# yangcaoai/CoDA_NeurIPS2023

Measured on NVIDIA H100. Metric: training scenes/sec (20k-pt SUN-RGBD synth, 256 queries), higher is better.
Workload: dtype fp32

## Files before the change

coda_neurips2023_b200/csrc/a32_prologue.cuh:

```cuda
#pragma once

namespace coda {
namespace a32 {

__device__ __forceinline__ float affine_relu(float x, float s, float h) { return fmaxf(fmaf(x, s, h), 0.f); }

__device__ __forceinline__ float bn_bwd(float y, float d, float s, float h, float al, float be) {
  return (fmaf(y, s, h) > 0.f ? s * d : 0.f) + fmaf(y, al, be);
}

__device__ __forceinline__ float bn_bwd_pooled(float y, float d, bool at_max, float s, float h, float al, float be) {
  return ((at_max && fmaf(y, s, h) > 0.f) ? s * d : 0.f) + fmaf(y, al, be);
}

__device__ __forceinline__ float bn_bwd_pooled_pre(float y, float d, bool at_max, float al, float be) {
  return (at_max ? d : 0.f) + fmaf(y, al, be);
}

}
}
```

coda_neurips2023_b200/csrc/gemm_a32_sm90.cu:

```cuda
#include "../../include/coda_gemm.h"
#include "a32_prologue.cuh"
#include "sm90_primitives.cuh"

#include <type_traits>

using namespace coda;

namespace {

constexpr int BM = 128;
constexpr int BK = 64;
constexpr int RAW_TILE = BM * BK * 4;
constexpr int A32_THREADS = 288;

struct A32Maps {
  CUtensorMap a;
  CUtensorMap a2;
  CUtensorMap b[3];
};

struct A32Params {
  int m, n, k;
  int mode;
  const float *scale;
  const float *shift;
  const float *alpha;
  const float *beta;
  const float *dpooled;
  const unsigned char *argmax;
  int group;
  const float *bias;
  int act;
  float *c;
  long long ldc;
  float *stats;
  int b_resident;
};

struct Alternation {
  int wg;
  bool started;
  __device__ __forceinline__ void begin() {
    if (wg == 1 || started) bar_sync(2 + wg, 256);
  }
  __device__ __forceinline__ void end() {
    bar_arrive(2 + (wg ^ 1), 256);
    started = true;
  }
  __device__ __forceinline__ void finish() {
    if (wg == 0 && started) bar_sync(2, 256);
  }
};

template <int NSPLIT, int BN, int RAW_KB, int B_STAGES, bool B_MN>
__global__ void __launch_bounds__(A32_THREADS, 1)
gemm_a32_kernel(const __grid_constant__ A32Maps maps, const A32Params P) {
  constexpr int MAX_RAW = RAW_KB / 32;
  constexpr int B_TILE = BN * BK * 2;
  constexpr int B_STAGE = NSPLIT * B_TILE;
  extern __shared__ __align__(1024) unsigned char smem_raw[];
  unsigned char *smem = smem_align1024(smem_raw);
  unsigned char *raw_ring = smem;
  const bool two_in = P.mode == CODA_A32_BN_BWD;
  const bool pooled = P.mode == CODA_A32_BN_BWD_POOLED || P.mode == CODA_A32_BN_BWD_POOLED_PRE;
  const int tile_groups = pooled ? (P.group >= BM ? 1 : BM / P.group) : 0;
  const int raw_stage_bytes = RAW_TILE * (two_in ? 2 : 1) + (tile_groups * 320 + 1023) / 1024 * 1024;
  const uint32_t nraw = (uint32_t)((RAW_KB * 1024) / raw_stage_bytes);
  unsigned char *b_ring = smem + (size_t)RAW_KB * 1024;
  float *s_stats = reinterpret_cast<float *>(b_ring + (size_t)B_STAGES * B_STAGE);
  __shared__ __align__(8) uint64_t raw_full[MAX_RAW], raw_empty[MAX_RAW];
  __shared__ __align__(8) uint64_t b_full[B_STAGES], b_empty[B_STAGES];

  const int warp = threadIdx.x >> 5, lane = threadIdx.x & 31;
  const int m = P.m, n = P.n;
  const int tiles_m = (m + BM - 1) / BM, tiles_n = (n + BN - 1) / BN;
  const long long nwork = (long long)tiles_m * tiles_n;
  const int nkb = (P.k + BK - 1) / BK;
  auto tile_at = [&](long long t, int &m0, int &n0) -> bool {
    if (P.b_resident) {
      const int per = (int)gridDim.x / tiles_n;
      const long long tm = (long long)(blockIdx.x / tiles_n) + t * per;
      if ((int)blockIdx.x >= per * tiles_n || tm >= tiles_m) return false;
      m0 = (int)tm * BM;
      n0 = (int)(blockIdx.x % tiles_n) * BN;
      return true;
    }
    const long long w = blockIdx.x + t * gridDim.x;
    if (w >= nwork) return false;
    n0 = (int)(w % tiles_n) * BN;
    m0 = (int)(w / tiles_n) * BM;
    return true;
  };

  if (threadIdx.x == 0) {
    for (int s = 0; s < MAX_RAW; ++s) { mbar_init(&raw_full[s], 1); mbar_init(&raw_empty[s], 8); }
    for (int s = 0; s < B_STAGES; ++s) { mbar_init(&b_full[s], 1); mbar_init(&b_empty[s], 2); }
    mbar_fence_init_cluster();
  }
  if (P.stats && warp < 8) {
    float *mine = s_stats + (size_t)warp * 2 * n;
    for (int i = lane; i < 2 * n; i += 32) mine[i] = 0.f;
  }
  __syncthreads();

  if (warp == 8) {
    if (lane == 0) {
      prefetch_tmap(&maps.a);
      if (two_in) prefetch_tmap(&maps.a2);
#pragma unroll
      for (int p = 0; p < NSPLIT; ++p) prefetch_tmap(&maps.b[p]);
    }
    uint32_t it = 0;
    int m0, n0;
    auto load_b = [&](int kb, int bs) {
      unsigned char *bt = b_ring + (size_t)bs * B_STAGE;
      mbar_arrive_expect_tx(&b_full[bs], (uint32_t)B_STAGE);
#pragma unroll
      for (int p = 0; p < NSPLIT; ++p) {
        if (!B_MN) {
          tma_load_3d(bt + p * B_TILE, &maps.b[p], &b_full[bs], kb * BK, n0, 0);
        } else {
#pragma unroll
          for (int g = 0; g < BN / 64; ++g)
            tma_load_3d(bt + p * B_TILE + g * 8192, &maps.b[p], &b_full[bs], n0 + g * 64, kb * BK, 0);
        }
      }
    };
    if (P.b_resident && tile_at(0, m0, n0)) {
      if (elect_one_sync())
        for (int kb = 0; kb < nkb; ++kb) load_b(kb, kb);
      __syncwarp();
    }
    for (long long t = 0; tile_at(t, m0, n0); ++t) {
      for (int kb = 0; kb < nkb; ++kb, ++it) {
        const int rs = it % nraw, bs = it % B_STAGES;
        mbar_wait(&raw_empty[rs], ((it / nraw) & 1u) ^ 1u);
        if (!P.b_resident) mbar_wait(&b_empty[bs], ((it / B_STAGES) & 1u) ^ 1u);
        if (elect_one_sync()) {
          unsigned char *rt = raw_ring + (size_t)rs * raw_stage_bytes;
          mbar_arrive_expect_tx(&raw_full[rs], (uint32_t)(RAW_TILE * (two_in ? 2 : 1) + tile_groups * 320));
          if (pooled) {
            const long long ngroups = P.m / P.group;
            for (int gt = 0; gt < tile_groups; ++gt) {
              long long g = (long long)m0 / P.group + gt;
              if (g >= ngroups) g = ngroups - 1;
              bulk_load_1d(rt + RAW_TILE + gt * 320, P.dpooled + g * P.k + kb * BK, 256, &raw_full[rs]);
              bulk_load_1d(rt + RAW_TILE + gt * 320 + 256, P.argmax + g * P.k + kb * BK, 64, &raw_full[rs]);
            }
          }
          tma_load_3d(rt, &maps.a, &raw_full[rs], kb * BK, m0, 0);
          tma_load_3d(rt + RAW_TILE / 2, &maps.a, &raw_full[rs], kb * BK + 32, m0, 0);
          if (two_in) {
            tma_load_3d(rt + RAW_TILE, &maps.a2, &raw_full[rs], kb * BK, m0, 0);
            tma_load_3d(rt + RAW_TILE + RAW_TILE / 2, &maps.a2, &raw_full[rs], kb * BK + 32, m0, 0);
          }
          if (!P.b_resident) load_b(kb, bs);
        }
        __syncwarp();
      }
    }
    return;
  }

  const int wg = warp >> 2, wl = warp & 3;
  const int g = lane >> 2, t4 = lane & 3;
  const int rloc[2] = {wg * 64 + wl * 16 + g, wg * 64 + wl * 16 + g + 8};
  float acc[BN / 2];
  uint32_t it = 0;
  int m0, n0;
  Alternation mma_turn{wg, false};
  for (long long t = 0; tile_at(t, m0, n0); ++t) {
    for (int kb = 0; kb < nkb; ++kb, ++it) {
      const int rs = it % nraw, bs = P.b_resident ? kb : (int)(it % B_STAGES);
      mbar_wait(&raw_full[rs], (it / nraw) & 1u);
      const unsigned char *rt = raw_ring + (size_t)rs * raw_stage_bytes;
      const int k0 = kb * BK;
      uint32_t af[BK / 16][NSPLIT][4];
      auto convert = [&](auto mode_tag) {
        constexpr int MODE = decltype(mode_tag)::value;
        const int mode = MODE >= 0 ? MODE : P.mode;
        int pgt = 0, pgi[2] = {0, 0};
        if (MODE < 0 && pooled) {
          pgt = P.group >= BM ? 0 : rloc[0] / P.group;
#pragma unroll
          for (int i = 0; i < 2; ++i) pgi[i] = (int)(((long long)m0 + rloc[i]) % P.group);
        }
#pragma unroll
        for (int kk = 0; kk < BK / 16; ++kk) {
#pragma unroll
          for (int c2 = 0; c2 < 2; ++c2) {
            const int col = kk * 16 + c2 * 8 + 2 * t4;
            const int kc = k0 + col;
            auto off = [&](int i) {
              const int row = rloc[i];
              return (uint32_t)(col >> 5) * (RAW_TILE / 2) + (uint32_t)row * 128u +
                     ((uint32_t)(((col & 31) >> 2) ^ (row & 7)) << 4) + (uint32_t)(col & 3) * 4u;
            };
            auto put = [&](int i, float2 x) {
              uint32_t w[NSPLIT];
              split_pair<NSPLIT>(x.x, x.y, w);
#pragma unroll
              for (int pl = 0; pl < NSPLIT; ++pl) af[kk][pl][c2 * 2 + i] = w[pl];
            };
            auto ld2 = [&](const float *v) { return __ldg(reinterpret_cast<const float2 *>(v + kc)); };
            if (mode == CODA_A32_AFFINE_RELU) {
              const float2 s2 = ld2(P.scale), h2 = ld2(P.shift);
#pragma unroll
              for (int i = 0; i < 2; ++i) {
                float2 x = *reinterpret_cast<const float2 *>(rt + off(i));
                x.x = a32::affine_relu(x.x, s2.x, h2.x);
                x.y = a32::affine_relu(x.y, s2.y, h2.y);
                put(i, x);
              }
            } else if (mode == CODA_A32_BN_BWD) {
              const float2 s2 = ld2(P.scale), h2 = ld2(P.shift), a2 = ld2(P.alpha), b2 = ld2(P.beta);
#pragma unroll
              for (int i = 0; i < 2; ++i) {
                float2 x = *reinterpret_cast<const float2 *>(rt + off(i));
                const float2 d = *reinterpret_cast<const float2 *>(rt + RAW_TILE + off(i));
                x.x = a32::bn_bwd(x.x, d.x, s2.x, h2.x, a2.x, b2.x);
                x.y = a32::bn_bwd(x.y, d.y, s2.y, h2.y, a2.y, b2.y);
                put(i, x);
              }
            } else if (mode == CODA_A32_BN_BWD_POOLED_PRE) {
              const unsigned char *px = rt + RAW_TILE + pgt * 320;
              const float2 a2 = ld2(P.alpha), b2 = ld2(P.beta);
              const float2 d = *reinterpret_cast<const float2 *>(px + col * 4);
              const uchar2 id = *reinterpret_cast<const uchar2 *>(px + 256 + col);
#pragma unroll
              for (int i = 0; i < 2; ++i) {
                float2 x = *reinterpret_cast<const float2 *>(rt + off(i));
                const int gi = pgi[i];
                x.x = a32::bn_bwd_pooled_pre(x.x, d.x, id.x == gi, a2.x, b2.x);
                x.y = a32::bn_bwd_pooled_pre(x.y, d.y, id.y == gi, a2.y, b2.y);
                put(i, x);
              }
            } else if (mode == CODA_A32_BN_BWD_POOLED) {
              const unsigned char *px = rt + RAW_TILE + pgt * 320;
              const float2 s2 = ld2(P.scale), h2 = ld2(P.shift), a2 = ld2(P.alpha), b2 = ld2(P.beta);
              const float2 d = *reinterpret_cast<const float2 *>(px + col * 4);
              const uchar2 id = *reinterpret_cast<const uchar2 *>(px + 256 + col);
#pragma unroll
              for (int i = 0; i < 2; ++i) {
                float2 x = *reinterpret_cast<const float2 *>(rt + off(i));
                const int gi = pgi[i];
                x.x = a32::bn_bwd_pooled(x.x, d.x, id.x == gi, s2.x, h2.x, a2.x, b2.x);
                x.y = a32::bn_bwd_pooled(x.y, d.y, id.y == gi, s2.y, h2.y, a2.y, b2.y);
                put(i, x);
              }
            } else {
#pragma unroll
              for (int i = 0; i < 2; ++i) put(i, *reinterpret_cast<const float2 *>(rt + off(i)));
            }
          }
        }
      };
      switch (P.mode) {
        case CODA_A32_PLAIN: convert(std::integral_constant<int, CODA_A32_PLAIN>{}); break;
        case CODA_A32_AFFINE_RELU: convert(std::integral_constant<int, CODA_A32_AFFINE_RELU>{}); break;
        default: convert(std::integral_constant<int, -1>{}); break;
      }
      __syncwarp();
      if (lane == 0) mbar_arrive(&raw_empty[rs]);
      mma_turn.begin();
      mbar_wait(&b_full[bs], P.b_resident ? 0u : ((it / B_STAGES) & 1u));
      unsigned char *bt = b_ring + (size_t)bs * B_STAGE;
      acc_fence(acc);
      wgmma_fence();
#pragma unroll
      for (int p = 0; p < n_products(NSPLIT); ++p) {
        const void *btile = bt + prod_b(NSPLIT, p) * B_TILE;
        const uint64_t bd = B_MN ? gmma_desc_mn_sw128(btile) : gmma_desc_k_sw128(btile);
        constexpr uint32_t KSTEP = B_MN ? 16 * 128 : 32;
#pragma unroll
        for (int kk = 0; kk < BK / 16; ++kk)
          Wgmma<BN, false>::template rs<B_MN ? 1 : 0>(acc, af[kk][prod_a(NSPLIT, p)], gmma_desc_advance(bd, kk * KSTEP),
                                                      (kb | p | kk) != 0);
      }
      wgmma_commit();
      mma_turn.end();
      wgmma_wait<0>();
      acc_fence(acc);
      if (!P.b_resident && (threadIdx.x & 127) == 0) mbar_arrive(&b_empty[bs]);
    }

    constexpr int EPI_C = 4;
#pragma unroll
    for (int cb = 0; cb < BN / 8; cb += EPI_C) {
      float csum[EPI_C][2], csq[EPI_C][2];
#pragma unroll
      for (int ci = 0; ci < EPI_C; ++ci) {
        const int c = cb + ci;
        const int col = n0 + c * 8 + 2 * t4;
        float cs0 = 0.f, cs1 = 0.f, cq0 = 0.f, cq1 = 0.f;
        const float bias0 = P.bias && col < n ? __ldg(P.bias + col) : 0.f;
        const float bias1 = P.bias && col + 1 < n ? __ldg(P.bias + col + 1) : 0.f;
#pragma unroll
        for (int i = 0; i < 2; ++i) {
          const int row = m0 + rloc[i];
          float v0 = acc[c * 4 + i * 2], v1 = acc[c * 4 + i * 2 + 1];
          if (P.bias) {
            if (col < n) v0 += bias0;
            if (col + 1 < n) v1 += bias1;
          }
          if (P.act == 1) { v0 = fmaxf(v0, 0.f); v1 = fmaxf(v1, 0.f); }
          if (row < m) {
            float *crow = P.c + (size_t)row * P.ldc;
            if (col + 1 < n) {
              *reinterpret_cast<float2 *>(crow + col) = make_float2(v0, v1);
            } else if (col < n) {
              crow[col] = v0;
            }
            cs0 += v0; cq0 = fmaf(v0, v0, cq0);
            cs1 += v1; cq1 = fmaf(v1, v1, cq1);
          }
        }
        csum[ci][0] = cs0; csum[ci][1] = cs1; csq[ci][0] = cq0; csq[ci][1] = cq1;
      }
      if (P.stats) {
        float *my_stats = s_stats + warp * 2 * n;
#pragma unroll
        for (int o = 4; o < 32; o <<= 1) {
#pragma unroll
          for (int ci = 0; ci < EPI_C; ++ci) {
#pragma unroll
            for (int j = 0; j < 2; ++j) {
              csum[ci][j] += __shfl_xor_sync(0xffffffffu, csum[ci][j], o);
              csq[ci][j] += __shfl_xor_sync(0xffffffffu, csq[ci][j], o);
            }
          }
        }
        if (g == 0) {
#pragma unroll
          for (int ci = 0; ci < EPI_C; ++ci) {
            const int col = n0 + (cb + ci) * 8 + 2 * t4;
#pragma unroll
            for (int j = 0; j < 2; ++j) {
              if (col + j < n) { my_stats[col + j] += csum[ci][j]; my_stats[n + col + j] += csq[ci][j]; }
            }
          }
        }
      }
    }
  }
  mma_turn.finish();
  if (P.stats) {
    bar_sync(1, 256);
    float *out = P.stats + (size_t)blockIdx.x * 2 * n;
    for (int i = threadIdx.x; i < 2 * n; i += 256) {
      float v = 0.f;
#pragma unroll
      for (int w = 0; w < 8; ++w) v += s_stats[(size_t)w * 2 * n + i];
      out[i] = v;
    }
  }
}

template <int NSPLIT, int BN, int RAW_KB, int B_STAGES, bool B_MN>
int launch_a32(const A32Maps &maps, const A32Params &P, cudaStream_t s) {
  static_assert(RAW_KB % 64 == 0 || RAW_KB == 96, "raw region");
  constexpr size_t smem = (size_t)RAW_KB * 1024 + (size_t)B_STAGES * NSPLIT * BN * BK * 2 + 1024;
  const size_t total = smem + (P.stats ? (size_t)16 * P.n * 4 : 0);
  constexpr size_t SMEM_MAX = 227 * 1024 - 2048;
  if (total > SMEM_MAX) return CODA_ETOOLARGE;
  if (P.mode == CODA_A32_BN_BWD && RAW_KB < 64) return CODA_EINVAL;
  constexpr auto kern = gemm_a32_kernel<NSPLIT, BN, RAW_KB, B_STAGES, B_MN>;
  if (const int st = raise_smem_limit<kern>((int)SMEM_MAX)) return st;
  const int tiles_m = (P.m + BM - 1) / BM, tiles_n = (P.n + BN - 1) / BN;
  const long long nwork = (long long)tiles_m * tiles_n;
  unsigned grid = (unsigned)(nwork < sm_count() ? nwork : sm_count());
  A32Params Q = P;
  const int nkb = (P.k + BK - 1) / BK;
  Q.b_resident = (nkb <= B_STAGES && tiles_n <= sm_count() && tiles_m >= 4 * (sm_count() / tiles_n)) ? 1 : 0;
  if (Q.b_resident) grid = (unsigned)((sm_count() / tiles_n) * tiles_n);
  kern<<<grid, A32_THREADS, total, s>>>(maps, Q);
  return launch_status();
}

}

extern "C" {

int coda_gemm_a32_grid(int m, int n) {
  if (m <= 0 || n <= 0) return 0;
  return sm_count();
}

int coda_gemm_a32(int nsplit, int m, int n, int k, const float *a, long long lda, int a_mode, const float *a_scale,
                  const float *a_shift, const float *a_alpha, const float *a_beta, const float *a2, long long lda2,
                  const unsigned char *a_argmax, int a_group, const void *b_planes, long long b_plane_stride,
                  int b_ld, int b_mn, const float *bias, int act, float *c, long long ldc, float *col_stats,
                  void *stream) {
  if (nsplit < 2 || nsplit > 3 || m < 0 || n < 0 || k <= 0) return CODA_EINVAL;
  if (m == 0 || n == 0) return CODA_OK;
  if (!a || !b_planes || !c || b_ld % 64 != 0 || (lda & 3) || (ldc & 3) || ((uintptr_t)a & 15) || ((uintptr_t)c & 15))
    return CODA_EINVAL;
  if (a_mode < CODA_A32_PLAIN || a_mode > CODA_A32_BN_BWD_POOLED_PRE) return CODA_EINVAL;
  if (a_mode != CODA_A32_PLAIN && (!a_scale || !a_shift || (k & 3))) return CODA_EINVAL;
  if (a_mode >= CODA_A32_BN_BWD && (!a2 || !a_alpha || !a_beta || ((uintptr_t)a2 & 15))) return CODA_EINVAL;
  if (a_mode == CODA_A32_BN_BWD && (lda2 & 3)) return CODA_EINVAL;
  if ((a_mode == CODA_A32_BN_BWD_POOLED || a_mode == CODA_A32_BN_BWD_POOLED_PRE) &&
      (!a_argmax || a_group < 32 || a_group > 256 || m % a_group != 0 || k % 64 != 0 ||
       !(a_group % 128 == 0 || 128 % a_group == 0) || a_group % 32 != 0))
    return CODA_EINVAL;
  const long long tiles128 = (long long)((m + BM - 1) / BM) * ((n + 127) / 128);
  const int bn = (n <= 64 || tiles128 <= sm_count() / 2) ? 64 : 128;
  A32Maps maps;
  int st = make_tmap_f32_box(&maps.a, a, k, m, lda, 32, BM);
  if (st != CODA_OK) return st;
  maps.a2 = maps.a;
  if (a_mode == CODA_A32_BN_BWD) {
    st = make_tmap_f32_box(&maps.a2, a2, k, m, lda2, 32, BM);
    if (st != CODA_OK) return st;
  }
  const int kpad = (k + 63) / 64 * 64;
  const char *bp = (const char *)b_planes;
  for (int p = 0; p < nsplit; ++p) {
    if (!b_mn) {
      if (b_ld < kpad) return CODA_EINVAL;
      st = make_tmap_k_major_16b(&maps.b[p], bp + (size_t)p * b_plane_stride * 2, 0, b_ld, n, 1, b_ld, 0, bn);
    } else {
      if (b_ld < n) return CODA_EINVAL;
      st = make_tmap_k_major_16b(&maps.b[p], bp + (size_t)p * b_plane_stride * 2, 0, b_ld, k, 1, b_ld, 0, 64);
    }
    if (st != CODA_OK) return st;
  }
  for (int p = nsplit; p < 3; ++p) maps.b[p] = maps.b[0];
  A32Params P;
  P.m = m; P.n = n; P.k = k; P.mode = a_mode; P.scale = a_scale; P.shift = a_shift; P.alpha = a_alpha; P.beta = a_beta;
  P.dpooled = a2; P.argmax = a_argmax; P.group = a_group; P.bias = bias; P.act = act; P.c = c; P.ldc = ldc; P.stats = col_stats;
  P.b_resident = 0;
  cudaStream_t s = (cudaStream_t)stream;
#define CODA_A32(NS, BN_, RS, BS)                                                   \
  return b_mn ? launch_a32<NS, BN_, RS, BS, true>(maps, P, s) : launch_a32<NS, BN_, RS, BS, false>(maps, P, s)
  const bool deep_b = !col_stats && k > 128 && a_mode != CODA_A32_BN_BWD;
  if (nsplit == 2) {
    if (bn == 64) CODA_A32(2, 64, 128, 4);
    CODA_A32(2, 128, 128, 2);
  }
  if (bn == 64) CODA_A32(3, 64, 128, 3);
  if (deep_b) CODA_A32(3, 128, 64, 3);
  CODA_A32(3, 128, 96, 2);
#undef CODA_A32
}

}
```

coda_neurips2023_b200/csrc/gemm_tn32_sm90.cu:

```cuda
#include "../../include/coda_gemm.h"
#include "a32_prologue.cuh"
#include "sm90_primitives.cuh"

using namespace coda;

namespace {

constexpr int BM = 128;
constexpr int BKR = 32;
constexpr int NS = 2;
constexpr int RAW_STAGES = 2, PL_STAGES = 3;
constexpr int TW = 8;
constexpr int TN32_THREADS = 288;

struct TN32Maps {
  CUtensorMap a, a2, b;
};

struct TN32Params {
  long long rows;
  int m, n;
  int a_mode, b_mode;
  const float *a_scale, *a_shift, *a_alpha, *a_beta;
  const float *dpooled;
  const unsigned char *argmax;
  int group;
  const float *b_scale, *b_shift;
  float *a_colsum;
  float *partial;
  float *c;
  long long ldc;
  int ksplit;
};

template <int BN>
__global__ void __launch_bounds__(TN32_THREADS, 1)
gemm_tn32_kernel(const __grid_constant__ TN32Maps maps, const TN32Params P) {
  constexpr int RAW_A = BKR * BM * 4;
  constexpr int RAW_B = BKR * BN * 4;
  constexpr int RAW_X = 1024;
  constexpr int RAW_STAGE = 2 * RAW_A + RAW_B + RAW_X;
  constexpr int PL_A = BKR * BM * 2;
  constexpr int PL_B = BKR * BN * 2;
  constexpr int PL_STAGE = NS * (PL_A + PL_B);
  extern __shared__ __align__(1024) unsigned char smem_raw[];
  unsigned char *smem = smem_align1024(smem_raw);
  unsigned char *raw_ring = smem;
  unsigned char *pl_ring = smem + (size_t)RAW_STAGES * RAW_STAGE;
  __shared__ __align__(8) uint64_t raw_full[RAW_STAGES], raw_empty[RAW_STAGES];
  __shared__ __align__(16) float s_colsum[TW][BM];

  const int warp = threadIdx.x >> 5, lane = threadIdx.x & 31;
  const int tiles_n = (P.n + BN - 1) / BN;
  const int tile = blockIdx.x / P.ksplit, ks = blockIdx.x % P.ksplit;
  const int m0 = (tile / tiles_n) * BM, n0 = (tile % tiles_n) * BN;
  const long long nkb_total = (P.rows + BKR - 1) / BKR;
  const long long per = (nkb_total + P.ksplit - 1) / P.ksplit;
  const long long kb0 = (long long)ks * per;
  const long long nkb = max(0ll, min(per, nkb_total - kb0));
  const bool two_in = P.a_mode == CODA_A32_BN_BWD;

  if (threadIdx.x == 0) {
    for (int s = 0; s < RAW_STAGES; ++s) { mbar_init(&raw_full[s], 1); mbar_init(&raw_empty[s], TW); }
    mbar_fence_init_cluster();
  }
  __syncthreads();

  if (warp == 8) {
    if (lane == 0) {
      prefetch_tmap(&maps.a);
      prefetch_tmap(&maps.b);
      if (two_in) prefetch_tmap(&maps.a2);
    }
    const bool pooled = P.a_mode == CODA_A32_BN_BWD_POOLED || P.a_mode == CODA_A32_BN_BWD_POOLED_PRE;
    const uint32_t bytes = (uint32_t)(RAW_A * (two_in ? 2 : 1) + RAW_B + (pooled ? 640 : 0));
    const long long ngroups = pooled ? P.rows / P.group : 0;
    for (long long i = 0; i < nkb; ++i) {
      const int rs = (int)(i % RAW_STAGES);
      mbar_wait(&raw_empty[rs], (uint32_t)((i / RAW_STAGES) & 1) ^ 1u);
      if (elect_one_sync()) {
        unsigned char *st = raw_ring + (size_t)rs * RAW_STAGE;
        const int r0 = (int)((kb0 + i) * BKR);
        mbar_arrive_expect_tx(&raw_full[rs], bytes);
        if (pooled) {
          long long g = (long long)r0 / P.group;
          if (g >= ngroups) g = ngroups - 1;
          bulk_load_1d(st + 2 * RAW_A + RAW_B, P.dpooled + g * P.m + m0, 512, &raw_full[rs]);
          bulk_load_1d(st + 2 * RAW_A + RAW_B + 512, P.argmax + g * P.m + m0, 128, &raw_full[rs]);
        }
#pragma unroll
        for (int g = 0; g < BM / 32; ++g) tma_load_3d(st + g * 4096, &maps.a, &raw_full[rs], m0 + g * 32, r0, 0);
        if (two_in) {
#pragma unroll
          for (int g = 0; g < BM / 32; ++g) tma_load_3d(st + RAW_A + g * 4096, &maps.a2, &raw_full[rs], m0 + g * 32, r0, 0);
        }
#pragma unroll
        for (int g = 0; g < BN / 32; ++g) tma_load_3d(st + 2 * RAW_A + g * 4096, &maps.b, &raw_full[rs], n0 + g * 32, r0, 0);
      }
      __syncwarp();
    }
    return;
  }

  const int tw = warp;
  const int wg = warp >> 2;
  const bool want_colsum = P.a_colsum != nullptr && n0 == 0;
  float4 csum = make_float4(0.f, 0.f, 0.f, 0.f);
  const int ca = m0 + lane * 4;
  float4 sa = make_float4(0.f, 0.f, 0.f, 0.f), ta = sa, al = sa, be = sa;
  if (P.a_mode != CODA_A32_PLAIN && ca < P.m) {
    sa = __ldg(reinterpret_cast<const float4 *>(P.a_scale + ca));
    ta = __ldg(reinterpret_cast<const float4 *>(P.a_shift + ca));
    al = __ldg(reinterpret_cast<const float4 *>(P.a_alpha + ca));
    be = __ldg(reinterpret_cast<const float4 *>(P.a_beta + ca));
  }
  constexpr int B_CHUNKS = BN / 4, B_RPP = 32 / B_CHUNKS;
  const int bch = lane % B_CHUNKS, brow_off = lane / B_CHUNKS;
  const int cb = n0 + bch * 4;
  float4 sb = make_float4(0.f, 0.f, 0.f, 0.f), tb = sb;
  if (P.b_mode == CODA_A32_AFFINE_RELU && cb < P.n) {
    sb = __ldg(reinterpret_cast<const float4 *>(P.b_scale + cb));
    tb = __ldg(reinterpret_cast<const float4 *>(P.b_shift + cb));
  }
  const bool a_col_ok = ca < P.m;
  const bool pooled_mode = P.a_mode == CODA_A32_BN_BWD_POOLED || P.a_mode == CODA_A32_BN_BWD_POOLED_PRE;
  int rem0 = pooled_mode ? (int)((kb0 * BKR) % P.group) : 0;
  int rs = 0, ps = 0;
  uint32_t raw_par = 0;
  float acc[BN / 2];
  for (long long i = 0; i < nkb; ++i) {
    mbar_wait_relaxed(&raw_full[rs], raw_par);
    const unsigned char *raw = raw_ring + (size_t)rs * RAW_STAGE;
    unsigned char *pl = pl_ring + (size_t)ps * PL_STAGE;
    const long long r0 = (kb0 + i) * BKR;
    const bool tail = r0 + BKR > P.rows;
#pragma unroll
      for (int j = 0; j < BKR / TW; ++j) {
        const int r = tw + j * TW;
        const long long grow = r0 + r;
        const uint32_t roff = (uint32_t)(lane >> 3) * 4096u + (uint32_t)r * 128u + (uint32_t)(((lane & 7) ^ (r & 7)) << 4);
        float4 y = *reinterpret_cast<const float4 *>(raw + roff);
        float4 o = y;
        if (P.a_mode == CODA_A32_BN_BWD) {
          const float4 d = *reinterpret_cast<const float4 *>(raw + RAW_A + roff);
          o.x = a32::bn_bwd(y.x, d.x, sa.x, ta.x, al.x, be.x);
          o.y = a32::bn_bwd(y.y, d.y, sa.y, ta.y, al.y, be.y);
          o.z = a32::bn_bwd(y.z, d.z, sa.z, ta.z, al.z, be.z);
          o.w = a32::bn_bwd(y.w, d.w, sa.w, ta.w, al.w, be.w);
        } else if (P.a_mode == CODA_A32_BN_BWD_POOLED_PRE) {
          const int gi = rem0 + r;
          const float4 d = *reinterpret_cast<const float4 *>(raw + 2 * RAW_A + RAW_B + lane * 16);
          const uchar4 id = *reinterpret_cast<const uchar4 *>(raw + 2 * RAW_A + RAW_B + 512 + lane * 4);
          o.x = a32::bn_bwd_pooled_pre(y.x, d.x, id.x == gi, al.x, be.x);
          o.y = a32::bn_bwd_pooled_pre(y.y, d.y, id.y == gi, al.y, be.y);
          o.z = a32::bn_bwd_pooled_pre(y.z, d.z, id.z == gi, al.z, be.z);
          o.w = a32::bn_bwd_pooled_pre(y.w, d.w, id.w == gi, al.w, be.w);
        } else if (P.a_mode == CODA_A32_BN_BWD_POOLED) {
          const int gi = rem0 + r;
          const float4 d = *reinterpret_cast<const float4 *>(raw + 2 * RAW_A + RAW_B + lane * 16);
          const uchar4 id = *reinterpret_cast<const uchar4 *>(raw + 2 * RAW_A + RAW_B + 512 + lane * 4);
          o.x = a32::bn_bwd_pooled(y.x, d.x, id.x == gi, sa.x, ta.x, al.x, be.x);
          o.y = a32::bn_bwd_pooled(y.y, d.y, id.y == gi, sa.y, ta.y, al.y, be.y);
          o.z = a32::bn_bwd_pooled(y.z, d.z, id.z == gi, sa.z, ta.z, al.z, be.z);
          o.w = a32::bn_bwd_pooled(y.w, d.w, id.w == gi, sa.w, ta.w, al.w, be.w);
        }
        if (tail && grow >= P.rows) o = make_float4(0.f, 0.f, 0.f, 0.f);
        if (want_colsum) { csum.x += o.x; csum.y += o.y; csum.z += o.z; csum.w += o.w; }
        const int col = lane * 4;
        split_store4<NS>(o, reinterpret_cast<__nv_bfloat16 *>(pl + (col >> 6) * (BKR * 128) + r * 128 +
                                                              ((((col & 63) >> 3) ^ (r & 7)) << 4) + ((col & 7) >> 2) * 8),
                         PL_A / 2);
      }
#pragma unroll
      for (int j = 0; j < BKR / (TW * B_RPP); ++j) {
        const int r = (tw + j * TW) * B_RPP + brow_off;
        const long long grow = r0 + r;
        const uint32_t roff = (uint32_t)(bch >> 3) * 4096u + (uint32_t)r * 128u + (uint32_t)(((bch & 7) ^ (r & 7)) << 4);
        float4 v = *reinterpret_cast<const float4 *>(raw + 2 * RAW_A + roff);
        if (P.b_mode == CODA_A32_AFFINE_RELU) {
          v.x = a32::affine_relu(v.x, sb.x, tb.x); v.y = a32::affine_relu(v.y, sb.y, tb.y);
          v.z = a32::affine_relu(v.z, sb.z, tb.z); v.w = a32::affine_relu(v.w, sb.w, tb.w);
        }
        if (tail && grow >= P.rows) v = make_float4(0.f, 0.f, 0.f, 0.f);
        const int col = bch * 4;
        split_store4<NS>(v, reinterpret_cast<__nv_bfloat16 *>(pl + NS * PL_A + (col >> 6) * (BKR * 128) + r * 128 +
                                                              ((((col & 63) >> 3) ^ (r & 7)) << 4) + ((col & 7) >> 2) * 8),
                         PL_B / 2);
      }
      fence_proxy_async_smem();
      __syncwarp();
      if (lane == 0) mbar_arrive(&raw_empty[rs]);
      bar_sync(1, 256);
      acc_fence(acc);
      wgmma_fence();
#pragma unroll
      for (int p = 0; p < n_products(NS); ++p) {
        const uint64_t ad = gmma_desc_mn_sw128(pl + prod_a(NS, p) * PL_A + wg * (BKR * 128), BKR * 128);
        const uint64_t bd = gmma_desc_mn_sw128(pl + NS * PL_A + prod_b(NS, p) * PL_B, BKR * 128);
#pragma unroll
        for (int kk = 0; kk < BKR / 16; ++kk)
          Wgmma<BN, false>::template ss<1, 1>(acc, gmma_desc_advance(ad, kk * 16 * 128), gmma_desc_advance(bd, kk * 16 * 128),
                                              (i | p | kk) != 0);
      }
      wgmma_commit();
      wgmma_wait<1>();
      acc_fence(acc);
      if (++rs == RAW_STAGES) { rs = 0; raw_par ^= 1u; }
      if (++ps == PL_STAGES) ps = 0;
      if (pooled_mode) { rem0 += BKR; if (rem0 >= P.group) rem0 -= P.group; }
  }
  wgmma_wait<0>();
  acc_fence(acc);
  if (nkb == 0) acc_zero(acc);
  *reinterpret_cast<float4 *>(&s_colsum[tw][lane * 4]) = csum;
  {
    const int g = lane >> 2, t4 = lane & 3;
    float *slot = P.partial + ((long long)tile * P.ksplit + ks) * (BM * BN);
#pragma unroll
    for (int i = 0; i < 2; ++i) {
      const int rl = wg * 64 + (warp & 3) * 16 + g + 8 * i, row = m0 + rl;
      float *crow = P.c + (size_t)row * P.ldc;
#pragma unroll
      for (int c = 0; c < BN / 8; ++c) {
        const int col = n0 + c * 8 + 2 * t4;
        const float2 v = make_float2(acc[c * 4 + i * 2], acc[c * 4 + i * 2 + 1]);
        if (P.ksplit > 1) *reinterpret_cast<float2 *>(slot + (size_t)rl * BN + c * 8 + 2 * t4) = v;
        else if (row < P.m && col < P.n) *reinterpret_cast<float2 *>(crow + col) = v;
      }
    }
  }
  bar_sync(1, 256);
  if (P.a_colsum && n0 == 0 && threadIdx.x < BM) {
    float cs = 0.f;
#pragma unroll
    for (int w = 0; w < TW; ++w) cs += s_colsum[w][threadIdx.x];
    if (P.ksplit > 1) {
      const int tiles_m = (P.m + BM - 1) / BM;
      P.partial[(long long)tiles_m * (tiles_n * P.ksplit) * (BM * BN) + ((long long)(m0 / BM) * P.ksplit + ks) * BM +
                threadIdx.x] = cs;
    } else if (m0 + (int)threadIdx.x < P.m) {
      P.a_colsum[m0 + threadIdx.x] = cs;
    }
  }
}

__global__ void __launch_bounds__(256)
colsum_reduce_kernel(const float *__restrict__ parts, int ksplit, int m, float *__restrict__ a_colsum) {
  const int col = blockIdx.x * blockDim.x + threadIdx.x;
  if (col >= m) return;
  const float *src = parts + ((long long)(col / BM) * ksplit) * BM + col % BM;
  float v = 0.f;
  for (int k = 0; k < ksplit; ++k) v += src[(long long)k * BM];
  a_colsum[col] = v;
}

template <int BN>
int launch_tn32(const TN32Maps &maps, TN32Params P, float *c, long long ldc, cudaStream_t s) {
  constexpr size_t smem = (size_t)RAW_STAGES * (2 * BKR * BM * 4 + BKR * BN * 4 + 1024) +
                          (size_t)PL_STAGES * NS * (BKR * BM * 2 + BKR * BN * 2) + 1024;
  static_assert(smem <= 227 * 1024, "smem budget");
  constexpr auto kern = gemm_tn32_kernel<BN>;
  if (const int st = raise_smem_limit<kern>((int)smem)) return st;
  const int num_sms = sm_count();
  const int tiles = ((P.m + BM - 1) / BM) * ((P.n + BN - 1) / BN);
  const long long nkb_total = (P.rows + BKR - 1) / BKR;
  int ksplit = num_sms / tiles;
  if (ksplit < 1) ksplit = 1;
  if (ksplit > nkb_total / 4) ksplit = (int)(nkb_total / 4 > 0 ? nkb_total / 4 : 1);
  P.ksplit = ksplit;
  const int tiles_m = (P.m + BM - 1) / BM;
  if (ksplit > 1) {
    const int st = split_scratch((size_t)tiles * ksplit * BM * BN + (size_t)tiles_m * ksplit * BM, s, &P.partial);
    if (st != CODA_OK) return st;
  }
  kern<<<tiles * ksplit, TN32_THREADS, smem, s>>>(maps, P);
  if (ksplit > 1) {
    const long long total = (long long)P.m * P.n;
    const long long blocks = (total + 255) / 256;
    splitk_reduce_kernel<<<(unsigned)(blocks < 8 * num_sms ? blocks : 8 * num_sms), 256, 0, s>>>(
        P.partial, ksplit, P.m, P.n, 1, BM, BN, nullptr, c, ldc, 0);
    if (P.a_colsum)
      colsum_reduce_kernel<<<(P.m + 255) / 256, 256, 0, s>>>(P.partial + (size_t)tiles * ksplit * BM * BN, ksplit, P.m,
                                                            P.a_colsum);
  }
  return launch_status();
}

}

extern "C" {

int coda_gemm_tn32(long long rows, int m, int n, const float *a, long long lda, int a_mode, const float *a_scale,
                   const float *a_shift, const float *a_alpha, const float *a_beta, const float *a2, long long lda2,
                   const unsigned char *a_argmax, int a_group, const float *b, long long ldb, int b_mode,
                   const float *b_scale, const float *b_shift, float *c, long long ldc, float *a_colsum, void *stream) {
  if (rows <= 0 || m <= 0 || n <= 0 || !a || !b || !c) return CODA_EINVAL;
  if ((lda & 3) || (ldb & 3) || (ldc & 3) || (m & 3) || (n & 3)) return CODA_EINVAL;
  if (((uintptr_t)a | (uintptr_t)b | (uintptr_t)c) & 15) return CODA_EINVAL;
  if (a_mode != CODA_A32_PLAIN && a_mode != CODA_A32_BN_BWD && a_mode != CODA_A32_BN_BWD_POOLED &&
      a_mode != CODA_A32_BN_BWD_POOLED_PRE)
    return CODA_EINVAL;
  if (b_mode != CODA_A32_PLAIN && b_mode != CODA_A32_AFFINE_RELU) return CODA_EINVAL;
  if (a_mode != CODA_A32_PLAIN && (!a_scale || !a_shift || !a_alpha || !a_beta || !a2 || ((uintptr_t)a2 & 15))) return CODA_EINVAL;
  if (a_mode == CODA_A32_BN_BWD && (lda2 & 3)) return CODA_EINVAL;
  if ((a_mode == CODA_A32_BN_BWD_POOLED || a_mode == CODA_A32_BN_BWD_POOLED_PRE) &&
      (!a_argmax || a_group < 32 || a_group > 256 || a_group % 32 != 0 || rows % a_group != 0 || m % 128 != 0))
    return CODA_EINVAL;
  if (b_mode == CODA_A32_AFFINE_RELU && (!b_scale || !b_shift)) return CODA_EINVAL;
  TN32Maps maps;
  int st = make_tmap_f32_box(&maps.a, a, m, rows, lda, 32, BKR);
  if (st != CODA_OK) return st;
  maps.a2 = maps.a;
  if (a_mode == CODA_A32_BN_BWD) {
    st = make_tmap_f32_box(&maps.a2, a2, m, rows, lda2, 32, BKR);
    if (st != CODA_OK) return st;
  }
  st = make_tmap_f32_box(&maps.b, b, n, rows, ldb, 32, BKR);
  if (st != CODA_OK) return st;
  TN32Params P;
  P.rows = rows; P.m = m; P.n = n; P.a_mode = a_mode; P.b_mode = b_mode;
  P.a_scale = a_scale; P.a_shift = a_shift; P.a_alpha = a_alpha; P.a_beta = a_beta;
  P.dpooled = a2; P.argmax = a_argmax; P.group = a_group; P.b_scale = b_scale; P.b_shift = b_shift; P.a_colsum = a_colsum; P.partial = nullptr; P.c = c; P.ldc = ldc; P.ksplit = 1;
  cudaStream_t s = (cudaStream_t)stream;
  if (n <= 64) return launch_tn32<64>(maps, P, c, ldc, s);
  return launch_tn32<128>(maps, P, c, ldc, s);
}

}
```

coda_neurips2023_b200/csrc/sa_mlp_kernels.cu:

```cuda
#include <cuda_bf16.h>
#include <math.h>
#include <stdint.h>

#include "../../include/coda_sa_mlp.h"
#include "coda_common.cuh"
#include "operand_split.cuh"

namespace {

constexpr int THREADS = 256;
constexpr int MAX_BLOCKS = 132 * 4;

__host__ __device__ inline bool channels_ok(int c) { return c >= 4 && c <= 1024 && c % 4 == 0 && THREADS % (c / 4) == 0; }

__host__ inline unsigned grid_for(long long rows, int c) {
  const long long per_iter = THREADS / (c / 4);
  const long long need = (rows + per_iter - 1) / per_iter;
  return (unsigned)(need < MAX_BLOCKS ? (need > 0 ? need : 1) : MAX_BLOCKS);
}

struct Affine4 {
  float4 mean, invstd, gamma, beta;
};
__device__ __forceinline__ Affine4 load_affine(const float *mean, const float *invstd, const float *gamma,
                                               const float *beta, int c4) {
  Affine4 a;
  a.mean = __ldg(reinterpret_cast<const float4 *>(mean) + c4);
  a.invstd = __ldg(reinterpret_cast<const float4 *>(invstd) + c4);
  a.gamma = __ldg(reinterpret_cast<const float4 *>(gamma) + c4);
  a.beta = __ldg(reinterpret_cast<const float4 *>(beta) + c4);
  return a;
}
__device__ __forceinline__ float4 xhat4(const float4 v, const Affine4 &a) {
  return make_float4((v.x - a.mean.x) * a.invstd.x, (v.y - a.mean.y) * a.invstd.y, (v.z - a.mean.z) * a.invstd.z,
                     (v.w - a.mean.w) * a.invstd.w);
}
__device__ __forceinline__ float4 bn4(const float4 xh, const Affine4 &a) {
  return make_float4(xh.x * a.gamma.x + a.beta.x, xh.y * a.gamma.y + a.beta.y, xh.z * a.gamma.z + a.beta.z,
                     xh.w * a.gamma.w + a.beta.w);
}

template <int NV>
__device__ __forceinline__ void reduce_slots(float4 (&acc)[NV], int cq, int slot, int c4, float4 *red ) {
#pragma unroll
  for (int i = 0; i < NV; ++i) {
    __syncthreads();
    red[threadIdx.x] = acc[i];
    __syncthreads();
    if (slot == 0) {
      float4 t = acc[i];
      for (int s = 1; s < THREADS / cq; ++s) {
        const float4 o = red[s * cq + c4];
        t.x += o.x; t.y += o.y; t.z += o.z; t.w += o.w;
      }
      acc[i] = t;
    }
  }
}

template <int CIN>
__global__ void __launch_bounds__(THREADS)
linear_small_k_kernel(long long rows, int cout, const float *__restrict__ x, const float *__restrict__ w,
                      float *__restrict__ y) {
  const int cq = cout >> 2, c4 = threadIdx.x % cq, slot = threadIdx.x / cq, nslots = THREADS / cq;
  float wr[4][CIN];
#pragma unroll
  for (int j = 0; j < 4; ++j)
#pragma unroll
    for (int k = 0; k < CIN; ++k) wr[j][k] = __ldg(w + (size_t)(c4 * 4 + j) * CIN + k);
  for (long long r = (long long)blockIdx.x * nslots + slot; r < rows; r += (long long)gridDim.x * nslots) {
    float xv[CIN];
#pragma unroll
    for (int k = 0; k < CIN; ++k) xv[k] = __ldg(x + r * CIN + k);
    float o[4];
#pragma unroll
    for (int j = 0; j < 4; ++j) {
      float a = xv[0] * wr[j][0];
#pragma unroll
      for (int k = 1; k < CIN; ++k) a = fmaf(xv[k], wr[j][k], a);
      o[j] = a;
    }
    reinterpret_cast<float4 *>(y + r * cout)[c4] = make_float4(o[0], o[1], o[2], o[3]);
  }
}

__global__ void __launch_bounds__(THREADS)
bn_stats_partial_kernel(long long rows, int c, const float *__restrict__ y, float *__restrict__ partial) {
  __shared__ float4 red[THREADS];
  const int cq = c >> 2, c4 = threadIdx.x % cq, slot = threadIdx.x / cq, nslots = THREADS / cq;
  float4 acc[2] = {make_float4(0.f, 0.f, 0.f, 0.f), make_float4(0.f, 0.f, 0.f, 0.f)};
  for (long long r = (long long)blockIdx.x * nslots + slot; r < rows; r += (long long)gridDim.x * nslots) {
    const float4 v = __ldg(reinterpret_cast<const float4 *>(y + r * c) + c4);
    acc[0].x += v.x; acc[0].y += v.y; acc[0].z += v.z; acc[0].w += v.w;
    acc[1].x = fmaf(v.x, v.x, acc[1].x); acc[1].y = fmaf(v.y, v.y, acc[1].y);
    acc[1].z = fmaf(v.z, v.z, acc[1].z); acc[1].w = fmaf(v.w, v.w, acc[1].w);
  }
  reduce_slots<2>(acc, cq, slot, c4, red);
  if (slot == 0) {
    float4 *p = reinterpret_cast<float4 *>(partial + (size_t)blockIdx.x * 2 * c);
    p[c4] = acc[0];
    p[cq + c4] = acc[1];
  }
}
__device__ __forceinline__ void warp_partials_sum(int nblocks, int c, int ch, const float *__restrict__ partial,
                                                  double &s, double &q) {
  const int lane = threadIdx.x & 31;
  s = 0.0; q = 0.0;
  for (int b = lane; b < nblocks; b += 32) {
    s += (double)partial[(size_t)b * 2 * c + ch];
    q += (double)partial[(size_t)b * 2 * c + c + ch];
  }
#pragma unroll
  for (int o = 16; o > 0; o >>= 1) {
    s += __shfl_xor_sync(0xffffffffu, s, o);
    q += __shfl_xor_sync(0xffffffffu, q, o);
  }
}
__global__ void __launch_bounds__(256)
bn_stats_finalize_kernel(int nblocks, long long rows, int c, const float *__restrict__ partial,
                         float eps, float momentum, float *running_mean, float *running_var,
                         float *__restrict__ mean, float *__restrict__ invstd) {
  const int ch = blockIdx.x * 8 + (threadIdx.x >> 5);
  if (ch >= c) return;
  double s, q;
  warp_partials_sum(nblocks, c, ch, partial, s, q);
  if ((threadIdx.x & 31) != 0) return;
  const double n = (double)rows, m = s / n;
  double var = q / n - m * m;
  if (var < 0.0) var = 0.0;
  mean[ch] = (float)m;
  invstd[ch] = (float)(1.0 / sqrt(var + (double)eps));
  if (running_mean) running_mean[ch] = (1.0f - momentum) * running_mean[ch] + momentum * (float)m;
  if (running_var) running_var[ch] = (1.0f - momentum) * running_var[ch] + momentum * (float)(var * (n / fmax(n - 1.0, 1.0)));
}

__global__ void __launch_bounds__(256)
bn_stats_finalize_affine_kernel(int nblocks, long long rows, int c, int cpad,
                                                const float *__restrict__ partial, float eps, float momentum,
                                                float *running_mean, float *running_var, const float *__restrict__ gamma,
                                                const float *__restrict__ beta, float *__restrict__ mean,
                                                float *__restrict__ invstd, float *__restrict__ scale,
                                                float *__restrict__ shift) {
  const int ch = blockIdx.x * 8 + (threadIdx.x >> 5);
  if (ch >= cpad) return;
  if (ch >= c) {
    if (scale && (threadIdx.x & 31) == 0) { scale[ch] = 0.f; shift[ch] = 0.f; }
    return;
  }
  double s, q;
  warp_partials_sum(nblocks, c, ch, partial, s, q);
  if ((threadIdx.x & 31) != 0) return;
  const double n = (double)rows, m = s / n;
  double var = q / n - m * m;
  if (var < 0.0) var = 0.0;
  const float is = (float)(1.0 / sqrt(var + (double)eps));
  mean[ch] = (float)m;
  invstd[ch] = is;
  if (running_mean) running_mean[ch] = (1.0f - momentum) * running_mean[ch] + momentum * (float)m;
  if (running_var) running_var[ch] = (1.0f - momentum) * running_var[ch] + momentum * (float)(var * (n / fmax(n - 1.0, 1.0)));
  if (scale) {
    const float sc = gamma[ch] * is;
    scale[ch] = sc;
    shift[ch] = beta[ch] - (float)m * sc;
  }
}
__global__ void __launch_bounds__(256)
bn_sums_f64_kernel(int nblocks, int c, const float *__restrict__ partial, double *__restrict__ sums) {
  const int ch = blockIdx.x * 8 + (threadIdx.x >> 5);
  if (ch >= c) return;
  double s, q;
  warp_partials_sum(nblocks, c, ch, partial, s, q);
  if ((threadIdx.x & 31) != 0) return;
  sums[ch] = s;
  sums[c + ch] = q;
}
__global__ void __launch_bounds__(256)
bn_finalize_sums_kernel(long long rows, int c, int cpad, const double *__restrict__ sums, float eps, float momentum,
                        float *running_mean, float *running_var, const float *__restrict__ gamma,
                        const float *__restrict__ beta, float *__restrict__ mean, float *__restrict__ invstd,
                        float *__restrict__ scale, float *__restrict__ shift) {
  const int ch = blockIdx.x * blockDim.x + threadIdx.x;
  if (ch >= cpad) return;
  if (ch >= c) {
    if (scale) { scale[ch] = 0.f; shift[ch] = 0.f; }
    return;
  }
  const double n = (double)rows, m = sums[ch] / n;
  double var = sums[c + ch] / n - m * m;
  if (var < 0.0) var = 0.0;
  const float is = (float)(1.0 / sqrt(var + (double)eps));
  mean[ch] = (float)m;
  invstd[ch] = is;
  if (running_mean) running_mean[ch] = (1.0f - momentum) * running_mean[ch] + momentum * (float)m;
  if (running_var) running_var[ch] = (1.0f - momentum) * running_var[ch] + momentum * (float)(var * (n / fmax(n - 1.0, 1.0)));
  if (scale) {
    const float sc = gamma[ch] * is;
    scale[ch] = sc;
    shift[ch] = beta[ch] - (float)m * sc;
  }
}

__global__ void bn_bwd_coefs_kernel(int c, int cpad, long long rows, const float *__restrict__ mean,
                                    const float *__restrict__ invstd, const float *__restrict__ gamma,
                                    const float *__restrict__ s1, const float *__restrict__ s2,
                                    float *__restrict__ alpha, float *__restrict__ beta) {
  const int ch = blockIdx.x * blockDim.x + threadIdx.x;
  if (ch >= cpad) return;
  if (ch >= c) { alpha[ch] = 0.f; beta[ch] = 0.f; return; }
  const float inv_n = 1.0f / (float)rows;
  const float sc = gamma[ch] * invstd[ch];
  const float a = -sc * invstd[ch] * (s2[ch] * inv_n);
  alpha[ch] = a;
  beta[ch] = -sc * (s1[ch] * inv_n) - a * mean[ch];
}

__global__ void __launch_bounds__(THREADS)
colsum_partial_kernel(long long rows, int c, const float *__restrict__ x, float *__restrict__ partial) {
  __shared__ float4 red[THREADS];
  const int cq = c >> 2, c4 = threadIdx.x % cq, slot = threadIdx.x / cq, nslots = THREADS / cq;
  float4 acc[1] = {make_float4(0.f, 0.f, 0.f, 0.f)};
  for (long long r = (long long)blockIdx.x * nslots + slot; r < rows; r += (long long)gridDim.x * nslots) {
    const float4 v = __ldg(reinterpret_cast<const float4 *>(x + r * c) + c4);
    acc[0].x += v.x; acc[0].y += v.y; acc[0].z += v.z; acc[0].w += v.w;
  }
  reduce_slots<1>(acc, cq, slot, c4, red);
  if (slot == 0) reinterpret_cast<float4 *>(partial + (size_t)blockIdx.x * c)[c4] = acc[0];
}
__global__ void __launch_bounds__(256)
colsum_finalize_kernel(int nblocks, int c, const float *__restrict__ partial, float *__restrict__ out) {
  const int ch = blockIdx.x * 8 + (threadIdx.x >> 5), lane = threadIdx.x & 31;
  if (ch >= c) return;
  float a = 0.f;
  for (int k = lane; k < nblocks; k += 32) a += partial[(size_t)k * c + ch];
#pragma unroll
  for (int o = 16; o > 0; o >>= 1) a += __shfl_xor_sync(0xffffffffu, a, o);
  if (lane == 0) out[ch] = a;
}

template <int NS>
__global__ void __launch_bounds__(THREADS)
bn_relu_pack_kernel(long long rows, int c, const float *__restrict__ y, const float *__restrict__ mean,
                    const float *__restrict__ invstd, const float *__restrict__ gamma, const float *__restrict__ beta,
                    __nv_bfloat16 *__restrict__ planes) {
  const int cq = c >> 2, c4 = threadIdx.x % cq, slot = threadIdx.x / cq, nslots = THREADS / cq;
  const Affine4 a = load_affine(mean, invstd, gamma, beta, c4);
  const size_t plane_stride = (size_t)rows * c;
  for (long long r = (long long)blockIdx.x * nslots + slot; r < rows; r += (long long)gridDim.x * nslots) {
    const float4 z = bn4(xhat4(__ldg(reinterpret_cast<const float4 *>(y + r * c) + c4), a), a);
    coda::split_store4<NS>(make_float4(fmaxf(z.x, 0.f), fmaxf(z.y, 0.f), fmaxf(z.z, 0.f), fmaxf(z.w, 0.f)),
                           planes + r * c + c4 * 4, plane_stride);
  }
}

__global__ void __launch_bounds__(THREADS)
bn_relu_maxpool_kernel(long long groups, int group, int c, const float *__restrict__ y, const float *__restrict__ mean,
                       const float *__restrict__ invstd, const float *__restrict__ gamma,
                       const float *__restrict__ beta, float *__restrict__ pooled, unsigned char *__restrict__ argmax) {
  __shared__ float4 sval[THREADS];
  __shared__ uchar4 sidx[THREADS];
  const int cq = c >> 2, c4 = threadIdx.x % cq, slot = threadIdx.x / cq, nslots = THREADS / cq;
  const Affine4 a = load_affine(mean, invstd, gamma, beta, c4);
  for (long long g = blockIdx.x; g < groups; g += gridDim.x) {
    float4 best = make_float4(-INFINITY, -INFINITY, -INFINITY, -INFINITY);
    uchar4 bi = make_uchar4(0, 0, 0, 0);
    for (int i = slot; i < group; i += nslots) {
      const float4 zz = bn4(xhat4(__ldg(reinterpret_cast<const float4 *>(y + (g * group + i) * c) + c4), a), a);
      const float4 z = make_float4(fmaxf(zz.x, 0.f), fmaxf(zz.y, 0.f), fmaxf(zz.z, 0.f), fmaxf(zz.w, 0.f));
      if (z.x > best.x) { best.x = z.x; bi.x = (unsigned char)i; }
      if (z.y > best.y) { best.y = z.y; bi.y = (unsigned char)i; }
      if (z.z > best.z) { best.z = z.z; bi.z = (unsigned char)i; }
      if (z.w > best.w) { best.w = z.w; bi.w = (unsigned char)i; }
    }
    __syncthreads();
    sval[threadIdx.x] = best;
    sidx[threadIdx.x] = bi;
    __syncthreads();
    if (slot == 0) {
      for (int s = 1; s < nslots; ++s) {
        const float4 o = sval[s * cq + c4];
        const uchar4 oi = sidx[s * cq + c4];
        if (o.x > best.x || (o.x == best.x && oi.x < bi.x)) { best.x = o.x; bi.x = oi.x; }
        if (o.y > best.y || (o.y == best.y && oi.y < bi.y)) { best.y = o.y; bi.y = oi.y; }
        if (o.z > best.z || (o.z == best.z && oi.z < bi.z)) { best.z = o.z; bi.z = oi.z; }
        if (o.w > best.w || (o.w == best.w && oi.w < bi.w)) { best.w = o.w; bi.w = oi.w; }
      }
      reinterpret_cast<float4 *>(pooled + g * c)[c4] = best;
      reinterpret_cast<uchar4 *>(argmax + g * c)[c4] = bi;
    }
  }
}

__global__ void __launch_bounds__(THREADS)
bn_relu_bwd_reduce_kernel(long long rows, int c, const float *__restrict__ y, const float *__restrict__ dz,
                          const float *__restrict__ mean, const float *__restrict__ invstd,
                          const float *__restrict__ gamma, const float *__restrict__ beta, float *__restrict__ partial) {
  __shared__ float4 red[THREADS];
  const int cq = c >> 2, c4 = threadIdx.x % cq, slot = threadIdx.x / cq, nslots = THREADS / cq;
  const Affine4 a = load_affine(mean, invstd, gamma, beta, c4);
  float4 acc[2] = {make_float4(0.f, 0.f, 0.f, 0.f), make_float4(0.f, 0.f, 0.f, 0.f)};
  for (long long r = (long long)blockIdx.x * nslots + slot; r < rows; r += (long long)gridDim.x * nslots) {
    const float4 xh = xhat4(__ldg(reinterpret_cast<const float4 *>(y + r * c) + c4), a);
    const float4 z = bn4(xh, a);
    float4 d = __ldg(reinterpret_cast<const float4 *>(dz + r * c) + c4);
    d.x = z.x > 0.f ? d.x : 0.f; d.y = z.y > 0.f ? d.y : 0.f; d.z = z.z > 0.f ? d.z : 0.f; d.w = z.w > 0.f ? d.w : 0.f;
    acc[0].x += d.x; acc[0].y += d.y; acc[0].z += d.z; acc[0].w += d.w;
    acc[1].x = fmaf(d.x, xh.x, acc[1].x); acc[1].y = fmaf(d.y, xh.y, acc[1].y);
    acc[1].z = fmaf(d.z, xh.z, acc[1].z); acc[1].w = fmaf(d.w, xh.w, acc[1].w);
  }
  reduce_slots<2>(acc, cq, slot, c4, red);
  if (slot == 0) {
    float4 *p = reinterpret_cast<float4 *>(partial + (size_t)blockIdx.x * 2 * c);
    p[c4] = acc[0];
    p[cq + c4] = acc[1];
  }
}
__global__ void __launch_bounds__(THREADS)
bn_relu_bwd_reduce_pooled_kernel(long long groups, int group, int c, const float *__restrict__ y,
                                 const float *__restrict__ dpooled, const unsigned char *__restrict__ argmax,
                                 const float *__restrict__ mean, const float *__restrict__ invstd,
                                 const float *__restrict__ gamma, const float *__restrict__ beta,
                                 float *__restrict__ partial, float *__restrict__ dprime) {
  __shared__ float4 red[THREADS];
  const int cq = c >> 2, c4 = threadIdx.x % cq, slot = threadIdx.x / cq, nslots = THREADS / cq;
  const Affine4 a = load_affine(mean, invstd, gamma, beta, c4);
  float4 acc[2] = {make_float4(0.f, 0.f, 0.f, 0.f), make_float4(0.f, 0.f, 0.f, 0.f)};
  for (long long g = (long long)blockIdx.x * nslots + slot; g < groups; g += (long long)gridDim.x * nslots) {
    const uchar4 id = __ldg(reinterpret_cast<const uchar4 *>(argmax + g * c) + c4);
    const float *base = y + g * group * c + c4 * 4;
    const float4 v = make_float4(__ldg(base + (size_t)id.x * c), __ldg(base + (size_t)id.y * c + 1),
                                 __ldg(base + (size_t)id.z * c + 2), __ldg(base + (size_t)id.w * c + 3));
    const float4 xh = xhat4(v, a);
    const float4 z = bn4(xh, a);
    float4 d = __ldg(reinterpret_cast<const float4 *>(dpooled + g * c) + c4);
    d.x = z.x > 0.f ? d.x : 0.f; d.y = z.y > 0.f ? d.y : 0.f; d.z = z.z > 0.f ? d.z : 0.f; d.w = z.w > 0.f ? d.w : 0.f;
    if (dprime)
      reinterpret_cast<float4 *>(dprime + g * c)[c4] =
          make_float4(a.gamma.x * a.invstd.x * d.x, a.gamma.y * a.invstd.y * d.y, a.gamma.z * a.invstd.z * d.z,
                      a.gamma.w * a.invstd.w * d.w);
    acc[0].x += d.x; acc[0].y += d.y; acc[0].z += d.z; acc[0].w += d.w;
    acc[1].x = fmaf(d.x, xh.x, acc[1].x); acc[1].y = fmaf(d.y, xh.y, acc[1].y);
    acc[1].z = fmaf(d.z, xh.z, acc[1].z); acc[1].w = fmaf(d.w, xh.w, acc[1].w);
  }
  reduce_slots<2>(acc, cq, slot, c4, red);
  if (slot == 0) {
    float4 *p = reinterpret_cast<float4 *>(partial + (size_t)blockIdx.x * 2 * c);
    p[c4] = acc[0];
    p[cq + c4] = acc[1];
  }
}
__global__ void __launch_bounds__(256)
sums_finalize_kernel(int nblocks, int c, const float *__restrict__ partial, float *__restrict__ s1,
                     float *__restrict__ s2) {
  const int ch = blockIdx.x * 8 + (threadIdx.x >> 5);
  if (ch >= c) return;
  double a, b;
  warp_partials_sum(nblocks, c, ch, partial, a, b);
  if ((threadIdx.x & 31) == 0) {
    s1[ch] = (float)a;
    s2[ch] = (float)b;
  }
}

struct BwdCoef4 {
  float4 k, m1, m2;
};
__device__ __forceinline__ BwdCoef4 load_coef(const Affine4 &a, const float *s1, const float *s2, int c4, float inv_n) {
  const float4 t1 = __ldg(reinterpret_cast<const float4 *>(s1) + c4), t2 = __ldg(reinterpret_cast<const float4 *>(s2) + c4);
  BwdCoef4 q;
  q.k = make_float4(a.gamma.x * a.invstd.x, a.gamma.y * a.invstd.y, a.gamma.z * a.invstd.z, a.gamma.w * a.invstd.w);
  q.m1 = make_float4(t1.x * inv_n, t1.y * inv_n, t1.z * inv_n, t1.w * inv_n);
  q.m2 = make_float4(t2.x * inv_n, t2.y * inv_n, t2.z * inv_n, t2.w * inv_n);
  return q;
}
__device__ __forceinline__ float4 dy4(const float4 d, const float4 xh, const BwdCoef4 &q) {
  return make_float4(q.k.x * (d.x - q.m1.x - xh.x * q.m2.x), q.k.y * (d.y - q.m1.y - xh.y * q.m2.y),
                     q.k.z * (d.z - q.m1.z - xh.z * q.m2.z), q.k.w * (d.w - q.m1.w - xh.w * q.m2.w));
}

template <int NS, bool POOLED>
__global__ void __launch_bounds__(THREADS)
bn_relu_bwd_pack_kernel(long long rows, int c, const float *__restrict__ y, const float *__restrict__ dz,
                        const float *__restrict__ dpooled, const unsigned char *__restrict__ argmax, int group,
                        const float *__restrict__ mean, const float *__restrict__ invstd,
                        const float *__restrict__ gamma, const float *__restrict__ beta, const float *__restrict__ s1,
                        const float *__restrict__ s2, __nv_bfloat16 *__restrict__ planes) {
  const int cq = c >> 2, c4 = threadIdx.x % cq, slot = threadIdx.x / cq, nslots = THREADS / cq;
  const Affine4 a = load_affine(mean, invstd, gamma, beta, c4);
  const BwdCoef4 q = load_coef(a, s1, s2, c4, 1.0f / (float)rows);
  const size_t plane_stride = (size_t)rows * c;
  for (long long r = (long long)blockIdx.x * nslots + slot; r < rows; r += (long long)gridDim.x * nslots) {
    const float4 xh = xhat4(__ldg(reinterpret_cast<const float4 *>(y + r * c) + c4), a);
    const float4 z = bn4(xh, a);
    float4 d;
    if (POOLED) {
      const long long g = r / group;
      const int i = (int)(r - g * group);
      const uchar4 id = __ldg(reinterpret_cast<const uchar4 *>(argmax + g * c) + c4);
      const float4 dp = __ldg(reinterpret_cast<const float4 *>(dpooled + g * c) + c4);
      d = make_float4(id.x == i ? dp.x : 0.f, id.y == i ? dp.y : 0.f, id.z == i ? dp.z : 0.f, id.w == i ? dp.w : 0.f);
    } else {
      d = __ldg(reinterpret_cast<const float4 *>(dz + r * c) + c4);
    }
    d.x = z.x > 0.f ? d.x : 0.f; d.y = z.y > 0.f ? d.y : 0.f; d.z = z.z > 0.f ? d.z : 0.f; d.w = z.w > 0.f ? d.w : 0.f;
    coda::split_store4<NS>(dy4(d, xh, q), planes + r * c + c4 * 4, plane_stride);
  }
}

template <int CIN>
__global__ void __launch_bounds__(THREADS)
bn_relu_bwd_small_k_kernel(long long rows, int c, const float *__restrict__ y, const float *__restrict__ dz,
                           const float *__restrict__ mean, const float *__restrict__ invstd,
                           const float *__restrict__ gamma, const float *__restrict__ beta,
                           const float *__restrict__ s1, const float *__restrict__ s2, const float *__restrict__ x,
                           float *__restrict__ partial) {
  __shared__ float4 red[THREADS];
  const int cq = c >> 2, c4 = threadIdx.x % cq, slot = threadIdx.x / cq, nslots = THREADS / cq;
  const Affine4 a = load_affine(mean, invstd, gamma, beta, c4);
  const BwdCoef4 q = load_coef(a, s1, s2, c4, 1.0f / (float)rows);
  float4 acc[CIN];
#pragma unroll
  for (int k = 0; k < CIN; ++k) acc[k] = make_float4(0.f, 0.f, 0.f, 0.f);
  for (long long r = (long long)blockIdx.x * nslots + slot; r < rows; r += (long long)gridDim.x * nslots) {
    const float4 xh = xhat4(__ldg(reinterpret_cast<const float4 *>(y + r * c) + c4), a);
    const float4 z = bn4(xh, a);
    float4 d = __ldg(reinterpret_cast<const float4 *>(dz + r * c) + c4);
    d.x = z.x > 0.f ? d.x : 0.f; d.y = z.y > 0.f ? d.y : 0.f; d.z = z.z > 0.f ? d.z : 0.f; d.w = z.w > 0.f ? d.w : 0.f;
    const float4 g = dy4(d, xh, q);
#pragma unroll
    for (int k = 0; k < CIN; ++k) {
      const float xv = __ldg(x + r * CIN + k);
      acc[k].x = fmaf(g.x, xv, acc[k].x); acc[k].y = fmaf(g.y, xv, acc[k].y);
      acc[k].z = fmaf(g.z, xv, acc[k].z); acc[k].w = fmaf(g.w, xv, acc[k].w);
    }
  }
  reduce_slots<CIN>(acc, cq, slot, c4, red);
  if (slot == 0) {
    float *p = partial + (size_t)blockIdx.x * c * CIN;
#pragma unroll
    for (int k = 0; k < CIN; ++k) {
      p[(size_t)(c4 * 4 + 0) * CIN + k] = acc[k].x;
      p[(size_t)(c4 * 4 + 1) * CIN + k] = acc[k].y;
      p[(size_t)(c4 * 4 + 2) * CIN + k] = acc[k].z;
      p[(size_t)(c4 * 4 + 3) * CIN + k] = acc[k].w;
    }
  }
}
__global__ void dw_finalize_kernel(int nblocks, int n, const float *__restrict__ partial, float *__restrict__ dw) {
  const int i = blockIdx.x * blockDim.x + threadIdx.x;
  if (i >= n) return;
  double a = 0.0;
  for (int k = 0; k < nblocks; ++k) a += (double)partial[(size_t)k * n + i];
  dw[i] = (float)a;
}

}

extern "C" {

long long coda_bn_rows_scratch_floats(int c) { return (long long)MAX_BLOCKS * 2 * c; }
long long coda_bn_rows_small_k_scratch_floats(int cin, int cout) { return (long long)MAX_BLOCKS * cin * cout; }

int coda_rows_linear_small_k(long long rows, int cin, int cout, const float *x, const float *w, float *y,
                             void *stream) {
  if (rows < 0 || cin < 1 || cin > 8 || !channels_ok(cout)) return CODA_EINVAL;
  if (rows == 0) return CODA_OK;
  if (!x || !w || !y) return CODA_EINVAL;
  cudaStream_t s = (cudaStream_t)stream;
  const unsigned grid = grid_for(rows, cout);
#define CODA_CASE(K) case K: linear_small_k_kernel<K><<<grid, THREADS, 0, s>>>(rows, cout, x, w, y); break;
  switch (cin) { CODA_CASE(1) CODA_CASE(2) CODA_CASE(3) CODA_CASE(4) CODA_CASE(5) CODA_CASE(6) CODA_CASE(7) CODA_CASE(8) }
#undef CODA_CASE
  return coda::launch_status();
}

int coda_bn_rows_stats(long long rows, int c, const float *y, float eps, float momentum, float *running_mean,
                       float *running_var, float *mean, float *invstd, float *scratch, void *stream) {
  if (rows <= 0 || !channels_ok(c) || !y || !mean || !invstd || !scratch) return CODA_EINVAL;
  cudaStream_t s = (cudaStream_t)stream;
  const unsigned grid = grid_for(rows, c);
  bn_stats_partial_kernel<<<grid, THREADS, 0, s>>>(rows, c, y, scratch);
  bn_stats_finalize_kernel<<<(c + 7) / 8, 256, 0, s>>>((int)grid, rows, c, scratch, eps, momentum, running_mean,
                                                           running_var, mean, invstd);
  return coda::launch_status();
}

int coda_bn_rows_stats_affine(long long rows, int c, const float *y, float eps, float momentum, float *running_mean,
                               float *running_var, const float *gamma, const float *beta, float *mean, float *invstd,
                               float *scale, float *shift, float *scratch, void *stream) {
  if (rows <= 0 || !channels_ok(c) || !y || !mean || !invstd || !scratch || !gamma || !beta || !scale || !shift)
    return CODA_EINVAL;
  cudaStream_t s = (cudaStream_t)stream;
  const unsigned grid = grid_for(rows, c);
  bn_stats_partial_kernel<<<grid, THREADS, 0, s>>>(rows, c, y, scratch);
  const int cpad = (c + 63) / 64 * 64;
  bn_stats_finalize_affine_kernel<<<(cpad + 7) / 8, 256, 0, s>>>((int)grid, rows, c, cpad, scratch, eps, momentum,
                                                                    running_mean, running_var, gamma, beta, mean,
                                                                    invstd, scale, shift);
  return coda::launch_status();
}

int coda_bn_stats_finalize(int nblocks, long long rows, int c, const float *partial, float eps, float momentum,
                           float *running_mean, float *running_var, const float *gamma, const float *beta,
                           float *mean, float *invstd, float *scale, float *shift, void *stream) {
  if (nblocks <= 0 || rows <= 0 || c <= 0 || !partial || !mean || !invstd) return CODA_EINVAL;
  if ((scale != nullptr) != (shift != nullptr) || (scale && (!gamma || !beta))) return CODA_EINVAL;
  const int cpad = (c + 63) / 64 * 64;
  bn_stats_finalize_affine_kernel<<<(cpad + 7) / 8, 256, 0, (cudaStream_t)stream>>>(
      nblocks, rows, c, cpad, partial, eps, momentum, running_mean, running_var, gamma, beta, mean, invstd, scale, shift);
  return coda::launch_status();
}

int coda_bn_rows_sums(long long rows, int c, const float *y, double *sums, float *scratch, void *stream) {
  if (rows <= 0 || !channels_ok(c) || !y || !sums || !scratch) return CODA_EINVAL;
  cudaStream_t s = (cudaStream_t)stream;
  const unsigned grid = grid_for(rows, c);
  bn_stats_partial_kernel<<<grid, THREADS, 0, s>>>(rows, c, y, scratch);
  bn_sums_f64_kernel<<<(c + 7) / 8, 256, 0, s>>>((int)grid, c, scratch, sums);
  return coda::launch_status();
}

int coda_bn_partials_sums(int nblocks, int c, const float *partial, double *sums, void *stream) {
  if (nblocks <= 0 || c <= 0 || !partial || !sums) return CODA_EINVAL;
  bn_sums_f64_kernel<<<(c + 7) / 8, 256, 0, (cudaStream_t)stream>>>(nblocks, c, partial, sums);
  return coda::launch_status();
}

int coda_bn_stats_finalize_sums(long long rows, int c, const double *sums, float eps, float momentum,
                                float *running_mean, float *running_var, const float *gamma, const float *beta,
                                float *mean, float *invstd, float *scale, float *shift, void *stream) {
  if (rows <= 0 || c <= 0 || !sums || !mean || !invstd) return CODA_EINVAL;
  if ((scale != nullptr) != (shift != nullptr) || (scale && (!gamma || !beta))) return CODA_EINVAL;
  const int cpad = scale ? (c + 63) / 64 * 64 : c;
  bn_finalize_sums_kernel<<<(cpad + 127) / 128, 128, 0, (cudaStream_t)stream>>>(
      rows, c, cpad, sums, eps, momentum, running_mean, running_var, gamma, beta, mean, invstd, scale, shift);
  return coda::launch_status();
}

int coda_bn_bwd_coefs(int c, long long rows, const float *mean, const float *invstd, const float *gamma,
                      const float *s1, const float *s2, float *alpha, float *beta, void *stream) {
  if (c <= 0 || rows <= 0 || !mean || !invstd || !gamma || !s1 || !s2 || !alpha || !beta) return CODA_EINVAL;
  const int cpad = (c + 63) / 64 * 64;
  bn_bwd_coefs_kernel<<<(cpad + 127) / 128, 128, 0, (cudaStream_t)stream>>>(c, cpad, rows, mean, invstd, gamma, s1, s2,
                                                                           alpha, beta);
  return coda::launch_status();
}

int coda_rows_colsum(long long rows, int c, const float *x, float *out, float *scratch, void *stream) {
  if (rows <= 0 || !channels_ok(c) || !x || !out || !scratch) return CODA_EINVAL;
  cudaStream_t s = (cudaStream_t)stream;
  unsigned grid = grid_for(rows, c);
  if (grid > 132) grid = 132;
  colsum_partial_kernel<<<grid, THREADS, 0, s>>>(rows, c, x, scratch);
  colsum_finalize_kernel<<<(c + 7) / 8, 256, 0, s>>>((int)grid, c, scratch, out);
  return coda::launch_status();
}

int coda_bn_relu_pack_rows(long long rows, int c, int nsplit, const float *y, const float *mean,
                           const float *invstd, const float *gamma, const float *beta, void *planes,
                           void *stream) {
  if (rows < 0 || !channels_ok(c) || c % 64 != 0 || nsplit < 1 || nsplit > 3) return CODA_EINVAL;
  if (rows == 0) return CODA_OK;
  if (!y || !mean || !invstd || !gamma || !beta || !planes) return CODA_EINVAL;
  cudaStream_t s = (cudaStream_t)stream;
  const unsigned grid = grid_for(rows, c);
  __nv_bfloat16 *p = (__nv_bfloat16 *)planes;
  if (nsplit == 1) bn_relu_pack_kernel<1><<<grid, THREADS, 0, s>>>(rows, c, y, mean, invstd, gamma, beta, p);
  else if (nsplit == 2) bn_relu_pack_kernel<2><<<grid, THREADS, 0, s>>>(rows, c, y, mean, invstd, gamma, beta, p);
  else bn_relu_pack_kernel<3><<<grid, THREADS, 0, s>>>(rows, c, y, mean, invstd, gamma, beta, p);
  return coda::launch_status();
}

int coda_bn_relu_maxpool_rows(long long groups, int group, int c, const float *y, const float *mean,
                              const float *invstd, const float *gamma, const float *beta, float *pooled,
                              unsigned char *argmax, void *stream) {
  if (groups < 0 || group < 1 || group > 256 || !channels_ok(c)) return CODA_EINVAL;
  if (groups == 0) return CODA_OK;
  if (!y || !mean || !invstd || !gamma || !beta || !pooled || !argmax) return CODA_EINVAL;
  const unsigned grid = (unsigned)(groups < 132 * 8 ? groups : 132 * 8);
  bn_relu_maxpool_kernel<<<grid, THREADS, 0, (cudaStream_t)stream>>>(groups, group, c, y, mean, invstd, gamma, beta,
                                                                    pooled, argmax);
  return coda::launch_status();
}

int coda_bn_relu_bwd_reduce(long long rows, int c, const float *y, const float *dz, const float *mean,
                            const float *invstd, const float *gamma, const float *beta, float *s1, float *s2,
                            float *scratch, void *stream) {
  if (rows <= 0 || !channels_ok(c) || !y || !dz || !mean || !invstd || !gamma || !beta || !s1 || !s2 || !scratch)
    return CODA_EINVAL;
  cudaStream_t s = (cudaStream_t)stream;
  const unsigned grid = grid_for(rows, c);
  bn_relu_bwd_reduce_kernel<<<grid, THREADS, 0, s>>>(rows, c, y, dz, mean, invstd, gamma, beta, scratch);
  sums_finalize_kernel<<<(c + 7) / 8, 256, 0, s>>>((int)grid, c, scratch, s1, s2);
  return coda::launch_status();
}

int coda_bn_relu_bwd_reduce_pooled(long long groups, int group, int c, const float *y, const float *dpooled,
                                   const unsigned char *argmax, const float *mean, const float *invstd,
                                   const float *gamma, const float *beta, float *s1, float *s2, float *scratch,
                                   float *dprime, void *stream) {
  if (groups <= 0 || group < 1 || group > 256 || !channels_ok(c) || !y || !dpooled || !argmax || !mean || !invstd ||
      !gamma || !beta || !s1 || !s2 || !scratch)
    return CODA_EINVAL;
  cudaStream_t s = (cudaStream_t)stream;
  const unsigned grid = grid_for(groups, c);
  bn_relu_bwd_reduce_pooled_kernel<<<grid, THREADS, 0, s>>>(groups, group, c, y, dpooled, argmax, mean, invstd, gamma,
                                                           beta, scratch, dprime);
  sums_finalize_kernel<<<(c + 7) / 8, 256, 0, s>>>((int)grid, c, scratch, s1, s2);
  return coda::launch_status();
}

int coda_bn_relu_bwd_pack(long long rows, int c, int nsplit, const float *y, const float *dz,
                          const float *dpooled, const unsigned char *argmax, int group, const float *mean,
                          const float *invstd, const float *gamma, const float *beta, const float *s1,
                          const float *s2, void *planes, void *stream) {
  if (rows < 0 || !channels_ok(c) || c % 64 != 0 || nsplit < 1 || nsplit > 3) return CODA_EINVAL;
  if (rows == 0) return CODA_OK;
  if (!y || !mean || !invstd || !gamma || !beta || !s1 || !s2 || !planes) return CODA_EINVAL;
  const bool pooled = dz == nullptr;
  if (pooled && (!dpooled || !argmax || group < 1 || group > 256 || rows % group != 0)) return CODA_EINVAL;
  cudaStream_t s = (cudaStream_t)stream;
  const unsigned grid = grid_for(rows, c);
  __nv_bfloat16 *p = (__nv_bfloat16 *)planes;
#define CODA_LAUNCH(NS, P) \
  bn_relu_bwd_pack_kernel<NS, P><<<grid, THREADS, 0, s>>>(rows, c, y, dz, dpooled, argmax, group, mean, invstd, gamma, \
                                                          beta, s1, s2, p)
  if (pooled) {
    if (nsplit == 1) CODA_LAUNCH(1, true); else if (nsplit == 2) CODA_LAUNCH(2, true); else CODA_LAUNCH(3, true);
  } else {
    if (nsplit == 1) CODA_LAUNCH(1, false); else if (nsplit == 2) CODA_LAUNCH(2, false); else CODA_LAUNCH(3, false);
  }
#undef CODA_LAUNCH
  return coda::launch_status();
}

int coda_bn_relu_bwd_small_k(long long rows, int cin, int cout, const float *y, const float *dz, const float *mean,
                             const float *invstd, const float *gamma, const float *beta, const float *s1,
                             const float *s2, const float *x, float *dw, float *scratch, void *stream) {
  if (rows <= 0 || cin < 1 || cin > 8 || !channels_ok(cout)) return CODA_EINVAL;
  if (!y || !dz || !mean || !invstd || !gamma || !beta || !s1 || !s2 || !x || !dw || !scratch) return CODA_EINVAL;
  cudaStream_t s = (cudaStream_t)stream;
  const unsigned grid = grid_for(rows, cout);
#define CODA_CASE(K)                                                                                              \
  case K:                                                                                                         \
    bn_relu_bwd_small_k_kernel<K><<<grid, THREADS, 0, s>>>(rows, cout, y, dz, mean, invstd, gamma, beta, s1, s2, x, \
                                                           scratch);                                             \
    break;
  switch (cin) { CODA_CASE(1) CODA_CASE(2) CODA_CASE(3) CODA_CASE(4) CODA_CASE(5) CODA_CASE(6) CODA_CASE(7) CODA_CASE(8) }
#undef CODA_CASE
  dw_finalize_kernel<<<(cin * cout + 127) / 128, 128, 0, s>>>((int)grid, cin * cout, scratch, dw);
  return coda::launch_status();
}

}
```

coda_neurips2023_b200/ops.py:

```python
from __future__ import annotations

import ctypes

import torch

from ._lib import check, lib, ptr, stream_of

_i = ctypes.c_int
_ll = ctypes.c_longlong
_f = ctypes.c_float


def _need_cuda(t: torch.Tensor, name: str) -> None:
    if not t.is_cuda:
        raise RuntimeError(f"{name}: CPU not supported (coda_b200 kernels are CUDA-only)")


def _f32c(t: torch.Tensor) -> torch.Tensor:
    if t.dtype != torch.float32:
        t = t.float()
    return t.contiguous()


class GradSink:
# ... 499 lines not shown
    def backward(ctx, dout):
        y, gamma, beta, mean, invstd = ctx.saved_tensors
        dc = _f32c(dout)
        rows, c = y.shape
        dev = y.device
        sg, sb = _sink(gamma), _sink(beta)
        if sg is None or sb is None:
            sg = sb = None
        s1 = torch.empty(c, dtype=torch.float32, device=dev) if sb is None else sb
        s2 = torch.empty(c, dtype=torch.float32, device=dev) if sg is None else sg
        dy = torch.empty_like(y)
        L = lib()
        seed = ptr(_seed_dev(dev) if ctx.p > 0 else None)
        args = (_ll(rows), _i(c), ptr(y), ptr(dc), ptr(mean), ptr(invstd), ptr(gamma), ptr(beta),
                _i(1 if ctx.relu else 0), _f(ctx.p), _uint(ctx.salt), seed)
        with torch.cuda.device(dev):
            check(L.coda_bn_act_rows_bwd_reduce(*args, ptr(s1), ptr(s2), ptr(_bn_scratch(c, dev)), stream_of(y)),
                  "bn_act_rows_bwd_reduce")
            t1, t2 = bn_sync_backward_sums(s1, s2) if ctx.sync else (s1, s2)
            check(L.coda_bn_act_rows_bwd(*args, ptr(t1), ptr(t2), ptr(dy), stream_of(y)), "bn_act_rows_bwd")
        if sg is not None:
            return dy, _sunk(sg), _sunk(sb), None, None, None, None
        return dy, s2, s1, None, None, None, None


def bn_act_rows(h: torch.Tensor, bn: torch.nn.modules.batchnorm._BatchNorm, relu: bool, drop_p: float,
                training: bool) -> torch.Tensor:
    _need_cuda(h, "bn_act_rows")
    if isinstance(bn, torch.nn.SyncBatchNorm):
        raise NotImplementedError("torch SyncBatchNorm modules are not executed by this package: keep the BatchNorm "
                                  "modules and switch synchronisation on with ops.set_bn_sync(True) / "
                                  "TrainStep(sync_bn=True) (DESIGN.md section 7)")
    c = h.shape[-1]
    if not (bn.affine and bn_channels_ok(c)):
        raise NotImplementedError(f"BatchNorm over {c} channels without affine parameters is not on the CoDA path")
    p = float(drop_p) if training else 0.0
    if bn.training or bn.running_mean is None:
        return _BNActRows.apply(h, bn.weight, bn.bias, bn, bool(relu), p, _next_salt() if p > 0.0 else 0)
    scale = bn.weight * torch.rsqrt(bn.running_var + bn.eps)
    out = h * scale + (bn.bias - bn.running_mean * scale)
    return torch.relu(out) if relu else out


def softmax_rows(x: torch.Tensor, log: bool = False) -> torch.Tensor:
    _need_cuda(x, "softmax_rows")
    xc = _f32c(x.detach())
    c = xc.shape[-1]
    y = torch.empty_like(xc)
    with torch.cuda.device(x.device):
        st = lib().coda_softmax_rows(_ll(xc.numel() // c), _i(c), _i(1 if log else 0), ptr(xc), ptr(y), stream_of(x))
    check(st, "softmax_rows")
    return y


@torch.no_grad()
def fourier_pos_embed(xyz: torch.Tensor, gauss_B: torch.Tensor, d_out: int, input_range=None) -> torch.Tensor:
    _need_cuda(xyz, "fourier_pos_embed")
    xc = _f32c(xyz)
    gb = _f32c(gauss_B)
    b, n, _ = xc.shape
    out = torch.empty((b, 2 * d_out, n), dtype=torch.float32, device=xyz.device)
    rmin = rmax = None
    if input_range is not None:
        rmin, rmax = _f32c(input_range[0]), _f32c(input_range[1])
    with torch.cuda.device(xyz.device):
        st = lib().coda_fourier_pos_embed(_i(b), _i(n), _i(d_out), _i(gb.shape[1]), _i(0 if rmin is None else 1),
                                          ptr(xc), ptr(rmin), ptr(rmax), ptr(gb), ptr(out), stream_of(xyz))
    check(st, "fourier_pos_embed")
    return out


@torch.no_grad()
def giou3d(corners1: torch.Tensor, corners2: torch.Tensor, nums_k2: torch.Tensor, rotated,
           rot_k2_limit: int | None = None) -> torch.Tensor:
    _need_cuda(corners1, "giou3d")
    c1, c2 = _f32c(corners1), _f32c(corners2)
    b, k1, k2 = c1.shape[0], c1.shape[1], c2.shape[1]
    nk = nums_k2.to(device=c1.device, dtype=torch.int32).contiguous()
    out = torch.empty((b, k1, k2), dtype=torch.float32, device=c1.device)
    lim = k2 if rot_k2_limit is None else int(rot_k2_limit)
    rdev = None
    if isinstance(rotated, torch.Tensor):
        rdev = rotated.to(device=c1.device, dtype=torch.int32).reshape(1).contiguous()
        rotated = False
    with torch.cuda.device(c1.device):
        st = lib().coda_giou3d(_i(b), _i(k1), _i(k2), _i(1 if rotated else 0), ptr(rdev), _i(lim), ptr(c1), ptr(c2),
                               ptr(nk), ptr(out), stream_of(c1))
    check(st, "giou3d")
    return out


@torch.no_grad()
def hungarian(cost: torch.Tensor, nactual: torch.Tensor):
    _need_cuda(cost, "hungarian")
    cc = _f32c(cost)
    b, nprop, ngt = cc.shape
    na = nactual.to(device=cc.device, dtype=torch.int32).contiguous()
    inds = torch.empty((b, nprop), dtype=torch.int64, device=cc.device)
    mask = torch.empty((b, nprop), dtype=torch.float32, device=cc.device)
    with torch.cuda.device(cc.device):
        st = lib().coda_hungarian(_i(b), _i(nprop), _i(ngt), ptr(cc), ptr(na), ptr(inds), ptr(mask), stream_of(cc))
    check(st, "hungarian")
    return inds, mask


CAMERAS = {"sunrgbd": 0, "scannet": 1}
_CAMERA_DIM = {"sunrgbd": 3, "scannet": 4}


@torch.no_grad()
def boxes_in_image(corners_xyz: torch.Tensor, size_unnorm: torch.Tensor, inputs: dict, camera: str = "sunrgbd",
                   extent: bool = False):
    if camera not in CAMERAS:
        raise ValueError(f"boxes_in_image: unknown camera {camera!r} (expected one of {sorted(CAMERAS)})")
    b, q = corners_xyz.shape[:2]
    n = _CAMERA_DIM[camera]
    kshape, tshape = tuple(inputs["K"].shape), tuple(inputs["Rtilt"].shape)
    if kshape != (b, n, n) or tshape != (b, n, n):
        raise ValueError(f"boxes_in_image: the {camera} camera needs K and Rtilt of shape ({b}, {n}, {n}); "
                         f"got K {kshape} and Rtilt {tshape}")
    _need_cuda(corners_xyz, "boxes_in_image")
    dev = corners_xyz.device
    f64 = lambda t, shape: t.to(device=dev, dtype=torch.double).reshape(shape).contiguous()
    i64 = lambda t: t.to(device=dev, dtype=torch.int64).reshape(b).contiguous()
    scale = f64(inputs["scale_array"], (b, 3))
    rot, K, Rtilt = f64(inputs["rot_array"], (b, 9)), f64(inputs["K"], (b, n * n)), f64(inputs["Rtilt"], (b, n * n))
    flip, img_flip = f64(inputs["flip_array"], (b,)), f64(inputs["image_flip_array"], (b,))
    flip_len = f64(inputs["flip_length"], (b,))
    zx = f64(inputs["zx_flip_array"], (b,)) if "zx_flip_array" in inputs else None
    boxes = torch.empty((b, q, 4), dtype=torch.int32, device=dev)
    valid = torch.empty((b, q), dtype=torch.uint8, device=dev)
    ext = torch.empty((b, q, 4), dtype=torch.double, device=dev) if extent else None
    cx, su = _f32c(corners_xyz), _f32c(size_unnorm)
    ow, oh, xo, yo = (i64(inputs[k]) for k in ("ori_width", "ori_height", "x_offset", "y_offset"))
    with torch.cuda.device(dev):
        st = lib().coda_boxes_in_image(_i(b), _i(q), _i(CAMERAS[camera]), ptr(cx), ptr(su), ptr(scale), ptr(rot),
                                       ptr(flip), ptr(zx), ptr(K), ptr(Rtilt), ptr(ow), ptr(oh), ptr(xo), ptr(yo),
                                       ptr(img_flip), ptr(flip_len), ptr(boxes), ptr(valid), ptr(ext),
                                       stream_of(corners_xyz))
    check(st, "boxes_in_image")
    return (boxes, valid.bool(), ext) if extent else (boxes, valid.bool())


@torch.no_grad()
def novel_candidates(boxes2d: torch.Tensor, valid: torch.Tensor, objectness: torch.Tensor, pred_corners: torch.Tensor,
                     gt_corners: torch.Tensor, gt_present: torch.Tensor, nms_iou: float, gt_iou: float,
                     min_objectness: float, cap: int):
    _need_cuda(boxes2d, "novel_candidates")
    b, q, _ = boxes2d.shape
    g = gt_corners.shape[1]
    bx = boxes2d.to(torch.int32).contiguous()
    vd = valid.to(torch.uint8).contiguous()
    cand = torch.empty((b, cap), dtype=torch.int32, device=bx.device)
    count = torch.empty((b, 2), dtype=torch.int32, device=bx.device)
    ob, pc, gc, gp = _f32c(objectness), _f32c(pred_corners), _f32c(gt_corners), _f32c(gt_present)
    with torch.cuda.device(bx.device):
        st = lib().coda_novel_candidates(_i(b), _i(q), _i(g), _i(cap), ptr(bx), ptr(vd), ptr(ob), ptr(pc), ptr(gc),
                                         ptr(gp), _f(nms_iou), _f(gt_iou), _f(min_objectness), ptr(cand), ptr(count),
                                         stream_of(bx))
    check(st, "novel_candidates")
    return cand, count


def attention(q: torch.Tensor, k: torch.Tensor, v: torch.Tensor, nhead: int, dropout_p: float = 0.0,
              training: bool = False, causal: bool = False, mask=None) -> torch.Tensor:
    _need_cuda(q, "attention")
    from . import attention_sm100

    return attention_sm100.attention(q, k, v, nhead, dropout_p, training, causal, mask)


def attention_mask_bits(mask: torch.Tensor, batch: int):
    _need_cuda(mask, "attention_mask_bits")
    from . import attention_launch

    return attention_launch.mask_bits(mask, batch)


def radius_mask_bits(xyz: torch.Tensor, radius: float):
    _need_cuda(xyz, "radius_mask_bits")
    from . import attention_launch

    return attention_launch.radius_mask_bits(xyz, radius)


def attention_fused(a: torch.Tensor, b, layout: str, nhead: int, dropout_p: float = 0.0, training: bool = False,
                    mask=None) -> torch.Tensor:
    _need_cuda(a, "attention")
    from . import attention_sm100

    return attention_sm100.attention_fused(a, b, layout, nhead, dropout_p, training, mask)


CLIP_MEAN = (0.48145466, 0.4578275, 0.40821073)
CLIP_STD = (0.26862954, 0.26130258, 0.27577711)


@torch.no_grad()
def crop_resize_normalize(images: torch.Tensor, scene: torch.Tensor, boxes: torch.Tensor, valid: torch.Tensor,
                          res: int, dtype=torch.float16, mean=CLIP_MEAN, std=CLIP_STD, patch: int = 0,
                          tile_rows: int = 0) -> torch.Tensor:
    _need_cuda(images, "crop_resize_normalize")
    if images.dtype != torch.uint8:
        raise RuntimeError("images must be uint8 (HWC)")
    img = images.contiguous()
    nimg, h, w, _ = img.shape
    n = boxes.shape[0]
    sc = scene.to(torch.int32).contiguous()
    bx = boxes.to(torch.int32).contiguous()
    vd = valid.to(torch.uint8).contiguous()
    if dtype not in (torch.float16, torch.float32):
        raise RuntimeError("output dtype must be float16 or float32")
    if patch > 0:
        assert res % patch == 0
        out = torch.empty((n, res // patch, res // patch, 3, patch, patch), dtype=dtype, device=img.device)
    else:
        out = torch.empty((n, 3, res, res), dtype=dtype, device=img.device)
    work = torch.empty(nimg * h * w, dtype=torch.int32, device=img.device)
    m = (ctypes.c_float * 3)(*mean)
    s = (ctypes.c_float * 3)(*std)
    with torch.cuda.device(img.device):
        st = lib().coda_crop_resize_normalize_ex(_i(nimg), _i(h), _i(w), _i(n), _i(res), ptr(img), ptr(sc), ptr(bx),
                                                 ptr(vd), m, s, _i(1 if dtype == torch.float16 else 0), _i(patch),
                                                 _i(tile_rows), ptr(work), ptr(out), stream_of(img))
    check(st, "crop_resize_normalize")
    return out


@torch.no_grad()
def clip_classify(feats: torch.Tensor, text: torch.Tensor, scale: torch.Tensor, row_map: torch.Tensor,
                  shape) -> tuple:
    _need_cuda(text, "clip_classify")
    for name, t in (("feats", feats), ("scale", scale), ("row_map", row_map)):
        if t.device != text.device:
            raise ValueError(f"clip_classify: {name} is on {t.device}, the text features on {text.device}")
    fc, tc, sc = _f32c(feats), _f32c(text), _f32c(scale.reshape(1))
    rm = row_map.to(torch.int32).contiguous()
    c, d = tc.shape
    if fc.shape[1:] != (d,):
        raise ValueError(f"clip_classify: features of width {tuple(fc.shape[1:])} against text of width {d}")
    prob = torch.empty((*shape, c), dtype=torch.float32, device=tc.device)
    logits = torch.empty_like(prob)
    if prob.numel() // c != rm.numel():
        raise ValueError(f"clip_classify: {rm.numel()} row-map entries for output rows {tuple(shape)}")
    with torch.cuda.device(tc.device):
        st = lib().coda_clip_classify(_ll(rm.numel()), _i(fc.shape[0]), _i(c), _i(d), ptr(fc), ptr(tc), ptr(sc),
                                      ptr(rm), ptr(prob), ptr(logits), stream_of(tc))
    check(st, "clip_classify")
    return prob, logits


DEFAULT_NSPLIT = 3


def _pad64(k: int) -> int:
    return (k + 63) // 64 * 64


def pack_split(x: torch.Tensor, rows: int, k: int, row_stride: int, k_stride: int, nsplit: int = DEFAULT_NSPLIT,
               scale: float = 1.0, batch: int = 1, batch_stride: int = 0) -> torch.Tensor:
    _need_cuda(x, "pack_split")
    assert x.dtype == torch.float32
    kpad = _pad64(k)
    out = torch.empty((nsplit, batch, rows, kpad), dtype=torch.bfloat16, device=x.device)
    base = x.data_ptr()
    with torch.cuda.device(x.device):
        for b in range(batch):
            st = lib().coda_pack_split_bf16_strided(
                _ll(rows), _i(k), _i(kpad), _ll(row_stride), _ll(k_stride),
                ctypes.c_void_p(base + 4 * b * batch_stride), _f(scale), _i(nsplit),
                ctypes.c_void_p(out.data_ptr() + 2 * b * rows * kpad), _ll(batch * rows * kpad), stream_of(x))
            check(st, "pack_split_bf16")
    return out


def gemm_nt(a_planes: torch.Tensor, b_planes: torch.Tensor, m: int, n: int, bias=None, relu: bool = False,
            out: torch.Tensor | None = None, act: int | None = None, out_dtype=torch.float32,
            residual: torch.Tensor | None = None) -> torch.Tensor:
    _need_cuda(a_planes, "gemm_nt")
    nsplit, batch, _, kpad = a_planes.shape
    assert b_planes.shape[0] == nsplit and b_planes.shape[3] == kpad and a_planes.dtype == b_planes.dtype
    is_fp16 = a_planes.dtype == torch.float16
    bb = b_planes.shape[1]
    assert bb in (1, batch)
    if out is None:
        out = torch.empty((batch, m, n), dtype=out_dtype, device=a_planes.device)
    if act is None:
        act = 1 if relu else 0
    if residual is not None:
        assert residual.dtype == torch.float16 and residual.shape == (m, n) and residual.stride(1) == 1
    with torch.cuda.device(a_planes.device):
        st = lib().coda_gemm_nt_res(
            _i(nsplit), _i(1 if is_fp16 else 0), _i(batch), _i(m), _i(n), _i(kpad), ptr(a_planes),
            _ll(a_planes.stride(0)), _ll(a_planes.stride(1)), ptr(b_planes), _ll(b_planes.stride(0)),
            _ll(b_planes.stride(1) if bb > 1 else 0), ptr(bias), _i(act), _i(1 if out.dtype == torch.float16 else 0),
            ptr(residual), _ll(residual.stride(0) if residual is not None else 0),
            ptr(out), _ll(out.stride(1)), _ll(out.stride(0)), stream_of(a_planes))
    check(st, "gemm_nt")
    return out


A32_PLAIN, A32_AFFINE_RELU, A32_BN_BWD, A32_BN_BWD_POOLED = 0, 1, 2, 3
A32_BN_BWD_POOLED_PRE = 4


def a32_ok(a: torch.Tensor) -> bool:
    return (a.dim() == 2 and a.dtype == torch.float32 and a.is_cuda and a.stride(1) == 1 and a.stride(0) % 4 == 0
            and a.stride(0) >= a.shape[1] and a.data_ptr() % 16 == 0 and a.shape[1] >= 1)


def gemm_a32(a: torch.Tensor, b_planes: torch.Tensor, n: int, *, mode: int = A32_PLAIN, scale=None, shift=None,
             alpha=None, beta=None, a2=None, argmax=None, group: int = 0, b_mn: bool = False, bias=None,
             relu: bool = False, out: torch.Tensor | None = None, want_stats: bool = False, nsplit: int | None = None):
    _need_cuda(a, "gemm_a32")
    m, k = a.shape
    ns = b_planes.shape[0] if nsplit is None else nsplit
    assert a32_ok(a) and 2 <= ns <= b_planes.shape[0] and b_planes.dtype == torch.bfloat16
    ld = b_planes.shape[3]
    if out is None:
        out = torch.empty((m, n), dtype=torch.float32, device=a.device)
    L = lib()
    stats = None
    if want_stats:
        stats = torch.zeros((int(L.coda_gemm_a32_grid(_i(m), _i(n))), 2, n), dtype=torch.float32, device=a.device)
    lda2 = 0
    if mode == A32_BN_BWD:
        assert a32_ok(a2) and a2.shape == a.shape
        lda2 = a2.stride(0)
    elif mode in (A32_BN_BWD_POOLED, A32_BN_BWD_POOLED_PRE):
        assert a2.is_contiguous() and argmax.is_contiguous() and a2.shape == (m // group, k)
    with torch.cuda.device(a.device):
        st = L.coda_gemm_a32(_i(ns), _i(m), _i(n), _i(k), ptr(a), _ll(a.stride(0)), _i(mode), ptr(scale), ptr(shift),
                             ptr(alpha), ptr(beta), ptr(a2), _ll(lda2), ptr(argmax), _i(group), ptr(b_planes),
                             _ll(b_planes.stride(0)), _i(ld), _i(1 if b_mn else 0), ptr(bias), _i(1 if relu else 0),
                             ptr(out), _ll(out.stride(0)), ptr(stats), stream_of(a))
    check(st, "gemm_a32")
    return (out, stats) if want_stats else out


def tn32_ok(a: torch.Tensor) -> bool:
    return a32_ok(a) and a.shape[1] % 4 == 0


def gemm_tn32(a: torch.Tensor, b: torch.Tensor, *, a_mode: int = A32_PLAIN, a_scale=None, a_shift=None, a_alpha=None,
              a_beta=None, a2=None, argmax=None, group: int = 0, b_mode: int = A32_PLAIN, b_scale=None,
              b_shift=None, out: torch.Tensor | None = None, colsum_out: torch.Tensor | None = None) -> torch.Tensor:
    _need_cuda(a, "gemm_tn32")
    rows, m = a.shape
    n = b.shape[1]
    assert tn32_ok(a) and tn32_ok(b) and b.shape[0] == rows
    if out is None:
        out = torch.empty((m, n), dtype=torch.float32, device=a.device)
    assert out.shape == (m, n) and out.stride(1) == 1 and out.stride(0) % 4 == 0 and out.data_ptr() % 16 == 0
    lda2 = 0
    if a_mode == A32_BN_BWD:
        assert a32_ok(a2) and a2.shape == a.shape
        lda2 = a2.stride(0)
    elif a_mode in (A32_BN_BWD_POOLED, A32_BN_BWD_POOLED_PRE):
        assert a2.is_contiguous() and argmax.is_contiguous() and a2.shape == (rows // group, m)
    with torch.cuda.device(a.device):
        st = lib().coda_gemm_tn32(_ll(rows), _i(m), _i(n), ptr(a), _ll(a.stride(0)), _i(a_mode), ptr(a_scale),
                                  ptr(a_shift), ptr(a_alpha), ptr(a_beta), ptr(a2), _ll(lda2), ptr(argmax), _i(group),
                                  ptr(b), _ll(b.stride(0)), _i(b_mode), ptr(b_scale), ptr(b_shift), ptr(out),
                                  _ll(out.stride(0)), ptr(colsum_out), stream_of(a))
    check(st, "gemm_tn32")
    return out


def gemm_tn(a_planes: torch.Tensor, b_planes: torch.Tensor, m: int, n: int) -> torch.Tensor:
    _need_cuda(a_planes, "gemm_tn")
    nsplit, _, mc, lda = a_planes.shape
    assert b_planes.shape[0] == nsplit and b_planes.shape[2] == mc
    ldb = b_planes.shape[3]
    out = torch.empty((m, n), dtype=torch.float32, device=a_planes.device)
    with torch.cuda.device(a_planes.device):
        st = lib().coda_gemm_tn(_i(nsplit), _i(mc), _i(m), _i(n), ptr(a_planes), _ll(a_planes.stride(0)), _i(lda),
                                ptr(b_planes), _ll(b_planes.stride(0)), _i(ldb), ptr(out), _ll(n), stream_of(a_planes))
    check(st, "gemm_tn")
    return out


BACKWARD_NSPLIT = 2
USE_TN_WGRAD = True


_WEIGHT_EPOCH = 0
_WEIGHT_CACHE: dict = {}
_PACK_LOG: list | None = None
_PACK_JOIN = None


def record_weight_packs(on: bool):
    global _PACK_LOG
    if on:
        _PACK_LOG = []
        return None
    log, _PACK_LOG = _PACK_LOG, None
    return log


def prepack_weights(requests, side_stream) -> None:
    global _PACK_JOIN
    with torch.cuda.stream(side_stream):
        for w, transposed, nsplit in requests:
            _packed_weight(w, transposed, nsplit)
    _PACK_JOIN = side_stream


_ACT_CACHE: dict = {}


def invalidate_weight_cache() -> None:
    global _WEIGHT_EPOCH
    _WEIGHT_EPOCH += 1
    _WEIGHT_CACHE.clear()
    _ACT_CACHE.clear()


def _packed_rows(x: torch.Tensor, nsplit: int) -> torch.Tensor:
    key = (x.data_ptr(), tuple(x.shape), x.stride(0), x._version, nsplit)
    hit = _ACT_CACHE.get(key)
    if hit is None:
        planes = pack_split(x, x.shape[0], x.shape[1], x.stride(0), 1, nsplit)
        if len(_ACT_CACHE) > 64:
            _ACT_CACHE.clear()
        _ACT_CACHE[key] = (planes, x)
        return planes
    return hit[0]


def _packed_weight(w: torch.Tensor, transposed: bool, nsplit: int) -> torch.Tensor:
    global _PACK_JOIN
    if _PACK_JOIN is not None and torch.cuda.current_stream(w.device) != _PACK_JOIN:
        torch.cuda.current_stream(w.device).wait_stream(_PACK_JOIN)
        _PACK_JOIN = None
    key = (w.data_ptr(), tuple(w.shape), w._version, _WEIGHT_EPOCH, transposed, nsplit)
    hit = _WEIGHT_CACHE.get(key)
    if hit is None:
        if _PACK_LOG is not None:
            _PACK_LOG.append((w.detach(), transposed, nsplit))
        n, k = w.shape
        wd = w.detach()
        planes = pack_split(wd, k, n, 1, k, nsplit) if transposed else pack_split(wd, n, k, k, 1, nsplit)
        if len(_WEIGHT_CACHE) > 512:
            _WEIGHT_CACHE.clear()
        hit = _WEIGHT_CACHE[key] = (planes, wd)
    return hit[0]


def colsum(x: torch.Tensor, out: torch.Tensor | None = None) -> torch.Tensor:
    rows, c = x.shape
    if not (x.is_cuda and x.dtype == torch.float32 and x.is_contiguous() and rows > 0
            and 4 <= c <= 1024 and c % 4 == 0 and 256 % (c // 4) == 0):
        if out is None:
            return x.sum(dim=0)
        return torch.sum(x, dim=0, out=out)
    if out is None:
        out = torch.empty(c, dtype=torch.float32, device=x.device)
    scratch = torch.empty(132 * 4 * 2 * c, dtype=torch.float32, device=x.device)
    with torch.cuda.device(x.device):
        st = lib().coda_rows_colsum(_ll(rows), _i(c), ptr(x), ptr(out), ptr(scratch), stream_of(x))
    check(st, "rows_colsum")
    return out


class _Linear(torch.autograd.Function):

    @staticmethod
    def forward(ctx, x, weight, bias, relu, nsplit):
        m, k = x.shape
        n = weight.shape[0]
        wp = _packed_weight(weight, False, nsplit)
        if not a32_ok(x):
            x = x.contiguous()
        if a32_ok(x) and n % 4 == 0:
            y = gemm_a32(x, wp, n, bias=bias, relu=relu)
        else:
            y = gemm_nt(_packed_rows(x, nsplit), wp, m, n, bias=bias, relu=relu)[0]
        ctx.save_for_backward(x, weight, y if relu else None, bias)
        ctx.has_bias, ctx.relu, ctx.nsplit = bias is not None, relu, nsplit
        return y

    @staticmethod
    def backward(ctx, dy):
        x, weight, y, bias = ctx.saved_tensors
        nsplit = min(ctx.nsplit, BACKWARD_NSPLIT)
        dy = dy.contiguous()
        m, k = x.shape
        n = weight.shape[0]
        dx = dw = db = None
        want_db = ctx.has_bias and ctx.needs_input_grad[2]
        pro = None
        if ctx.relu:
            if (a32_ok(dy) and a32_ok(y) and tn32_ok(dy) and tn32_ok(x) and k % 4 == 0 and nsplit == 2
                    and ctx.needs_input_grad[1]):
                one, zero = _unit_vectors(n, dy.device)
                pro = dict(scale=one, shift=zero, alpha=zero, beta=zero)
            else:
                dy = dy * (y > 0).to(dy.dtype)
        if pro is not None:
            if ctx.needs_input_grad[0]:
                dx = gemm_a32(y, _packed_weight(weight, False, ctx.nsplit), k, mode=A32_BN_BWD, a2=dy, b_mn=True,
                              nsplit=nsplit, **pro)
            sw, sb = _sink(weight), None
            if want_db:
                sb = _sink(bias)
                db = torch.empty(n, dtype=torch.float32, device=dy.device) if sb is None else sb
            dw = gemm_tn32(y, x, a_mode=A32_BN_BWD, a2=dy, a_scale=one, a_shift=zero, a_alpha=zero, a_beta=zero,
                           out=sw, colsum_out=db)
            if sw is not None:
                dw = _sunk(sw)
            if sb is not None:
                db = _sunk(sb)
            return dx, dw, db, None, None
        if ctx.needs_input_grad[0]:
            if a32_ok(dy) and k % 4 == 0:
                dx = gemm_a32(dy, _packed_weight(weight, False, ctx.nsplit), k, b_mn=True, nsplit=nsplit)
            else:
                dx = gemm_nt(pack_split(dy, m, n, n, 1, nsplit), _packed_weight(weight, True, nsplit), m, k)[0]
        if ctx.needs_input_grad[1]:
            if tn32_ok(dy) and tn32_ok(x) and nsplit == 2:
                sw = _sink(weight) if k % 4 == 0 else None
                sb = None
                if want_db:
                    sb = _sink(bias)
                    db = torch.empty(n, dtype=torch.float32, device=dy.device) if sb is None else sb
                dw = gemm_tn32(dy, x, out=sw, colsum_out=db)
                if sw is not None:
                    dw = _sunk(sw)
                if sb is not None:
                    db = _sunk(sb)
                want_db = False
            else:
                dya = pack_split(dy, m, n, n, 1, nsplit)
                xa = _packed_rows(x, nsplit)
                dw = gemm_tn(dya, xa, n, k)
        if want_db:
            sb = _sink(bias)
            db = colsum(dy, out=sb)
            if sb is not None:
                db = _sunk(sb)
        return dx, dw, db, None, None


_UNIT: dict = {}


def _unit_vectors(n: int, device):
    key = ((n + 127) // 128 * 128, device)
    hit = _UNIT.get(key)
    if hit is None:
        hit = _UNIT[key] = (torch.ones(key[0], dtype=torch.float32, device=device),
                            torch.zeros(key[0], dtype=torch.float32, device=device))
    return hit


_BIAS32: dict = {}


def _bias_fp32(bias):
    key = (bias.data_ptr(), tuple(bias.shape), bias._version)
    hit = _BIAS32.get(key)
    if hit is None:
        if len(_BIAS32) > 256:
            _BIAS32.clear()
        hit = _BIAS32[key] = (bias.detach().float(), bias)
    return hit[0]


def linear(x: torch.Tensor, weight: torch.Tensor, bias=None, relu: bool = False, nsplit: int | None = None,
           quick_gelu: bool = False, residual: torch.Tensor | None = None):
    _need_cuda(x, "linear")
    lead = x.shape[:-1]
    k = x.shape[-1]
    n = weight.shape[0]
    x2 = x.reshape(-1, k)
    if x2.dtype == torch.float16:
        assert weight.dtype == torch.float16 and k % 64 == 0, "fp16 path needs fp16 weights and K % 64 == 0"
        x2 = x2.contiguous()
        res2 = None
        if residual is not None:
            res2 = residual.reshape(-1, n)
            if res2.dtype != torch.float16 or res2.stride(1) != 1 or res2.stride(0) % 8 != 0 or n % 8 != 0:
                res2 = None
        y = gemm_nt(x2.view(1, 1, x2.shape[0], k), weight.detach().contiguous().view(1, 1, n, k), x2.shape[0], n,
                    bias=None if bias is None else _bias_fp32(bias), act=2 if quick_gelu else (1 if relu else 0),
                    out_dtype=torch.float16, residual=res2)[0]
        y = y.reshape(*lead, n)
        return y + residual if (residual is not None and res2 is None) else y
    if residual is not None:
        raise NotImplementedError("fused residual exists on the fp16 inference path only")
    if x2.stride(-1) != 1:
        x2 = x2.contiguous()
    w2 = weight.reshape(n, -1)
    y = _Linear.apply(x2.float(), w2, bias, relu, DEFAULT_NSPLIT if nsplit is None else nsplit)
    return y.reshape(*lead, n)


class Linear(torch.nn.Linear):

    def forward(self, x):
        return linear(x, self.weight, self.bias)


class _TextCE(torch.autograd.Function):
    @staticmethod
    def forward(ctx, s, e, label, w, scale, c):
        rows, ld = s.shape
        d = e.shape[1]
        loss = torch.empty(rows, dtype=torch.float32, device=s.device)
        lse, inv = torch.empty_like(loss), torch.empty_like(loss)
        with torch.cuda.device(s.device):
            check(lib().coda_text_ce_fwd(_ll(rows), _i(c), _i(ld), _i(d), ptr(s), ptr(e), ptr(label), ptr(w),
                                         ptr(scale), ptr(loss), ptr(lse), ptr(inv), stream_of(s)), "text_ce_fwd")
        ctx.save_for_backward(s, e, label, w, scale, lse, inv)
        ctx.c = c
        return loss

    @staticmethod
    def backward(ctx, g):
        s, e, label, w, scale, lse, inv = ctx.saved_tensors
        rows, ld = s.shape
        d = e.shape[1]
        gc = _f32c(g)
        ds, dnorm = torch.empty_like(s), torch.empty_like(e)
        with torch.cuda.device(s.device):
            check(lib().coda_text_ce_bwd(_ll(rows), _i(ctx.c), _i(ld), _i(d), ptr(s), ptr(e), ptr(label), ptr(w),
                                         ptr(scale), ptr(lse), ptr(inv), ptr(gc), ptr(ds), ptr(dnorm), stream_of(s)),
                  "text_ce_bwd")
        return ds, dnorm, None, None, None, None


def text_ce_rows(s: torch.Tensor, e: torch.Tensor, label: torch.Tensor, w: torch.Tensor, scale: torch.Tensor,
                 c: int) -> torch.Tensor:
    _need_cuda(s, "text_ce_rows")
    assert s.dim() == 2 and e.dim() == 2 and s.shape[0] == e.shape[0] and s.shape[1] % 4 == 0 and 1 <= c <= s.shape[1]
    assert label.numel() == s.shape[0] and w.numel() == s.shape[0] and scale.numel() == 1
    assert not w.requires_grad and not scale.requires_grad
    return _TextCE.apply(_f32c(s), _f32c(e), label.to(torch.int64).contiguous(), _f32c(w).reshape(-1),
                         _f32c(scale.reshape(1)), c)


_PADDED_TEXT: dict = {}


def _rows_padded4(t: torch.Tensor) -> torch.Tensor:
    c = t.shape[0]
    if c % 4 == 0:
        return t
    key = (t.data_ptr(), tuple(t.shape), t.stride(), t._version)
    hit = _PADDED_TEXT.get(key)
    if hit is None:
        if len(_PADDED_TEXT) > 8:
            _PADDED_TEXT.clear()
        padded = torch.zeros(((c + 3) // 4 * 4, t.shape[1]), dtype=torch.float32, device=t.device)
        padded[:c].copy_(t.detach())
        hit = _PADDED_TEXT[key] = (padded, t)
    return hit[0]


def text_contrastive_ce(e: torch.Tensor, text: torch.Tensor, label: torch.Tensor, w: torch.Tensor,
                        scale: torch.Tensor) -> torch.Tensor:
    _need_cuda(e, "text_contrastive_ce")
    c = text.shape[0]
    s = linear(e, _rows_padded4(text.to(torch.float32)))
    return text_ce_rows(s, e, label, w, scale, c)

# ... 151 lines not shown
```

coda_neurips2023_b200/sa_mlp.py:

```python
from __future__ import annotations

import ctypes

import torch
import torch.nn as nn

from . import ops
from ._lib import check, lib, ptr, stream_of

_i, _ll, _f = ctypes.c_int, ctypes.c_longlong, ctypes.c_float
BACKWARD_PLANES = 2


def _channels_ok(c: int) -> bool:
    return 4 <= c <= 1024 and c % 4 == 0 and 256 % (c // 4) == 0


def applicable(x: torch.Tensor, blocks, group: int) -> bool:
    if not (x.is_cuda and x.dtype == torch.float32 and 1 <= group <= 256) or len(blocks) == 0:
        return False
    cin = x.shape[-1]
    if cin > 8 and cin % 64 != 0:
        return False
    if cin <= 8 and x.requires_grad and torch.is_grad_enabled():
        return False
    for li, (conv, bn) in enumerate(blocks):
        cout = conv.weight.shape[0]
        if conv.bias is not None or not bn.training or not bn.affine or not _channels_ok(cout):
            return False
        if li < len(blocks) - 1 and cout % 64 != 0:
            return False
        if cout > 256 and (li > 0 or cin > 8):
            return False
    return True


def _scratch(c: int, device) -> torch.Tensor:
    lib().coda_bn_rows_scratch_floats.restype = ctypes.c_longlong
    return torch.empty(int(lib().coda_bn_rows_scratch_floats(_i(c))), dtype=torch.float32, device=device)


def _stats(y: torch.Tensor, bn: nn.modules.batchnorm._BatchNorm):
    rows, c = y.shape
    momentum = 0.0 if bn.momentum is None else float(bn.momentum)
    track = bn.track_running_stats and bn.running_mean is not None
    if track and bn.num_batches_tracked is not None:
        bn.num_batches_tracked.add_(1)
        if bn.momentum is None:
            raise NotImplementedError("cumulative-average BatchNorm momentum is not on the CoDA path")
    mean = torch.empty(c, dtype=torch.float32, device=y.device)
    invstd = torch.empty(c, dtype=torch.float32, device=y.device)
    with torch.cuda.device(y.device):
        st = lib().coda_bn_rows_stats(_ll(rows), _i(c), ptr(y), _f(bn.eps), _f(momentum),
                                      ptr(bn.running_mean if track else None), ptr(bn.running_var if track else None),
                                      ptr(mean), ptr(invstd), ptr(_scratch(c, y.device)), stream_of(y))
    check(st, "bn_rows_stats")
    return mean, invstd


def _stats_affine(y: torch.Tensor, bn, gamma, beta):
    rows, c = y.shape
    momentum, track = _bn_bookkeeping(bn)
    dev = y.device
    if ops.bn_sync_world() > 1:
        return ops.bn_stats_synced(rows, c, bn, momentum, track, gamma, beta, True, y=y)
    cpad = ops._pad64(c)
    mean = torch.empty(c, dtype=torch.float32, device=dev)
    invstd = torch.empty(c, dtype=torch.float32, device=dev)
    scale = torch.empty(cpad, dtype=torch.float32, device=dev)
    shift = torch.empty(cpad, dtype=torch.float32, device=dev)
    with torch.cuda.device(dev):
        st = lib().coda_bn_rows_stats_affine(_ll(rows), _i(c), ptr(y), _f(bn.eps), _f(momentum),
                                             ptr(bn.running_mean if track else None),
                                             ptr(bn.running_var if track else None), ptr(gamma), ptr(beta), ptr(mean),
                                             ptr(invstd), ptr(scale), ptr(shift), ptr(_scratch(c, dev)), stream_of(y))
    check(st, "bn_rows_stats_affine")
    return mean, invstd, scale, shift


def _bn_bookkeeping(bn):
    momentum = 0.0 if bn.momentum is None else float(bn.momentum)
    track = bn.track_running_stats and bn.running_mean is not None
    if track and bn.num_batches_tracked is not None:
        bn.num_batches_tracked.add_(1)
        if bn.momentum is None:
            raise NotImplementedError("cumulative-average BatchNorm momentum is not on the CoDA path")
    return momentum, track


def _stats_from_partials(partials: torch.Tensor, rows: int, bn, gamma, beta, want_affine: bool):
    nblocks, _, c = partials.shape
    momentum, track = _bn_bookkeeping(bn)
    dev = partials.device
    if ops.bn_sync_world() > 1:
        return ops.bn_stats_synced(rows, c, bn, momentum, track, gamma, beta, want_affine, partials=partials)
    mean = torch.empty(c, dtype=torch.float32, device=dev)
    invstd = torch.empty(c, dtype=torch.float32, device=dev)
    scale = shift = None
    if want_affine:
        scale = torch.empty(ops._pad64(c), dtype=torch.float32, device=dev)
        shift = torch.empty(ops._pad64(c), dtype=torch.float32, device=dev)
    with torch.cuda.device(dev):
        st = lib().coda_bn_stats_finalize(_i(nblocks), _ll(rows), _i(c), ptr(partials), _f(bn.eps), _f(momentum),
                                          ptr(bn.running_mean if track else None),
                                          ptr(bn.running_var if track else None), ptr(gamma), ptr(beta), ptr(mean),
                                          ptr(invstd), ptr(scale), ptr(shift), stream_of(partials))
    check(st, "bn_stats_finalize")
    return mean, invstd, scale, shift


class _SharedMLPMax(torch.autograd.Function):

    @staticmethod
    def forward(ctx, x, group, nsplit, bns, *params):
        L = lib()
        nl = len(bns)
        rows, c0 = x.shape
        dev = x.device
        ys, means, invstds, scales, shifts = [], [], [], [], []
        small_k = c0 <= 8
        scale = shift = None
        with torch.cuda.device(dev):
            for li in range(nl):
                w, gamma, beta = params[3 * li: 3 * li + 3]
                cout, cin = w.shape
                last = li == nl - 1
                if li == 0 and small_k:
                    y = torch.empty((rows, cout), dtype=torch.float32, device=dev)
                    check(L.coda_rows_linear_small_k(_ll(rows), _i(cin), _i(cout), ptr(x), ptr(w.contiguous()), ptr(y),
                                                     stream_of(x)), "rows_linear_small_k")
                    mean, invstd, scale, shift = _stats_affine(y, bns[li], gamma, beta)
                else:
                    wp = ops._packed_weight(w, False, nsplit)
                    if li == 0:
                        y, part = ops.gemm_a32(x, wp, cout, want_stats=True)
                    else:
                        y, part = ops.gemm_a32(ys[-1], wp, cout, mode=ops.A32_AFFINE_RELU, scale=scale, shift=shift,
                                               want_stats=True)
                    mean, invstd, scale, shift = _stats_from_partials(part, rows, bns[li], gamma, beta, True)
                ys.append(y); means.append(mean); invstds.append(invstd); scales.append(scale); shifts.append(shift)
                if last:
                    groups = rows // group
                    pooled = torch.empty((groups, cout), dtype=torch.float32, device=dev)
                    argmax = torch.empty((groups, cout), dtype=torch.uint8, device=dev)
                    check(L.coda_bn_relu_maxpool_rows(_ll(groups), _i(group), _i(cout), ptr(y), ptr(mean), ptr(invstd),
                                                      ptr(gamma), ptr(beta), ptr(pooled), ptr(argmax), stream_of(x)),
                          "bn_relu_maxpool_rows")
        ctx.nl, ctx.group, ctx.small_k, ctx.nsplit = nl, group, small_k, nsplit
        ctx.sync = ops.bn_sync_world() > 1
        ctx.save_for_backward(x, argmax, *ys, *means, *invstds, *scales, *shifts, *params)
        ctx.mark_non_differentiable(argmax)
        return pooled, argmax

    @staticmethod
    def backward(ctx, dpooled, _dargmax):
        L = lib()
        nl, group = ctx.nl, ctx.group
        saved = ctx.saved_tensors
        x, argmax = saved[0], saved[1]
        ys = saved[2: 2 + nl]
        means = saved[2 + nl: 2 + 2 * nl]
        invstds = saved[2 + 2 * nl: 2 + 3 * nl]
        scales = saved[2 + 3 * nl: 2 + 4 * nl]
        shifts = saved[2 + 4 * nl: 2 + 5 * nl]
        params = saved[2 + 5 * nl:]
        rows = x.shape[0]
        dev = x.device
        ns = BACKWARD_PLANES
        grads = [None] * (3 * nl)
        dx = None
        dz = None
        dpooled = dpooled.contiguous()
        with torch.cuda.device(dev):
            for li in range(nl - 1, -1, -1):
                w, gamma, beta = params[3 * li: 3 * li + 3]
                cout, cin = w.shape
                y, mean, invstd = ys[li], means[li], invstds[li]
                sg, sb = ops._sink(gamma), ops._sink(beta)
                if sg is None or sb is None:
                    sg = sb = None
                s1 = torch.empty(cout, dtype=torch.float32, device=dev) if sb is None else sb
                s2 = torch.empty(cout, dtype=torch.float32, device=dev) if sg is None else sg
                scratch = _scratch(cout, dev)
                pooled_form = li == nl - 1
                if pooled_form:
                    dprime = torch.empty_like(dpooled)
                    check(L.coda_bn_relu_bwd_reduce_pooled(_ll(rows // group), _i(group), _i(cout), ptr(y), ptr(dpooled),
                                                           ptr(argmax), ptr(mean), ptr(invstd), ptr(gamma), ptr(beta),
                                                           ptr(s1), ptr(s2), ptr(scratch), ptr(dprime), stream_of(x)),
                          "bn_relu_bwd_reduce_pooled")
                else:
                    check(L.coda_bn_relu_bwd_reduce(_ll(rows), _i(cout), ptr(y), ptr(dz), ptr(mean), ptr(invstd),
                                                    ptr(gamma), ptr(beta), ptr(s1), ptr(s2), ptr(scratch), stream_of(x)),
                          "bn_relu_bwd_reduce")
                loc1, loc2 = s1, s2
                if ctx.sync:
                    s1, s2 = ops.bn_sync_backward_sums(s1, s2)
                if sg is None:
                    grads[3 * li + 1], grads[3 * li + 2] = loc2, loc1
                else:
                    ops._sunk(sg), ops._sunk(sb)
                sw = ops._sink(w)
                if li == 0 and ctx.small_k:
                    if nl == 1:
                        dz = torch.zeros((rows // group, group, cout), dtype=torch.float32, device=dev)
                        dz.scatter_(1, argmax.long().unsqueeze(1), dpooled.unsqueeze(1))
                        dz = dz.view(rows, cout)
                    L.coda_bn_rows_small_k_scratch_floats.restype = ctypes.c_longlong
                    sc = torch.empty(int(L.coda_bn_rows_small_k_scratch_floats(_i(cin), _i(cout))), dtype=torch.float32,
                                     device=dev)
                    dw = torch.empty((cout, cin), dtype=torch.float32, device=dev) if sw is None else sw
                    check(L.coda_bn_relu_bwd_small_k(_ll(rows), _i(cin), _i(cout), ptr(y), ptr(dz), ptr(mean), ptr(invstd),
                                                     ptr(gamma), ptr(beta), ptr(s1), ptr(s2), ptr(x), ptr(dw), ptr(sc),
                                                     stream_of(x)), "bn_relu_bwd_small_k")
                    grads[0] = dw if sw is None else ops._sunk(sw)
                    break
                if sw is not None and cin % 4 != 0:
                    sw = None
                cpad = ops._pad64(cout)
                alpha = torch.empty(cpad, dtype=torch.float32, device=dev)
                bcoef = torch.empty(cpad, dtype=torch.float32, device=dev)
                check(L.coda_bn_bwd_coefs(_i(cout), _ll(rows), ptr(mean), ptr(invstd), ptr(gamma), ptr(s1), ptr(s2),
                                          ptr(alpha), ptr(bcoef), stream_of(x)), "bn_bwd_coefs")
                pro = dict(a_scale=scales[li], a_shift=shifts[li], a_alpha=alpha, a_beta=bcoef)
                if pooled_form and group % 32 == 0 and (128 % group == 0 or group % 128 == 0) and cout % 128 == 0:
                    mode, a2 = ops.A32_BN_BWD_POOLED_PRE, dprime
                    extra = dict(argmax=argmax, group=group)
                elif pooled_form:
                    dz = torch.zeros((rows // group, group, cout), dtype=torch.float32, device=dev)
                    dz.scatter_(1, argmax.long().unsqueeze(1), dpooled.unsqueeze(1))
                    dz = dz.view(rows, cout)
                    mode, a2, extra = ops.A32_BN_BWD, dz, {}
                else:
                    mode, a2, extra = ops.A32_BN_BWD, dz, {}
                if li > 0:
                    grads[3 * li] = ops.gemm_tn32(y, ys[li - 1], a_mode=mode, a2=a2, b_mode=ops.A32_AFFINE_RELU,
                                                  b_scale=scales[li - 1], b_shift=shifts[li - 1], out=sw, **pro, **extra)
                else:
                    grads[3 * li] = ops.gemm_tn32(y, x, a_mode=mode, a2=a2, out=sw, **pro, **extra)
                if sw is not None:
                    grads[3 * li] = ops._sunk(sw)
                if li > 0 or ctx.needs_input_grad[0]:
                    dz_new = ops.gemm_a32(y, ops._packed_weight(w, False, ctx.nsplit), cin, mode=mode, scale=scales[li],
                                          shift=shifts[li], alpha=alpha, beta=bcoef, a2=a2, b_mn=True, nsplit=ns,
                                          **extra)
                    dz = dz_new
                    if li == 0:
                        dx = dz
        return (dx, None, None, None, *grads)


def shared_mlp_max(x_rows: torch.Tensor, blocks, group: int, nsplit: int | None = None) -> torch.Tensor:
    params = []
    for conv, bn in blocks:
        params += [conv.weight.reshape(conv.weight.shape[0], -1), bn.weight, bn.bias]
    pooled, _ = _SharedMLPMax.apply(x_rows.contiguous(), int(group), ops.DEFAULT_NSPLIT if nsplit is None else nsplit,
                                    [bn for _, bn in blocks], *params)
    return pooled


INFER_WIDTHS = (64, 128, 256)
INFER_GROUP = 64
INFER_PLANES = 3


def infer_applicable(x: torch.Tensor, blocks, group: int) -> bool:
    if not (x.is_cuda and x.dtype == torch.float32 and x.dim() == 4 and group == INFER_GROUP
            and x.shape[3] == group and x.shape[1] in (3, 6) and len(blocks) == len(INFER_WIDTHS)):
        return False
    if x.stride(3) != 1:
        return False
    params = [t for conv, bn in blocks for t in (conv.weight, bn.weight, bn.bias)]
    if torch.is_grad_enabled() and (x.requires_grad or any(p is not None and p.requires_grad for p in params)):
        return False
    cin = x.shape[1]
    for (conv, bn), cout in zip(blocks, INFER_WIDTHS):
        if conv.bias is not None or tuple(conv.weight.shape) != (cout, cin, 1, 1):
            return False
        if bn.training or not bn.affine or bn.running_mean is None or bn.running_var is None:
            return False
        if any(t.dtype != torch.float32 or t.device != x.device
               for t in (conv.weight, bn.weight, bn.bias, bn.running_mean, bn.running_var)):
            return False
        cin = cout
    return True


def _folded_affine(blocks) -> torch.Tensor:
    parts = []
    with torch.no_grad():
        for _, bn in blocks:
            scale = bn.weight * torch.rsqrt(bn.running_var + bn.eps)
            parts += [scale, bn.bias - bn.running_mean * scale]
        return torch.cat(parts)


def shared_mlp_max_infer(x: torch.Tensor, blocks, group: int) -> torch.Tensor:
    b, c0, npoint, nsample = x.shape
    (conv1, _), (conv2, _), (conv3, _) = blocks
    w1 = conv1.weight.detach().reshape(INFER_WIDTHS[0], c0).contiguous()
    w2 = ops._packed_weight(conv2.weight.reshape(INFER_WIDTHS[1], -1), False, INFER_PLANES)
    w3 = ops._packed_weight(conv3.weight.reshape(INFER_WIDTHS[2], -1), False, INFER_PLANES)
    affine = _folded_affine(blocks)
    out = torch.empty((b * npoint, INFER_WIDTHS[2]), dtype=torch.float32, device=x.device)
    with torch.cuda.device(x.device):
        st = lib().coda_sa_mlp_max_infer(_ll(b), _i(c0), _i(npoint), _i(nsample), ptr(x), _ll(x.stride(0)),
                                         _ll(x.stride(1)), _ll(x.stride(2)), ptr(w1), ptr(w2), _ll(w2.stride(0)),
                                         ptr(w3), _ll(w3.stride(0)), ptr(affine), ptr(out), _ll(out.stride(0)),
                                         stream_of(x))
    check(st, "sa_mlp_max_infer")
    return out
```

include/coda_gemm.h:

```cpp
#ifndef CODA_GEMM_H
#define CODA_GEMM_H

#ifdef __cplusplus
extern "C" {
#endif

int coda_pack_split_bf16(long long rows, int k, int kpad, long long src_row_stride,
                         long long src_k_stride, const float *src, float scale, int nsplit,
                         void *planes, void *stream);

int coda_pack_split_bf16_strided(long long rows, int k, int kpad, long long src_row_stride,
                                 long long src_k_stride, const float *src, float scale, int nsplit,
                                 void *planes, long long plane_stride, void *stream);

int coda_gemm_nt(int nsplit, int is_fp16, int batch, int m, int n, int kpad, const void *a,
                 long long a_plane_stride, long long a_batch_stride, const void *b,
                 long long b_plane_stride, long long b_batch_stride, const float *bias, int relu,
                 float *c, long long ldc, long long c_batch_stride, void *stream);

int coda_gemm_nt_ex(int nsplit, int is_fp16, int batch, int m, int n, int kpad, const void *a,
                    long long a_plane_stride, long long a_batch_stride, const void *b,
                    long long b_plane_stride, long long b_batch_stride, const float *bias, int act,
                    int out_half, void *c, long long ldc, long long c_batch_stride, void *stream);

int coda_gemm_nt_res(int nsplit, int is_fp16, int batch, int m, int n, int kpad, const void *a,
                     long long a_plane_stride, long long a_batch_stride, const void *b,
                     long long b_plane_stride, long long b_batch_stride, const float *bias, int act,
                     int out_half, const void *residual, long long ldr, void *c, long long ldc,
                     long long c_batch_stride, void *stream);

int coda_gemm_tn(int nsplit, int mc, int m, int n, const void *a, long long a_plane_stride, int lda,
                 const void *b, long long b_plane_stride, int ldb, float *c, long long ldc, void *stream);

#define CODA_A32_PLAIN 0
#define CODA_A32_AFFINE_RELU 1
#define CODA_A32_BN_BWD 2
#define CODA_A32_BN_BWD_POOLED 3
#define CODA_A32_BN_BWD_POOLED_PRE 4
int coda_gemm_a32_grid(int m, int n);
int coda_gemm_a32(int nsplit, int m, int n, int k, const float *a, long long lda, int a_mode, const float *a_scale,
                  const float *a_shift, const float *a_alpha, const float *a_beta, const float *a2, long long lda2,
                  const unsigned char *a_argmax, int a_group, const void *b_planes, long long b_plane_stride,
                  int b_ld, int b_mn, const float *bias, int act, float *c, long long ldc, float *col_stats,
                  void *stream);

int coda_gemm_tn32(long long rows, int m, int n, const float *a, long long lda, int a_mode, const float *a_scale,
                   const float *a_shift, const float *a_alpha, const float *a_beta, const float *a2, long long lda2,
                   const unsigned char *a_argmax, int a_group, const float *b, long long ldb, int b_mode,
                   const float *b_scale, const float *b_shift, float *c, long long ldc, float *a_colsum, void *stream);

#ifdef __cplusplus
}
#endif
#endif
```

include/coda_sa_mlp.h:

```cpp
#ifndef CODA_SA_MLP_H
#define CODA_SA_MLP_H

#ifdef __cplusplus
extern "C" {
#endif

long long coda_bn_rows_scratch_floats(int c);

int coda_rows_linear_small_k(long long rows, int cin, int cout, const float *x, const float *w, float *y,
                             void *stream);

int coda_bn_rows_stats(long long rows, int c, const float *y, float eps, float momentum, float *running_mean,
                       float *running_var, float *mean, float *invstd, float *scratch, void *stream);

int coda_bn_rows_stats_affine(long long rows, int c, const float *y, float eps, float momentum, float *running_mean,
                               float *running_var, const float *gamma, const float *beta, float *mean, float *invstd,
                               float *scale, float *shift, float *scratch, void *stream);

int coda_bn_stats_finalize(int nblocks, long long rows, int c, const float *partial, float eps, float momentum,
                           float *running_mean, float *running_var, const float *gamma, const float *beta,
                           float *mean, float *invstd, float *scale, float *shift, void *stream);
int coda_bn_rows_sums(long long rows, int c, const float *y, double *sums, float *scratch, void *stream);
int coda_bn_partials_sums(int nblocks, int c, const float *partial, double *sums, void *stream);
int coda_bn_stats_finalize_sums(long long rows, int c, const double *sums, float eps, float momentum,
                                float *running_mean, float *running_var, const float *gamma, const float *beta,
                                float *mean, float *invstd, float *scale, float *shift, void *stream);

int coda_bn_bwd_coefs(int c, long long rows, const float *mean, const float *invstd, const float *gamma,
                      const float *s1, const float *s2, float *alpha, float *beta, void *stream);

int coda_rows_colsum(long long rows, int c, const float *x, float *out, float *scratch, void *stream);

int coda_bn_relu_pack_rows(long long rows, int c, int nsplit, const float *y, const float *mean,
                           const float *invstd, const float *gamma, const float *beta, void *planes,
                           void *stream);

int coda_bn_relu_maxpool_rows(long long groups, int group, int c, const float *y, const float *mean,
                              const float *invstd, const float *gamma, const float *beta, float *pooled,
                              unsigned char *argmax, void *stream);

int coda_bn_relu_bwd_reduce(long long rows, int c, const float *y, const float *dz, const float *mean,
                            const float *invstd, const float *gamma, const float *beta, float *s1, float *s2,
                            float *scratch, void *stream);
int coda_bn_relu_bwd_reduce_pooled(long long groups, int group, int c, const float *y, const float *dpooled,
                                   const unsigned char *argmax, const float *mean, const float *invstd,
                                   const float *gamma, const float *beta, float *s1, float *s2, float *scratch,
                                   float *dprime, void *stream);

int coda_bn_relu_bwd_pack(long long rows, int c, int nsplit, const float *y, const float *dz,
                          const float *dpooled, const unsigned char *argmax, int group, const float *mean,
                          const float *invstd, const float *gamma, const float *beta, const float *s1,
                          const float *s2, void *planes, void *stream);

long long coda_bn_rows_small_k_scratch_floats(int cin, int cout);
int coda_bn_relu_bwd_small_k(long long rows, int cin, int cout, const float *y, const float *dz, const float *mean,
                             const float *invstd, const float *gamma, const float *beta, const float *s1,
                             const float *s2, const float *x, float *dw, float *scratch, void *stream);

int coda_sa_mlp_max_infer(long long batch, int c0, int npoint, int nsample, const float *x, long long x_batch_stride,
                          long long x_channel_stride, long long x_point_stride, const float *w1, const void *w2_planes,
                          long long w2_plane_stride, const void *w3_planes, long long w3_plane_stride,
                          const float *affine, float *out, long long ldo, void *stream);

#ifdef __cplusplus
}
#endif
#endif
```

Before: 199.1.

## Recompute small-K first layer inside GEMM prologues instead of storing its output

Adds a SMALLK_AFFINE_RELU mode in which the first SA-MLP layer (cin ≤ 8) is not materialized. Each GEMM consumer instead recomputes it on the fly from the raw xyz/features and the layer weights, which are staged in shared memory. BN statistics, the backward reduce and the small-k weight-gradient kernels get matching 'first' variants. This removes the write and re-read of the wide first-layer activation in forward and backward, at the cost of redundant FMAs and more kernel template variants.

Measured after the change: 201.8, median of 6. 1.4% higher.

```diff
diff --git a/coda_neurips2023_b200/csrc/a32_prologue.cuh b/coda_neurips2023_b200/csrc/a32_prologue.cuh
--- a/coda_neurips2023_b200/csrc/a32_prologue.cuh
+++ b/coda_neurips2023_b200/csrc/a32_prologue.cuh
@@ -2,6 +2,14 @@
 
 namespace coda {
 namespace a32 {
+
+__device__ __forceinline__ float first_layer(const float *x, const float *w, int cin) {
+  float a = x[0] * w[0];
+#pragma unroll
+  for (int k = 1; k < 8; ++k)
+    if (k < cin) a = fmaf(x[k], w[k], a);
+  return a;
+}
 
 __device__ __forceinline__ float affine_relu(float x, float s, float h) { return fmaxf(fmaf(x, s, h), 0.f); }
 
diff --git a/coda_neurips2023_b200/csrc/gemm_a32_sm90.cu b/coda_neurips2023_b200/csrc/gemm_a32_sm90.cu
--- a/coda_neurips2023_b200/csrc/gemm_a32_sm90.cu
+++ b/coda_neurips2023_b200/csrc/gemm_a32_sm90.cu
@@ -1,6 +1,8 @@
 #include "../../include/coda_gemm.h"
 #include "a32_prologue.cuh"
 #include "sm90_primitives.cuh"
+
+#include <string.h>
 
 #include <type_traits>
 
@@ -36,6 +38,9 @@
   float *stats;
   int b_resident;
 };
+__device__ __forceinline__ const float *smallk_x0(const A32Params &P) { return P.dpooled; }
+__device__ __forceinline__ const float *smallk_w0(const A32Params &P) { return P.alpha; }
+__device__ __forceinline__ int smallk_cin(const A32Params &P) { return P.group; }
 
 struct Alternation {
   int wg;
@@ -52,7 +57,7 @@
   }
 };
 
-template <int NSPLIT, int BN, int RAW_KB, int B_STAGES, bool B_MN>
+template <int NSPLIT, int BN, int RAW_KB, int B_STAGES, bool B_MN, bool SMALLK>
 __global__ void __launch_bounds__(A32_THREADS, 1)
 gemm_a32_kernel(const __grid_constant__ A32Maps maps, const A32Params P) {
   constexpr int MAX_RAW = RAW_KB / 32;
@@ -68,6 +73,8 @@
   const uint32_t nraw = (uint32_t)((RAW_KB * 1024) / raw_stage_bytes);
   unsigned char *b_ring = smem + (size_t)RAW_KB * 1024;
   float *s_stats = reinterpret_cast<float *>(b_ring + (size_t)B_STAGES * B_STAGE);
+  float *s_w0 = s_stats + (P.stats ? 16 * P.n : 0);
+  constexpr bool small_k = SMALLK;
   __shared__ __align__(8) uint64_t raw_full[MAX_RAW], raw_empty[MAX_RAW];
   __shared__ __align__(8) uint64_t b_full[B_STAGES], b_empty[B_STAGES];
 
@@ -101,11 +108,18 @@
     float *mine = s_stats + (size_t)warp * 2 * n;
     for (int i = lane; i < 2 * n; i += 32) mine[i] = 0.f;
   }
+  if (small_k && warp < 8) {
+    const int cin = smallk_cin(P);
+    for (int i = threadIdx.x; i < 64 * cin; i += 256) {
+      const int q = i >> 6, j = i & 63;
+      s_w0[i] = j < P.k ? __ldg(smallk_w0(P) + j * cin + q) : 0.f;
+    }
+  }
   __syncthreads();
 
   if (warp == 8) {
     if (lane == 0) {
-      prefetch_tmap(&maps.a);
+      if (!small_k) prefetch_tmap(&maps.a);
       if (two_in) prefetch_tmap(&maps.a2);
 #pragma unroll
       for (int p = 0; p < NSPLIT; ++p) prefetch_tmap(&maps.b[p]);
@@ -136,9 +150,19 @@
         const int rs = it % nraw, bs = it % B_STAGES;
         mbar_wait(&raw_empty[rs], ((it / nraw) & 1u) ^ 1u);
         if (!P.b_resident) mbar_wait(&b_empty[bs], ((it / B_STAGES) & 1u) ^ 1u);
+        const bool x_whole = small_k && m0 + BM <= m;
+        const uint32_t x_bytes = small_k ? (uint32_t)(BM * smallk_cin(P) * 4) : 0u;
+        if (small_k && !x_whole) {
+          float *dst = reinterpret_cast<float *>(raw_ring + (size_t)rs * raw_stage_bytes);
+          const float *src = smallk_x0(P) + (size_t)m0 * smallk_cin(P);
+          const int have = (m - m0) * smallk_cin(P);
+          for (int i = lane; i < BM * smallk_cin(P); i += 32) dst[i] = i < have ? __ldg(src + i) : 0.f;
+          __syncwarp();
+        }
         if (elect_one_sync()) {
           unsigned char *rt = raw_ring + (size_t)rs * raw_stage_bytes;
-          mbar_arrive_expect_tx(&raw_full[rs], (uint32_t)(RAW_TILE * (two_in ? 2 : 1) + tile_groups * 320));
+          mbar_arrive_expect_tx(&raw_full[rs], small_k ? (x_whole ? x_bytes : 0u)
+                                                       : (uint32_t)(RAW_TILE * (two_in ? 2 : 1) + tile_groups * 320));
           if (pooled) {
             const long long ngroups = P.m / P.group;
             for (int gt = 0; gt < tile_groups; ++gt) {
@@ -148,8 +172,12 @@
               bulk_load_1d(rt + RAW_TILE + gt * 320 + 256, P.argmax + g * P.k + kb * BK, 64, &raw_full[rs]);
             }
           }
-          tma_load_3d(rt, &maps.a, &raw_full[rs], kb * BK, m0, 0);
-          tma_load_3d(rt + RAW_TILE / 2, &maps.a, &raw_full[rs], kb * BK + 32, m0, 0);
+          if (x_whole) {
+            bulk_load_1d(rt, smallk_x0(P) + (size_t)m0 * smallk_cin(P), x_bytes, &raw_full[rs]);
+          } else if (!small_k) {
+            tma_load_3d(rt, &maps.a, &raw_full[rs], kb * BK, m0, 0);
+            tma_load_3d(rt + RAW_TILE / 2, &maps.a, &raw_full[rs], kb * BK + 32, m0, 0);
+          }
           if (two_in) {
             tma_load_3d(rt + RAW_TILE, &maps.a2, &raw_full[rs], kb * BK, m0, 0);
             tma_load_3d(rt + RAW_TILE + RAW_TILE / 2, &maps.a2, &raw_full[rs], kb * BK + 32, m0, 0);
@@ -212,6 +240,46 @@
                 x.y = a32::affine_relu(x.y, s2.y, h2.y);
                 put(i, x);
               }
+            } else if (small_k) {
+              const float2 s2 = ld2(P.scale), h2 = ld2(P.shift);
+              auto pair = [&](int cin) {
+                float wa[8], wb[8];
+#pragma unroll
+                for (int q = 0; q < 8; ++q) {
+                  if (q < cin) {
+                    const float2 w2 = *reinterpret_cast<const float2 *>(s_w0 + q * 64 + kc);
+                    wa[q] = w2.x;
+                    wb[q] = w2.y;
+                  }
+                }
+#pragma unroll
+                for (int i = 0; i < 2; ++i) {
+                  const float *xs = reinterpret_cast<const float *>(rt) + rloc[i] * cin;
+                  float xr[8];
+#pragma unroll
+                  for (int q = 0; q < 8; ++q)
+                    if (q < cin) xr[q] = xs[q];
+                  put(i, make_float2(a32::affine_relu(a32::first_layer(xr, wa, cin), s2.x, h2.x),
+                                     a32::affine_relu(a32::first_layer(xr, wb, cin), s2.y, h2.y)));
+                }
+              };
+              if (smallk_cin(P) == 3) {
+                pair(3);
+              } else {
+                const int cin = smallk_cin(P);
+                const float *xs = reinterpret_cast<const float *>(rt);
+#pragma unroll
+                for (int i = 0; i < 2; ++i) {
+                  float y[2];
+#pragma unroll
+                  for (int j = 0; j < 2; ++j) {
+                    float acc = xs[rloc[i] * cin] * s_w0[kc + j];
+                    for (int q = 1; q < cin; ++q) acc = fmaf(xs[rloc[i] * cin + q], s_w0[q * 64 + kc + j], acc);
+                    y[j] = acc;
+                  }
+                  put(i, make_float2(a32::affine_relu(y[0], s2.x, h2.x), a32::affine_relu(y[1], s2.y, h2.y)));
+                }
+              }
             } else if (mode == CODA_A32_BN_BWD) {
               const float2 s2 = ld2(P.scale), h2 = ld2(P.shift), a2 = ld2(P.alpha), b2 = ld2(P.beta);
 #pragma unroll
@@ -255,7 +323,9 @@
           }
         }
       };
-      switch (P.mode) {
+      if constexpr (SMALLK) {
+        convert(std::integral_constant<int, CODA_A32_SMALLK_AFFINE_RELU>{});
+      } else switch (P.mode) {
         case CODA_A32_PLAIN: convert(std::integral_constant<int, CODA_A32_PLAIN>{}); break;
         case CODA_A32_AFFINE_RELU: convert(std::integral_constant<int, CODA_A32_AFFINE_RELU>{}); break;
         default: convert(std::integral_constant<int, -1>{}); break;
@@ -356,15 +426,15 @@
   }
 }
 
-template <int NSPLIT, int BN, int RAW_KB, int B_STAGES, bool B_MN>
+template <int NSPLIT, int BN, int RAW_KB, int B_STAGES, bool B_MN, bool SMALLK = false>
 int launch_a32(const A32Maps &maps, const A32Params &P, cudaStream_t s) {
   static_assert(RAW_KB % 64 == 0 || RAW_KB == 96, "raw region");
   constexpr size_t smem = (size_t)RAW_KB * 1024 + (size_t)B_STAGES * NSPLIT * BN * BK * 2 + 1024;
-  const size_t total = smem + (P.stats ? (size_t)16 * P.n * 4 : 0);
+  const size_t total = smem + (P.stats ? (size_t)16 * P.n * 4 : 0) + (SMALLK ? (size_t)64 * 8 * 4 : 0);
   constexpr size_t SMEM_MAX = 227 * 1024 - 2048;
   if (total > SMEM_MAX) return CODA_ETOOLARGE;
   if (P.mode == CODA_A32_BN_BWD && RAW_KB < 64) return CODA_EINVAL;
-  constexpr auto kern = gemm_a32_kernel<NSPLIT, BN, RAW_KB, B_STAGES, B_MN>;
+  constexpr auto kern = gemm_a32_kernel<NSPLIT, BN, RAW_KB, B_STAGES, B_MN, SMALLK>;
   if (const int st = raise_smem_limit<kern>((int)SMEM_MAX)) return st;
   const int tiles_m = (P.m + BM - 1) / BM, tiles_n = (P.n + BN - 1) / BN;
   const long long nwork = (long long)tiles_m * tiles_n;
@@ -390,14 +460,18 @@
                   const float *a_shift, const float *a_alpha, const float *a_beta, const float *a2, long long lda2,
                   const unsigned char *a_argmax, int a_group, const void *b_planes, long long b_plane_stride,
                   int b_ld, int b_mn, const float *bias, int act, float *c, long long ldc, float *col_stats,
-                  void *stream) {
+                  const float *x0, const float *w0, int cin, void *stream) {
   if (nsplit < 2 || nsplit > 3 || m < 0 || n < 0 || k <= 0) return CODA_EINVAL;
   if (m == 0 || n == 0) return CODA_OK;
-  if (!a || !b_planes || !c || b_ld % 64 != 0 || (lda & 3) || (ldc & 3) || ((uintptr_t)a & 15) || ((uintptr_t)c & 15))
-    return CODA_EINVAL;
-  if (a_mode < CODA_A32_PLAIN || a_mode > CODA_A32_BN_BWD_POOLED_PRE) return CODA_EINVAL;
+  const bool small_k = a_mode == CODA_A32_SMALLK_AFFINE_RELU;
+  if (small_k ? a != nullptr : (!a || (lda & 3) || ((uintptr_t)a & 15))) return CODA_EINVAL;
+  if (!b_planes || !c || b_ld % 64 != 0 || (ldc & 3) || ((uintptr_t)c & 15)) return CODA_EINVAL;
+  if (a_mode < CODA_A32_PLAIN || a_mode > CODA_A32_SMALLK_AFFINE_RELU) return CODA_EINVAL;
   if (a_mode != CODA_A32_PLAIN && (!a_scale || !a_shift || (k & 3))) return CODA_EINVAL;
-  if (a_mode >= CODA_A32_BN_BWD && (!a2 || !a_alpha || !a_beta || ((uintptr_t)a2 & 15))) return CODA_EINVAL;
+  const bool bwd = a_mode == CODA_A32_BN_BWD || a_mode == CODA_A32_BN_BWD_POOLED || a_mode == CODA_A32_BN_BWD_POOLED_PRE;
+  if (bwd && (!a2 || !a_alpha || !a_beta || ((uintptr_t)a2 & 15))) return CODA_EINVAL;
+  if (small_k != (x0 != nullptr) || small_k != (w0 != nullptr)) return CODA_EINVAL;
+  if (small_k && (cin < 1 || cin > 8 || ((uintptr_t)x0 & 15) || k > 64 || b_mn)) return CODA_EINVAL;
   if (a_mode == CODA_A32_BN_BWD && (lda2 & 3)) return CODA_EINVAL;
   if ((a_mode == CODA_A32_BN_BWD_POOLED || a_mode == CODA_A32_BN_BWD_POOLED_PRE) &&
       (!a_argmax || a_group < 32 || a_group > 256 || m % a_group != 0 || k % 64 != 0 ||
@@ -406,7 +480,8 @@
   const long long tiles128 = (long long)((m + BM - 1) / BM) * ((n + 127) / 128);
   const int bn = (n <= 64 || tiles128 <= sm_count() / 2) ? 64 : 128;
   A32Maps maps;
-  int st = make_tmap_f32_box(&maps.a, a, k, m, lda, 32, BM);
+  memset(&maps, 0, sizeof(maps));
+  int st = small_k ? CODA_OK : make_tmap_f32_box(&maps.a, a, k, m, lda, 32, BM);
   if (st != CODA_OK) return st;
   maps.a2 = maps.a;
   if (a_mode == CODA_A32_BN_BWD) {
@@ -429,17 +504,19 @@
   A32Params P;
   P.m = m; P.n = n; P.k = k; P.mode = a_mode; P.scale = a_scale; P.shift = a_shift; P.alpha = a_alpha; P.beta = a_beta;
   P.dpooled = a2; P.argmax = a_argmax; P.group = a_group; P.bias = bias; P.act = act; P.c = c; P.ldc = ldc; P.stats = col_stats;
+  if (small_k) { P.dpooled = x0; P.alpha = w0; P.group = cin; }
   P.b_resident = 0;
   cudaStream_t s = (cudaStream_t)stream;
-#define CODA_A32(NS, BN_, RS, BS)                                                   \
-  return b_mn ? launch_a32<NS, BN_, RS, BS, true>(maps, P, s) : launch_a32<NS, BN_, RS, BS, false>(maps, P, s)
+#define CODA_A32(NS, BN_, RS, BS)                                                                           \
+  return small_k ? launch_a32<NS, BN_, RS, BS, false, true>(maps, P, s)                                    \
+                 : b_mn ? launch_a32<NS, BN_, RS, BS, true>(maps, P, s) : launch_a32<NS, BN_, RS, BS, false>(maps, P, s)
   const bool deep_b = !col_stats && k > 128 && a_mode != CODA_A32_BN_BWD;
   if (nsplit == 2) {
     if (bn == 64) CODA_A32(2, 64, 128, 4);
     CODA_A32(2, 128, 128, 2);
   }
   if (bn == 64) CODA_A32(3, 64, 128, 3);
-  if (deep_b) CODA_A32(3, 128, 64, 3);
+  if (deep_b) return b_mn ? launch_a32<3, 128, 64, 3, true>(maps, P, s) : launch_a32<3, 128, 64, 3, false>(maps, P, s);
   CODA_A32(3, 128, 96, 2);
 #undef CODA_A32
 }
diff --git a/coda_neurips2023_b200/csrc/gemm_tn32_sm90.cu b/coda_neurips2023_b200/csrc/gemm_tn32_sm90.cu
--- a/coda_neurips2023_b200/csrc/gemm_tn32_sm90.cu
+++ b/coda_neurips2023_b200/csrc/gemm_tn32_sm90.cu
@@ -1,6 +1,8 @@
 #include "../../include/coda_gemm.h"
 #include "a32_prologue.cuh"
 #include "sm90_primitives.cuh"
+
+#include <string.h>
 
 using namespace coda;
 
@@ -31,9 +33,11 @@
   float *c;
   long long ldc;
   int ksplit;
+  const float *x0, *w0;
+  int cin;
 };
 
-template <int BN>
+template <int BN, bool SMALLK_B>
 __global__ void __launch_bounds__(TN32_THREADS, 1)
 gemm_tn32_kernel(const __grid_constant__ TN32Maps maps, const TN32Params P) {
   constexpr int RAW_A = BKR * BM * 4;
@@ -49,6 +53,7 @@
   unsigned char *pl_ring = smem + (size_t)RAW_STAGES * RAW_STAGE;
   __shared__ __align__(8) uint64_t raw_full[RAW_STAGES], raw_empty[RAW_STAGES];
   __shared__ __align__(16) float s_colsum[TW][BM];
+  __shared__ __align__(16) float s_w0[SMALLK_B ? 64 * 8 : 1];
 
   const int warp = threadIdx.x >> 5, lane = threadIdx.x & 31;
   const int tiles_n = (P.n + BN - 1) / BN;
@@ -59,29 +64,43 @@
   const long long kb0 = (long long)ks * per;
   const long long nkb = max(0ll, min(per, nkb_total - kb0));
   const bool two_in = P.a_mode == CODA_A32_BN_BWD;
+  constexpr bool small_k = SMALLK_B;
 
   if (threadIdx.x == 0) {
     for (int s = 0; s < RAW_STAGES; ++s) { mbar_init(&raw_full[s], 1); mbar_init(&raw_empty[s], TW); }
     mbar_fence_init_cluster();
   }
+  if (small_k)
+    for (int i = threadIdx.x; i < 64 * P.cin; i += TN32_THREADS) {
+      const int q = i >> 6, j = i & 63;
+      s_w0[i] = j < P.n ? __ldg(P.w0 + j * P.cin + q) : 0.f;
+    }
   __syncthreads();
 
   if (warp == 8) {
     if (lane == 0) {
       prefetch_tmap(&maps.a);
-      prefetch_tmap(&maps.b);
+      if (!small_k) prefetch_tmap(&maps.b);
       if (two_in) prefetch_tmap(&maps.a2);
     }
     const bool pooled = P.a_mode == CODA_A32_BN_BWD_POOLED || P.a_mode == CODA_A32_BN_BWD_POOLED_PRE;
-    const uint32_t bytes = (uint32_t)(RAW_A * (two_in ? 2 : 1) + RAW_B + (pooled ? 640 : 0));
+    const uint32_t bytes = (uint32_t)(RAW_A * (two_in ? 2 : 1) + (small_k ? 0 : RAW_B) + (pooled ? 640 : 0));
+    const uint32_t x_bytes = (uint32_t)(BKR * P.cin * 4);
     const long long ngroups = pooled ? P.rows / P.group : 0;
     for (long long i = 0; i < nkb; ++i) {
       const int rs = (int)(i % RAW_STAGES);
       mbar_wait(&raw_empty[rs], (uint32_t)((i / RAW_STAGES) & 1) ^ 1u);
+      unsigned char *st = raw_ring + (size_t)rs * RAW_STAGE;
+      const int r0 = (int)((kb0 + i) * BKR);
+      const bool x_whole = small_k && (long long)r0 + BKR <= P.rows;
+      if (small_k && !x_whole) {
+        float *dst = reinterpret_cast<float *>(st + 2 * RAW_A);
+        const long long have = (P.rows - r0) * P.cin;
+        for (int j = lane; j < BKR * P.cin; j += 32) dst[j] = j < have ? __ldg(P.x0 + (long long)r0 * P.cin + j) : 0.f;
+        __syncwarp();
+      }
       if (elect_one_sync()) {
-        unsigned char *st = raw_ring + (size_t)rs * RAW_STAGE;
-        const int r0 = (int)((kb0 + i) * BKR);
-        mbar_arrive_expect_tx(&raw_full[rs], bytes);
+        mbar_arrive_expect_tx(&raw_full[rs], bytes + (x_whole ? x_bytes : 0u));
         if (pooled) {
           long long g = (long long)r0 / P.group;
           if (g >= ngroups) g = ngroups - 1;
@@ -94,8 +113,13 @@
 #pragma unroll
           for (int g = 0; g < BM / 32; ++g) tma_load_3d(st + RAW_A + g * 4096, &maps.a2, &raw_full[rs], m0 + g * 32, r0, 0);
         }
-#pragma unroll
-        for (int g = 0; g < BN / 32; ++g) tma_load_3d(st + 2 * RAW_A + g * 4096, &maps.b, &raw_full[rs], n0 + g * 32, r0, 0);
+        if (x_whole) {
+          bulk_load_1d(st + 2 * RAW_A, P.x0 + (long long)r0 * P.cin, x_bytes, &raw_full[rs]);
+        } else if (!small_k) {
+#pragma unroll
+          for (int g = 0; g < BN / 32; ++g)
+            tma_load_3d(st + 2 * RAW_A + g * 4096, &maps.b, &raw_full[rs], n0 + g * 32, r0, 0);
+        }
       }
       __syncwarp();
     }
@@ -118,7 +142,7 @@
   const int bch = lane % B_CHUNKS, brow_off = lane / B_CHUNKS;
   const int cb = n0 + bch * 4;
   float4 sb = make_float4(0.f, 0.f, 0.f, 0.f), tb = sb;
-  if (P.b_mode == CODA_A32_AFFINE_RELU && cb < P.n) {
+  if ((P.b_mode == CODA_A32_AFFINE_RELU || small_k) && cb < P.n) {
     sb = __ldg(reinterpret_cast<const float4 *>(P.b_scale + cb));
     tb = __ldg(reinterpret_cast<const float4 *>(P.b_shift + cb));
   }
@@ -176,7 +200,29 @@
         const int r = (tw + j * TW) * B_RPP + brow_off;
         const long long grow = r0 + r;
         const uint32_t roff = (uint32_t)(bch >> 3) * 4096u + (uint32_t)r * 128u + (uint32_t)(((bch & 7) ^ (r & 7)) << 4);
-        float4 v = *reinterpret_cast<const float4 *>(raw + 2 * RAW_A + roff);
+        float4 v;
+        if (small_k) {
+          const float *xr = reinterpret_cast<const float *>(raw + 2 * RAW_A) + r * P.cin;
+          auto rebuild = [&](int cin) {
+            float w[4][8], xv[8];
+#pragma unroll
+            for (int q = 0; q < 8; ++q) {
+              if (q < cin) {
+                const float4 w4 = *reinterpret_cast<const float4 *>(s_w0 + q * 64 + bch * 4);
+                w[0][q] = w4.x; w[1][q] = w4.y; w[2][q] = w4.z; w[3][q] = w4.w;
+                xv[q] = xr[q];
+              }
+            }
+            v.x = a32::affine_relu(a32::first_layer(xv, w[0], cin), sb.x, tb.x);
+            v.y = a32::affine_relu(a32::first_layer(xv, w[1], cin), sb.y, tb.y);
+            v.z = a32::affine_relu(a32::first_layer(xv, w[2], cin), sb.z, tb.z);
+            v.w = a32::affine_relu(a32::first_layer(xv, w[3], cin), sb.w, tb.w);
+          };
+          if (P.cin == 3) rebuild(3);
+          else rebuild(P.cin);
+        } else {
+          v = *reinterpret_cast<const float4 *>(raw + 2 * RAW_A + roff);
+        }
         if (P.b_mode == CODA_A32_AFFINE_RELU) {
           v.x = a32::affine_relu(v.x, sb.x, tb.x); v.y = a32::affine_relu(v.y, sb.y, tb.y);
           v.z = a32::affine_relu(v.z, sb.z, tb.z); v.w = a32::affine_relu(v.w, sb.w, tb.w);
@@ -254,12 +300,12 @@
   a_colsum[col] = v;
 }
 
-template <int BN>
+template <int BN, bool SMALLK_B = false>
 int launch_tn32(const TN32Maps &maps, TN32Params P, float *c, long long ldc, cudaStream_t s) {
   constexpr size_t smem = (size_t)RAW_STAGES * (2 * BKR * BM * 4 + BKR * BN * 4 + 1024) +
                           (size_t)PL_STAGES * NS * (BKR * BM * 2 + BKR * BN * 2) + 1024;
   static_assert(smem <= 227 * 1024, "smem budget");
-  constexpr auto kern = gemm_tn32_kernel<BN>;
+  constexpr auto kern = gemm_tn32_kernel<BN, SMALLK_B>;
   if (const int st = raise_smem_limit<kern>((int)smem)) return st;
   const int num_sms = sm_count();
   const int tiles = ((P.m + BM - 1) / BM) * ((P.n + BN - 1) / BN);
@@ -293,21 +339,26 @@
 int coda_gemm_tn32(long long rows, int m, int n, const float *a, long long lda, int a_mode, const float *a_scale,
                    const float *a_shift, const float *a_alpha, const float *a_beta, const float *a2, long long lda2,
                    const unsigned char *a_argmax, int a_group, const float *b, long long ldb, int b_mode,
-                   const float *b_scale, const float *b_shift, float *c, long long ldc, float *a_colsum, void *stream) {
-  if (rows <= 0 || m <= 0 || n <= 0 || !a || !b || !c) return CODA_EINVAL;
+                   const float *b_scale, const float *b_shift, float *c, long long ldc, float *a_colsum,
+                   const float *x0, const float *w0, int cin, void *stream) {
+  const bool small_k = b_mode == CODA_A32_SMALLK_AFFINE_RELU;
+  if (rows <= 0 || m <= 0 || n <= 0 || !a || !c || (small_k ? b != nullptr : !b)) return CODA_EINVAL;
   if ((lda & 3) || (ldb & 3) || (ldc & 3) || (m & 3) || (n & 3)) return CODA_EINVAL;
   if (((uintptr_t)a | (uintptr_t)b | (uintptr_t)c) & 15) return CODA_EINVAL;
+  if (small_k != (x0 != nullptr) || small_k != (w0 != nullptr)) return CODA_EINVAL;
+  if (small_k && (cin < 1 || cin > 8 || n > 64 || ((uintptr_t)x0 & 15))) return CODA_EINVAL;
   if (a_mode != CODA_A32_PLAIN && a_mode != CODA_A32_BN_BWD && a_mode != CODA_A32_BN_BWD_POOLED &&
       a_mode != CODA_A32_BN_BWD_POOLED_PRE)
     return CODA_EINVAL;
-  if (b_mode != CODA_A32_PLAIN && b_mode != CODA_A32_AFFINE_RELU) return CODA_EINVAL;
+  if (b_mode != CODA_A32_PLAIN && b_mode != CODA_A32_AFFINE_RELU && !small_k) return CODA_EINVAL;
   if (a_mode != CODA_A32_PLAIN && (!a_scale || !a_shift || !a_alpha || !a_beta || !a2 || ((uintptr_t)a2 & 15))) return CODA_EINVAL;
   if (a_mode == CODA_A32_BN_BWD && (lda2 & 3)) return CODA_EINVAL;
   if ((a_mode == CODA_A32_BN_BWD_POOLED || a_mode == CODA_A32_BN_BWD_POOLED_PRE) &&
       (!a_argmax || a_group < 32 || a_group > 256 || a_group % 32 != 0 || rows % a_group != 0 || m % 128 != 0))
     return CODA_EINVAL;
-  if (b_mode == CODA_A32_AFFINE_RELU && (!b_scale || !b_shift)) return CODA_EINVAL;
+  if (b_mode != CODA_A32_PLAIN && (!b_scale || !b_shift)) return CODA_EINVAL;
   TN32Maps maps;
+  memset(&maps, 0, sizeof(maps));
   int st = make_tmap_f32_box(&maps.a, a, m, rows, lda, 32, BKR);
   if (st != CODA_OK) return st;
   maps.a2 = maps.a;
@@ -315,13 +366,17 @@
     st = make_tmap_f32_box(&maps.a2, a2, m, rows, lda2, 32, BKR);
     if (st != CODA_OK) return st;
   }
-  st = make_tmap_f32_box(&maps.b, b, n, rows, ldb, 32, BKR);
-  if (st != CODA_OK) return st;
+  if (!small_k) {
+    st = make_tmap_f32_box(&maps.b, b, n, rows, ldb, 32, BKR);
+    if (st != CODA_OK) return st;
+  }
   TN32Params P;
   P.rows = rows; P.m = m; P.n = n; P.a_mode = a_mode; P.b_mode = b_mode;
   P.a_scale = a_scale; P.a_shift = a_shift; P.a_alpha = a_alpha; P.a_beta = a_beta;
   P.dpooled = a2; P.argmax = a_argmax; P.group = a_group; P.b_scale = b_scale; P.b_shift = b_shift; P.a_colsum = a_colsum; P.partial = nullptr; P.c = c; P.ldc = ldc; P.ksplit = 1;
+  P.x0 = x0; P.w0 = w0; P.cin = cin;
   cudaStream_t s = (cudaStream_t)stream;
+  if (small_k) return launch_tn32<64, true>(maps, P, c, ldc, s);
   if (n <= 64) return launch_tn32<64>(maps, P, c, ldc, s);
   return launch_tn32<128>(maps, P, c, ldc, s);
 }
diff --git a/coda_neurips2023_b200/csrc/sa_mlp_kernels.cu b/coda_neurips2023_b200/csrc/sa_mlp_kernels.cu
--- a/coda_neurips2023_b200/csrc/sa_mlp_kernels.cu
+++ b/coda_neurips2023_b200/csrc/sa_mlp_kernels.cu
@@ -2,7 +2,10 @@
 #include <math.h>
 #include <stdint.h>
 
+#include <type_traits>
+
 #include "../../include/coda_sa_mlp.h"
+#include "a32_prologue.cuh"
 #include "coda_common.cuh"
 #include "operand_split.cuh"
 
@@ -58,39 +61,54 @@
   }
 }
 
+struct StoredRows {
+  static constexpr bool kRebuilt = false;
+  const float4 *y;
+  int cq;
+  __device__ StoredRows(const float *y_, const float *, int c, int c4)
+      : y(reinterpret_cast<const float4 *>(y_) + c4), cq(c >> 2) {}
+  __device__ float4 operator()(long long r) const { return __ldg(y + r * cq); }
+};
+template <int CIN>
+struct FirstLayerRows {
+  static constexpr bool kRebuilt = true;
+  const float *x;
+  float w[4][CIN];
+  __device__ FirstLayerRows(const float *x_, const float *w0, int, int c4) : x(x_) {
+#pragma unroll
+    for (int j = 0; j < 4; ++j)
+#pragma unroll
+      for (int k = 0; k < CIN; ++k) w[j][k] = __ldg(w0 + (size_t)(c4 * 4 + j) * CIN + k);
+  }
+  __device__ float4 operator()(long long r) const {
+    float xv[CIN];
+#pragma unroll
+    for (int k = 0; k < CIN; ++k) xv[k] = __ldg(x + r * CIN + k);
+    return make_float4(coda::a32::first_layer(xv, w[0], CIN), coda::a32::first_layer(xv, w[1], CIN),
+                       coda::a32::first_layer(xv, w[2], CIN), coda::a32::first_layer(xv, w[3], CIN));
+  }
+};
+
 template <int CIN>
 __global__ void __launch_bounds__(THREADS)
 linear_small_k_kernel(long long rows, int cout, const float *__restrict__ x, const float *__restrict__ w,
                       float *__restrict__ y) {
   const int cq = cout >> 2, c4 = threadIdx.x % cq, slot = threadIdx.x / cq, nslots = THREADS / cq;
-  float wr[4][CIN];
-#pragma unroll
-  for (int j = 0; j < 4; ++j)
-#pragma unroll
-    for (int k = 0; k < CIN; ++k) wr[j][k] = __ldg(w + (size_t)(c4 * 4 + j) * CIN + k);
-  for (long long r = (long long)blockIdx.x * nslots + slot; r < rows; r += (long long)gridDim.x * nslots) {
-    float xv[CIN];
-#pragma unroll
-    for (int k = 0; k < CIN; ++k) xv[k] = __ldg(x + r * CIN + k);
-    float o[4];
-#pragma unroll
-    for (int j = 0; j < 4; ++j) {
-      float a = xv[0] * wr[j][0];
-#pragma unroll
-      for (int k = 1; k < CIN; ++k) a = fmaf(xv[k], wr[j][k], a);
-      o[j] = a;
-    }
-    reinterpret_cast<float4 *>(y + r * cout)[c4] = make_float4(o[0], o[1], o[2], o[3]);
-  }
-}
-
-__global__ void __launch_bounds__(THREADS)
-bn_stats_partial_kernel(long long rows, int c, const float *__restrict__ y, float *__restrict__ partial) {
+  const FirstLayerRows<CIN> in(x, w, cout, c4);
+  for (long long r = (long long)blockIdx.x * nslots + slot; r < rows; r += (long long)gridDim.x * nslots)
+    reinterpret_cast<float4 *>(y + r * cout)[c4] = in(r);
+}
+
+template <class Rows>
+__global__ void __launch_bounds__(THREADS)
+bn_stats_partial_kernel(long long rows, int c, const float *__restrict__ y, const float *__restrict__ w,
+                        float *__restrict__ partial) {
   __shared__ float4 red[THREADS];
   const int cq = c >> 2, c4 = threadIdx.x % cq, slot = threadIdx.x / cq, nslots = THREADS / cq;
+  const Rows in(y, w, c, c4);
   float4 acc[2] = {make_float4(0.f, 0.f, 0.f, 0.f), make_float4(0.f, 0.f, 0.f, 0.f)};
   for (long long r = (long long)blockIdx.x * nslots + slot; r < rows; r += (long long)gridDim.x * nslots) {
-    const float4 v = __ldg(reinterpret_cast<const float4 *>(y + r * c) + c4);
+    const float4 v = in(r);
     acc[0].x += v.x; acc[0].y += v.y; acc[0].z += v.z; acc[0].w += v.w;
     acc[1].x = fmaf(v.x, v.x, acc[1].x); acc[1].y = fmaf(v.y, v.y, acc[1].y);
     acc[1].z = fmaf(v.z, v.z, acc[1].z); acc[1].w = fmaf(v.w, v.w, acc[1].w);
@@ -290,22 +308,32 @@
   }
 }
 
-__global__ void __launch_bounds__(THREADS)
-bn_relu_bwd_reduce_kernel(long long rows, int c, const float *__restrict__ y, const float *__restrict__ dz,
-                          const float *__restrict__ mean, const float *__restrict__ invstd,
-                          const float *__restrict__ gamma, const float *__restrict__ beta, float *__restrict__ partial) {
+template <class Rows>
+__global__ void __launch_bounds__(THREADS)
+bn_relu_bwd_reduce_kernel(long long rows, int c, const float *__restrict__ y, const float *__restrict__ w,
+                          const float *__restrict__ dz, const float *__restrict__ mean,
+                          const float *__restrict__ invstd, const float *__restrict__ gamma,
+                          const float *__restrict__ beta, float *__restrict__ partial) {
   __shared__ float4 red[THREADS];
   const int cq = c >> 2, c4 = threadIdx.x % cq, slot = threadIdx.x / cq, nslots = THREADS / cq;
   const Affine4 a = load_affine(mean, invstd, gamma, beta, c4);
+  const Rows in(y, w, c, c4);
   float4 acc[2] = {make_float4(0.f, 0.f, 0.f, 0.f), make_float4(0.f, 0.f, 0.f, 0.f)};
-  for (long long r = (long long)blockIdx.x * nslots + slot; r < rows; r += (long long)gridDim.x * nslots) {
-    const float4 xh = xhat4(__ldg(reinterpret_cast<const float4 *>(y + r * c) + c4), a);
+  auto row = [&](long long r) {
+    const float4 xh = xhat4(in(r), a);
     const float4 z = bn4(xh, a);
     float4 d = __ldg(reinterpret_cast<const float4 *>(dz + r * c) + c4);
     d.x = z.x > 0.f ? d.x : 0.f; d.y = z.y > 0.f ? d.y : 0.f; d.z = z.z > 0.f ? d.z : 0.f; d.w = z.w > 0.f ? d.w : 0.f;
     acc[0].x += d.x; acc[0].y += d.y; acc[0].z += d.z; acc[0].w += d.w;
     acc[1].x = fmaf(d.x, xh.x, acc[1].x); acc[1].y = fmaf(d.y, xh.y, acc[1].y);
     acc[1].z = fmaf(d.z, xh.z, acc[1].z); acc[1].w = fmaf(d.w, xh.w, acc[1].w);
+  };
+  const long long r0 = (long long)blockIdx.x * nslots + slot, step = (long long)gridDim.x * nslots;
+  if constexpr (Rows::kRebuilt) {
+#pragma unroll 2
+    for (long long r = r0; r < rows; r += step) row(r);
+  } else {
+    for (long long r = r0; r < rows; r += step) row(r);
   }
   reduce_slots<2>(acc, cq, slot, c4, red);
   if (slot == 0) {
@@ -406,7 +434,7 @@
   }
 }
 
-template <int CIN>
+template <int CIN, class Rows>
 __global__ void __launch_bounds__(THREADS)
 bn_relu_bwd_small_k_kernel(long long rows, int c, const float *__restrict__ y, const float *__restrict__ dz,
                            const float *__restrict__ mean, const float *__restrict__ invstd,
@@ -417,11 +445,12 @@
   const int cq = c >> 2, c4 = threadIdx.x % cq, slot = threadIdx.x / cq, nslots = THREADS / cq;
   const Affine4 a = load_affine(mean, invstd, gamma, beta, c4);
   const BwdCoef4 q = load_coef(a, s1, s2, c4, 1.0f / (float)rows);
+  const Rows in(Rows::kRebuilt ? x : y, y, c, c4);
   float4 acc[CIN];
 #pragma unroll
   for (int k = 0; k < CIN; ++k) acc[k] = make_float4(0.f, 0.f, 0.f, 0.f);
-  for (long long r = (long long)blockIdx.x * nslots + slot; r < rows; r += (long long)gridDim.x * nslots) {
-    const float4 xh = xhat4(__ldg(reinterpret_cast<const float4 *>(y + r * c) + c4), a);
+  auto row = [&](long long r) {
+    const float4 xh = xhat4(in(r), a);
     const float4 z = bn4(xh, a);
     float4 d = __ldg(reinterpret_cast<const float4 *>(dz + r * c) + c4);
     d.x = z.x > 0.f ? d.x : 0.f; d.y = z.y > 0.f ? d.y : 0.f; d.z = z.z > 0.f ? d.z : 0.f; d.w = z.w > 0.f ? d.w : 0.f;
@@ -432,6 +461,13 @@
       acc[k].x = fmaf(g.x, xv, acc[k].x); acc[k].y = fmaf(g.y, xv, acc[k].y);
       acc[k].z = fmaf(g.z, xv, acc[k].z); acc[k].w = fmaf(g.w, xv, acc[k].w);
     }
+  };
+  const long long r0 = (long long)blockIdx.x * nslots + slot, step = (long long)gridDim.x * nslots;
+  if constexpr (Rows::kRebuilt) {
+#pragma unroll 2
+    for (long long r = r0; r < rows; r += step) row(r);
+  } else {
+    for (long long r = r0; r < rows; r += step) row(r);
   }
   reduce_slots<CIN>(acc, cq, slot, c4, red);
   if (slot == 0) {
@@ -453,6 +489,22 @@
   dw[i] = (float)a;
 }
 
+template <bool REBUILT>
+int launch_bwd_small_k(long long rows, int cin, int cout, const float *y, const float *dz, const float *mean,
+                       const float *invstd, const float *gamma, const float *beta, const float *s1, const float *s2,
+                       const float *x, float *dw, float *scratch, cudaStream_t s) {
+  const unsigned grid = grid_for(rows, cout);
+#define CODA_CASE(K)                                                                                              \
+  case K:                                                                                                         \
+    bn_relu_bwd_small_k_kernel<K, std::conditional_t<REBUILT, FirstLayerRows<K>, StoredRows>>                     \
+        <<<grid, THREADS, 0, s>>>(rows, cout, y, dz, mean, invstd, gamma, beta, s1, s2, x, scratch);              \
+    break;
+  switch (cin) { CODA_CASE(1) CODA_CASE(2) CODA_CASE(3) CODA_CASE(4) CODA_CASE(5) CODA_CASE(6) CODA_CASE(7) CODA_CASE(8) }
+#undef CODA_CASE
+  dw_finalize_kernel<<<(cin * cout + 127) / 128, 128, 0, s>>>((int)grid, cin * cout, scratch, dw);
+  return coda::launch_status();
+}
+
 }
 
 extern "C" {
@@ -478,7 +530,7 @@
   if (rows <= 0 || !channels_ok(c) || !y || !mean || !invstd || !scratch) return CODA_EINVAL;
   cudaStream_t s = (cudaStream_t)stream;
   const unsigned grid = grid_for(rows, c);
-  bn_stats_partial_kernel<<<grid, THREADS, 0, s>>>(rows, c, y, scratch);
+  bn_stats_partial_kernel<StoredRows><<<grid, THREADS, 0, s>>>(rows, c, y, nullptr, scratch);
   bn_stats_finalize_kernel<<<(c + 7) / 8, 256, 0, s>>>((int)grid, rows, c, scratch, eps, momentum, running_mean,
                                                            running_var, mean, invstd);
   return coda::launch_status();
@@ -491,7 +543,7 @@
     return CODA_EINVAL;
   cudaStream_t s = (cudaStream_t)stream;
   const unsigned grid = grid_for(rows, c);
-  bn_stats_partial_kernel<<<grid, THREADS, 0, s>>>(rows, c, y, scratch);
+  bn_stats_partial_kernel<StoredRows><<<grid, THREADS, 0, s>>>(rows, c, y, nullptr, scratch);
   const int cpad = (c + 63) / 64 * 64;
   bn_stats_finalize_affine_kernel<<<(cpad + 7) / 8, 256, 0, s>>>((int)grid, rows, c, cpad, scratch, eps, momentum,
                                                                     running_mean, running_var, gamma, beta, mean,
@@ -514,7 +566,7 @@
   if (rows <= 0 || !channels_ok(c) || !y || !sums || !scratch) return CODA_EINVAL;
   cudaStream_t s = (cudaStream_t)stream;
   const unsigned grid = grid_for(rows, c);
-  bn_stats_partial_kernel<<<grid, THREADS, 0, s>>>(rows, c, y, scratch);
+  bn_stats_partial_kernel<StoredRows><<<grid, THREADS, 0, s>>>(rows, c, y, nullptr, scratch);
   bn_sums_f64_kernel<<<(c + 7) / 8, 256, 0, s>>>((int)grid, c, scratch, sums);
   return coda::launch_status();
 }
@@ -589,7 +641,27 @@
     return CODA_EINVAL;
   cudaStream_t s = (cudaStream_t)stream;
   const unsigned grid = grid_for(rows, c);
-  bn_relu_bwd_reduce_kernel<<<grid, THREADS, 0, s>>>(rows, c, y, dz, mean, invstd, gamma, beta, scratch);
+  bn_relu_bwd_reduce_kernel<StoredRows><<<grid, THREADS, 0, s>>>(rows, c, y, nullptr, dz, mean, invstd, gamma, beta,
+                                                                 scratch);
+  sums_finalize_kernel<<<(c + 7) / 8, 256, 0, s>>>((int)grid, c, scratch, s1, s2);
+  return coda::launch_status();
+}
+
+int coda_bn_relu_bwd_reduce_first(long long rows, int cin, int c, const float *x, const float *w0, const float *dz,
+                                  const float *mean, const float *invstd, const float *gamma, const float *beta,
+                                  float *s1, float *s2, float *scratch, void *stream) {
+  if (rows <= 0 || cin < 1 || cin > 8 || !channels_ok(c) || !x || !w0 || !dz || !mean || !invstd || !gamma || !beta ||
+      !s1 || !s2 || !scratch)
+    return CODA_EINVAL;
+  cudaStream_t s = (cudaStream_t)stream;
+  const unsigned grid = grid_for(rows, c);
+#define CODA_CASE(K)                                                                                                  \
+  case K:                                                                                                             \
+    bn_relu_bwd_reduce_kernel<FirstLayerRows<K>><<<grid, THREADS, 0, s>>>(rows, c, x, w0, dz, mean, invstd, gamma, beta, \
+                                                                         scratch);                                    \
+    break;
+  switch (cin) { CODA_CASE(1) CODA_CASE(2) CODA_CASE(3) CODA_CASE(4) CODA_CASE(5) CODA_CASE(6) CODA_CASE(7) CODA_CASE(8) }
+#undef CODA_CASE
   sums_finalize_kernel<<<(c + 7) / 8, 256, 0, s>>>((int)grid, c, scratch, s1, s2);
   return coda::launch_status();
 }
@@ -638,17 +710,31 @@
                              const float *s2, const float *x, float *dw, float *scratch, void *stream) {
   if (rows <= 0 || cin < 1 || cin > 8 || !channels_ok(cout)) return CODA_EINVAL;
   if (!y || !dz || !mean || !invstd || !gamma || !beta || !s1 || !s2 || !x || !dw || !scratch) return CODA_EINVAL;
-  cudaStream_t s = (cudaStream_t)stream;
-  const unsigned grid = grid_for(rows, cout);
-#define CODA_CASE(K)                                                                                              \
-  case K:                                                                                                         \
-    bn_relu_bwd_small_k_kernel<K><<<grid, THREADS, 0, s>>>(rows, cout, y, dz, mean, invstd, gamma, beta, s1, s2, x, \
-                                                           scratch);                                             \
-    break;
+  return launch_bwd_small_k<false>(rows, cin, cout, y, dz, mean, invstd, gamma, beta, s1, s2, x, dw, scratch,
+                                   (cudaStream_t)stream);
+}
+
+int coda_bn_relu_bwd_small_k_first(long long rows, int cin, int cout, const float *w0, const float *dz,
+                                   const float *mean, const float *invstd, const float *gamma, const float *beta,
+                                   const float *s1, const float *s2, const float *x, float *dw, float *scratch,
+                                   void *stream) {
+  if (rows <= 0 || cin < 1 || cin > 8 || !channels_ok(cout)) return CODA_EINVAL;
+  if (!w0 || !dz || !mean || !invstd || !gamma || !beta || !s1 || !s2 || !x || !dw || !scratch) return CODA_EINVAL;
+  return launch_bwd_small_k<true>(rows, cin, cout, w0, dz, mean, invstd, gamma, beta, s1, s2, x, dw, scratch,
+                                  (cudaStream_t)stream);
+}
+
+int coda_bn_first_layer_partials(long long rows, int cin, int c, const float *x, const float *w0, float *partial,
+                                 int *nblocks, void *stream) {
+  if (rows <= 0 || cin < 1 || cin > 8 || !channels_ok(c) || !x || !w0 || !partial || !nblocks) return CODA_EINVAL;
+  cudaStream_t s = (cudaStream_t)stream;
+  const unsigned grid = grid_for(rows, c);
+#define CODA_CASE(K) \
+  case K: bn_stats_partial_kernel<FirstLayerRows<K>><<<grid, THREADS, 0, s>>>(rows, c, x, w0, partial); break;
   switch (cin) { CODA_CASE(1) CODA_CASE(2) CODA_CASE(3) CODA_CASE(4) CODA_CASE(5) CODA_CASE(6) CODA_CASE(7) CODA_CASE(8) }
 #undef CODA_CASE
-  dw_finalize_kernel<<<(cin * cout + 127) / 128, 128, 0, s>>>((int)grid, cin * cout, scratch, dw);
-  return coda::launch_status();
-}
-
-}
+  *nblocks = (int)grid;
+  return coda::launch_status();
+}
+
+}
diff --git a/coda_neurips2023_b200/ops.py b/coda_neurips2023_b200/ops.py
--- a/coda_neurips2023_b200/ops.py
+++ b/coda_neurips2023_b200/ops.py
@@ -825,6 +825,7 @@
 
 A32_PLAIN, A32_AFFINE_RELU, A32_BN_BWD, A32_BN_BWD_POOLED = 0, 1, 2, 3
 A32_BN_BWD_POOLED_PRE = 4
+A32_SMALLK_AFFINE_RELU = 5
 
 
 def a32_ok(a: torch.Tensor) -> bool:
@@ -834,11 +835,14 @@
 
 def gemm_a32(a: torch.Tensor, b_planes: torch.Tensor, n: int, *, mode: int = A32_PLAIN, scale=None, shift=None,
              alpha=None, beta=None, a2=None, argmax=None, group: int = 0, b_mn: bool = False, bias=None,
-             relu: bool = False, out: torch.Tensor | None = None, want_stats: bool = False, nsplit: int | None = None):
+             relu: bool = False, out: torch.Tensor | None = None, want_stats: bool = False, nsplit: int | None = None,
+             w0=None):
     _need_cuda(a, "gemm_a32")
-    m, k = a.shape
+    small_k = mode == A32_SMALLK_AFFINE_RELU
+    m, k = (a.shape[0], w0.shape[0]) if small_k else a.shape
     ns = b_planes.shape[0] if nsplit is None else nsplit
-    assert a32_ok(a) and 2 <= ns <= b_planes.shape[0] and b_planes.dtype == torch.bfloat16
+    assert (a.is_contiguous() and a.dtype == torch.float32 and w0.is_contiguous()) if small_k else a32_ok(a)
+    assert 2 <= ns <= b_planes.shape[0] and b_planes.dtype == torch.bfloat16
     ld = b_planes.shape[3]
     if out is None:
         out = torch.empty((m, n), dtype=torch.float32, device=a.device)
@@ -853,10 +857,12 @@
     elif mode in (A32_BN_BWD_POOLED, A32_BN_BWD_POOLED_PRE):
         assert a2.is_contiguous() and argmax.is_contiguous() and a2.shape == (m // group, k)
     with torch.cuda.device(a.device):
-        st = L.coda_gemm_a32(_i(ns), _i(m), _i(n), _i(k), ptr(a), _ll(a.stride(0)), _i(mode), ptr(scale), ptr(shift),
-                             ptr(alpha), ptr(beta), ptr(a2), _ll(lda2), ptr(argmax), _i(group), ptr(b_planes),
-                             _ll(b_planes.stride(0)), _i(ld), _i(1 if b_mn else 0), ptr(bias), _i(1 if relu else 0),
-                             ptr(out), _ll(out.stride(0)), ptr(stats), stream_of(a))
+        st = L.coda_gemm_a32(_i(ns), _i(m), _i(n), _i(k), ptr(None if small_k else a), _ll(0 if small_k else a.stride(0)),
+                             _i(mode), ptr(scale), ptr(shift), ptr(alpha), ptr(beta), ptr(a2), _ll(lda2), ptr(argmax),
+                             _i(group), ptr(b_planes), _ll(b_planes.stride(0)), _i(ld), _i(1 if b_mn else 0),
+                             ptr(bias), _i(1 if relu else 0), ptr(out), _ll(out.stride(0)), ptr(stats),
+                             ptr(a if small_k else None), ptr(w0 if small_k else None), _i(a.shape[1] if small_k else 0),
+                             stream_of(a))
     check(st, "gemm_a32")
     return (out, stats) if want_stats else out
 
@@ -867,11 +873,14 @@
 
 def gemm_tn32(a: torch.Tensor, b: torch.Tensor, *, a_mode: int = A32_PLAIN, a_scale=None, a_shift=None, a_alpha=None,
               a_beta=None, a2=None, argmax=None, group: int = 0, b_mode: int = A32_PLAIN, b_scale=None,
-              b_shift=None, out: torch.Tensor | None = None, colsum_out: torch.Tensor | None = None) -> torch.Tensor:
+              b_shift=None, out: torch.Tensor | None = None, colsum_out: torch.Tensor | None = None,
+              b_w0=None) -> torch.Tensor:
     _need_cuda(a, "gemm_tn32")
     rows, m = a.shape
-    n = b.shape[1]
-    assert tn32_ok(a) and tn32_ok(b) and b.shape[0] == rows
+    small_k = b_mode == A32_SMALLK_AFFINE_RELU
+    n = b_w0.shape[0] if small_k else b.shape[1]
+    assert tn32_ok(a) and b.shape[0] == rows
+    assert (b.is_contiguous() and b.dtype == torch.float32 and b_w0.is_contiguous()) if small_k else tn32_ok(b)
     if out is None:
         out = torch.empty((m, n), dtype=torch.float32, device=a.device)
     assert out.shape == (m, n) and out.stride(1) == 1 and out.stride(0) % 4 == 0 and out.data_ptr() % 16 == 0
@@ -884,8 +893,9 @@
     with torch.cuda.device(a.device):
         st = lib().coda_gemm_tn32(_ll(rows), _i(m), _i(n), ptr(a), _ll(a.stride(0)), _i(a_mode), ptr(a_scale),
                                   ptr(a_shift), ptr(a_alpha), ptr(a_beta), ptr(a2), _ll(lda2), ptr(argmax), _i(group),
-                                  ptr(b), _ll(b.stride(0)), _i(b_mode), ptr(b_scale), ptr(b_shift), ptr(out),
-                                  _ll(out.stride(0)), ptr(colsum_out), stream_of(a))
+                                  ptr(None if small_k else b), _ll(0 if small_k else b.stride(0)), _i(b_mode),
+                                  ptr(b_scale), ptr(b_shift), ptr(out), _ll(out.stride(0)), ptr(colsum_out),
+                                  ptr(b if small_k else None), ptr(b_w0), _i(b.shape[1] if small_k else 0), stream_of(a))
     check(st, "gemm_tn32")
     return out
 
diff --git a/coda_neurips2023_b200/sa_mlp.py b/coda_neurips2023_b200/sa_mlp.py
--- a/coda_neurips2023_b200/sa_mlp.py
+++ b/coda_neurips2023_b200/sa_mlp.py
@@ -10,6 +10,8 @@
 
 _i, _ll, _f = ctypes.c_int, ctypes.c_longlong, ctypes.c_float
 BACKWARD_PLANES = 2
+RECOMPUTE_FIRST = True
+FIRST_WIDTH = 64
 
 
 def _channels_ok(c: int) -> bool:
@@ -33,6 +35,22 @@
         if cout > 256 and (li > 0 or cin > 8):
             return False
     return True
+
+
+def _rebuilds_first(x: torch.Tensor, w0: torch.Tensor, nl: int) -> bool:
+    return (RECOMPUTE_FIRST and nl >= 2 and x.shape[1] <= 8 and w0.shape[0] == FIRST_WIDTH
+            and x.data_ptr() % 16 == 0)
+
+
+def _first_layer_partials(x: torch.Tensor, w0: torch.Tensor) -> torch.Tensor:
+    rows, cin = x.shape
+    c = w0.shape[0]
+    part = _scratch(c, x.device)
+    nblocks = ctypes.c_int(0)
+    with torch.cuda.device(x.device):
+        check(lib().coda_bn_first_layer_partials(_ll(rows), _i(cin), _i(c), ptr(x), ptr(w0), ptr(part),
+                                                 ctypes.byref(nblocks), stream_of(x)), "bn_first_layer_partials")
+    return part[: nblocks.value * 2 * c].view(nblocks.value, 2, c)
 
 
 def _scratch(c: int, device) -> torch.Tensor:
@@ -119,13 +137,19 @@
         dev = x.device
         ys, means, invstds, scales, shifts = [], [], [], [], []
         small_k = c0 <= 8
+        first = small_k and _rebuilds_first(x, params[0], nl)
+        w0 = params[0].contiguous()
         scale = shift = None
         with torch.cuda.device(dev):
             for li in range(nl):
                 w, gamma, beta = params[3 * li: 3 * li + 3]
                 cout, cin = w.shape
                 last = li == nl - 1
-                if li == 0 and small_k:
+                if li == 0 and first:
+                    y = None
+                    part = _first_layer_partials(x, w0)
+                    mean, invstd, scale, shift = _stats_from_partials(part, rows, bns[li], gamma, beta, True)
+                elif li == 0 and small_k:
                     y = torch.empty((rows, cout), dtype=torch.float32, device=dev)
                     check(L.coda_rows_linear_small_k(_ll(rows), _i(cin), _i(cout), ptr(x), ptr(w.contiguous()), ptr(y),
                                                      stream_of(x)), "rows_linear_small_k")
@@ -134,6 +158,9 @@
                     wp = ops._packed_weight(w, False, nsplit)
                     if li == 0:
                         y, part = ops.gemm_a32(x, wp, cout, want_stats=True)
+                    elif li == 1 and first:
+                        y, part = ops.gemm_a32(x, wp, cout, mode=ops.A32_SMALLK_AFFINE_RELU, w0=w0, scale=scale,
+                                               shift=shift, want_stats=True)
                     else:
                         y, part = ops.gemm_a32(ys[-1], wp, cout, mode=ops.A32_AFFINE_RELU, scale=scale, shift=shift,
                                                want_stats=True)
@@ -146,7 +173,7 @@
                     check(L.coda_bn_relu_maxpool_rows(_ll(groups), _i(group), _i(cout), ptr(y), ptr(mean), ptr(invstd),
                                                       ptr(gamma), ptr(beta), ptr(pooled), ptr(argmax), stream_of(x)),
                           "bn_relu_maxpool_rows")
-        ctx.nl, ctx.group, ctx.small_k, ctx.nsplit = nl, group, small_k, nsplit
+        ctx.nl, ctx.group, ctx.small_k, ctx.nsplit, ctx.first = nl, group, small_k, nsplit, first
         ctx.sync = ops.bn_sync_world() > 1
         ctx.save_for_backward(x, argmax, *ys, *means, *invstds, *scales, *shifts, *params)
         ctx.mark_non_differentiable(argmax)
@@ -170,6 +197,7 @@
         grads = [None] * (3 * nl)
         dx = None
         dz = None
+        w0 = params[0].contiguous()
         dpooled = dpooled.contiguous()
         with torch.cuda.device(dev):
             for li in range(nl - 1, -1, -1):
@@ -189,6 +217,10 @@
                                                            ptr(argmax), ptr(mean), ptr(invstd), ptr(gamma), ptr(beta),
                                                            ptr(s1), ptr(s2), ptr(scratch), ptr(dprime), stream_of(x)),
                           "bn_relu_bwd_reduce_pooled")
+                elif li == 0 and ctx.first:
+                    check(L.coda_bn_relu_bwd_reduce_first(_ll(rows), _i(cin), _i(cout), ptr(x), ptr(w0), ptr(dz),
+                                                          ptr(mean), ptr(invstd), ptr(gamma), ptr(beta), ptr(s1),
+                                                          ptr(s2), ptr(scratch), stream_of(x)), "bn_relu_bwd_reduce_first")
                 else:
                     check(L.coda_bn_relu_bwd_reduce(_ll(rows), _i(cout), ptr(y), ptr(dz), ptr(mean), ptr(invstd),
                                                     ptr(gamma), ptr(beta), ptr(s1), ptr(s2), ptr(scratch), stream_of(x)),
@@ -210,9 +242,15 @@
                     sc = torch.empty(int(L.coda_bn_rows_small_k_scratch_floats(_i(cin), _i(cout))), dtype=torch.float32,
                                      device=dev)
                     dw = torch.empty((cout, cin), dtype=torch.float32, device=dev) if sw is None else sw
-                    check(L.coda_bn_relu_bwd_small_k(_ll(rows), _i(cin), _i(cout), ptr(y), ptr(dz), ptr(mean), ptr(invstd),
-                                                     ptr(gamma), ptr(beta), ptr(s1), ptr(s2), ptr(x), ptr(dw), ptr(sc),
-                                                     stream_of(x)), "bn_relu_bwd_small_k")
+                    if ctx.first:
+                        check(L.coda_bn_relu_bwd_small_k_first(_ll(rows), _i(cin), _i(cout), ptr(w0), ptr(dz), ptr(mean),
+                                                               ptr(invstd), ptr(gamma), ptr(beta), ptr(s1), ptr(s2),
+                                                               ptr(x), ptr(dw), ptr(sc), stream_of(x)),
+                              "bn_relu_bwd_small_k_first")
+                    else:
+                        check(L.coda_bn_relu_bwd_small_k(_ll(rows), _i(cin), _i(cout), ptr(y), ptr(dz), ptr(mean),
+                                                         ptr(invstd), ptr(gamma), ptr(beta), ptr(s1), ptr(s2), ptr(x),
+                                                         ptr(dw), ptr(sc), stream_of(x)), "bn_relu_bwd_small_k")
                     grads[0] = dw if sw is None else ops._sunk(sw)
                     break
                 if sw is not None and cin % 4 != 0:
@@ -233,7 +271,10 @@
                     mode, a2, extra = ops.A32_BN_BWD, dz, {}
                 else:
                     mode, a2, extra = ops.A32_BN_BWD, dz, {}
-                if li > 0:
+                if li == 1 and ctx.first:
+                    grads[3 * li] = ops.gemm_tn32(y, x, a_mode=mode, a2=a2, b_mode=ops.A32_SMALLK_AFFINE_RELU,
+                                                  b_scale=scales[0], b_shift=shifts[0], b_w0=w0, out=sw, **pro, **extra)
+                elif li > 0:
                     grads[3 * li] = ops.gemm_tn32(y, ys[li - 1], a_mode=mode, a2=a2, b_mode=ops.A32_AFFINE_RELU,
                                                   b_scale=scales[li - 1], b_shift=shifts[li - 1], out=sw, **pro, **extra)
                 else:
diff --git a/include/coda_gemm.h b/include/coda_gemm.h
--- a/include/coda_gemm.h
+++ b/include/coda_gemm.h
@@ -37,17 +37,19 @@
 #define CODA_A32_BN_BWD 2
 #define CODA_A32_BN_BWD_POOLED 3
 #define CODA_A32_BN_BWD_POOLED_PRE 4
+#define CODA_A32_SMALLK_AFFINE_RELU 5
 int coda_gemm_a32_grid(int m, int n);
 int coda_gemm_a32(int nsplit, int m, int n, int k, const float *a, long long lda, int a_mode, const float *a_scale,
                   const float *a_shift, const float *a_alpha, const float *a_beta, const float *a2, long long lda2,
                   const unsigned char *a_argmax, int a_group, const void *b_planes, long long b_plane_stride,
                   int b_ld, int b_mn, const float *bias, int act, float *c, long long ldc, float *col_stats,
-                  void *stream);
+                  const float *x0, const float *w0, int cin, void *stream);
 
 int coda_gemm_tn32(long long rows, int m, int n, const float *a, long long lda, int a_mode, const float *a_scale,
                    const float *a_shift, const float *a_alpha, const float *a_beta, const float *a2, long long lda2,
                    const unsigned char *a_argmax, int a_group, const float *b, long long ldb, int b_mode,
-                   const float *b_scale, const float *b_shift, float *c, long long ldc, float *a_colsum, void *stream);
+                   const float *b_scale, const float *b_shift, float *c, long long ldc, float *a_colsum,
+                   const float *x0, const float *w0, int cin, void *stream);
 
 #ifdef __cplusplus
 }
diff --git a/include/coda_sa_mlp.h b/include/coda_sa_mlp.h
--- a/include/coda_sa_mlp.h
+++ b/include/coda_sa_mlp.h
@@ -9,6 +9,16 @@
 
 int coda_rows_linear_small_k(long long rows, int cin, int cout, const float *x, const float *w, float *y,
                              void *stream);
+
+int coda_bn_first_layer_partials(long long rows, int cin, int c, const float *x, const float *w0, float *partial,
+                                 int *nblocks, void *stream);
+int coda_bn_relu_bwd_reduce_first(long long rows, int cin, int c, const float *x, const float *w0, const float *dz,
+                                  const float *mean, const float *invstd, const float *gamma, const float *beta,
+                                  float *s1, float *s2, float *scratch, void *stream);
+int coda_bn_relu_bwd_small_k_first(long long rows, int cin, int cout, const float *w0, const float *dz,
+                                   const float *mean, const float *invstd, const float *gamma, const float *beta,
+                                   const float *s1, const float *s2, const float *x, float *dw, float *scratch,
+                                   void *stream);
 
 int coda_bn_rows_stats(long long rows, int c, const float *y, float eps, float momentum, float *running_mean,
                        float *running_var, float *mean, float *invstd, float *scratch, void *stream);
```
